# vwxyzjn/cleanrl

Measured on NVIDIA H100. Metric: env steps/sec (SPS) PPO Breakout num_envs=1024, higher is better.
Workload: dtype bf16

## Files before the change

### cleanrl_b200/csrc/common.cuh

```cuda
#pragma once
#include <cuda_runtime.h>
#include <cstdarg>
#include <cstdint>
#include <cstdio>
#include "../../include/b200rl.h"

namespace b200rl {

char* err_buf();
int fail(int code, const char* fmt, ...);

void note_launches(int n);
inline int check_launch(const char* what, int kernels = 1) {
    note_launches(kernels);
    cudaError_t e = cudaGetLastError();
    if (e != cudaSuccess) return fail(B200RL_ERR_CUDA, "%s: %s", what, cudaGetErrorString(e));
    return B200RL_OK;
}

#define B200RL_REQUIRE(cond, ...) \
    do { if (!(cond)) return ::b200rl::fail(B200RL_ERR_INVALID_ARGUMENT, __VA_ARGS__); } while (0)

inline bool aligned(const void* p, size_t a) { return (reinterpret_cast<uintptr_t>(p) % a) == 0; }
inline int64_t ceil_div(int64_t a, int64_t b) { return (a + b - 1) / b; }

bool prof_enabled();
void prof_begin(cudaStream_t s, const char* name, double flops, double bytes);
void prof_end(cudaStream_t s);
struct ProfScope {
    cudaStream_t s; bool on;
    ProfScope(cudaStream_t s_, const char* name, double flops, double bytes) : s(s_), on(prof_enabled()) {
        if (on) prof_begin(s, name, flops, bytes);
    }
    ~ProfScope() { if (on) prof_end(s); }
};

__device__ __forceinline__ float warp_sum(float v) {
#pragma unroll
    for (int o = 16; o > 0; o >>= 1) v += __shfl_xor_sync(0xffffffffu, v, o);
    return v;
}

__device__ __forceinline__ float block_sum(float v, float* red) {
    const int lane = threadIdx.x & 31, wid = threadIdx.x >> 5;
    v = warp_sum(v);
    __syncthreads();
    if (lane == 0) red[wid] = v;
    __syncthreads();
    const int nw = (blockDim.x + 31) >> 5;
    float r = (threadIdx.x < nw) ? red[threadIdx.x] : 0.f;
    if (wid == 0) r = warp_sum(r);
    if (threadIdx.x == 0) red[0] = r;
    __syncthreads();
    r = red[0];
    return r;
}

}
```

### cleanrl_b200/csrc/net_tc.cu

```cuda
#include <cuda.h>
#include <algorithm>
#include "tc_base.cuh"
#include "tc_conv_win.cuh"
#include "tc_conv1_u8.cuh"
#include "tc_gemm_tma.cuh"
#include "tc_wgrad_win.cuh"
#include "tc_reduce.cuh"
#include "tc_aux.cuh"
#include "tc_heads.cuh"
#include "tc_heads_wide.cuh"
#include "tc_lstm.cuh"

namespace b200rl {

struct NatureLayout {
    int A;
    int64_t c1w, c1b, c2w, c2b, c3w, c3b, fcw, fcb, hw, hb, total;
    int64_t w1f, w2f, w2dg, w3f, w3dg, wfcf, wfcdg, w1l, w1sc, packed_total;
    bool wide; int G; int64_t whf, whdg, hbp;
    int64_t wih, whh, bih, bhh, whhp;
    explicit NatureLayout(int A_) : A(A_), wih(-1), whh(-1), bih(-1), bhh(-1), whhp(-1) {
        int64_t o = 0;
        c1w = o; o += 32 * 4 * 8 * 8;  c1b = o; o += 32;
        c2w = o; o += 64 * 32 * 4 * 4; c2b = o; o += 64;
// ... 52 lines not shown
    }
};

struct NatureActs {
    int64_t x0, act1, act2, act3, hid, dhid, dact3a, dact3b, dact2a, dact2b, dact1, m1, m2, m3, m4, total;
    explicit NatureActs(int64_t n, bool with_x0 = true) {
        int64_t o = 0;
        x0 = o; if (with_x0) o += n * 28224;
        act1 = o; o += n * 12800;
        act2 = o; o += n * 5184;
        act3 = o; o += n * 3136;
        hid = o;  o += n * 512;
        dhid = o; o += n * 512;
        dact3a = o; o += n * 5184;
        dact3b = o; o += n * 7744;
        dact2a = o; o += n * 6400;
        dact2b = o; o += n * 7744;
        dact1 = o; o += n * 14112;
        auto pad8 = [](int64_t v) { return (v + 7) & ~int64_t(7); };
        m1 = o; o += pad8(n * 100 * 4 * 2);
        m2 = o; o += pad8(n * 81 * 2 * 2);
        m3 = o; o += pad8(n * 49 * 2 * 2);
        m4 = o; o += pad8(n * 16 * 2);
        total = o;
    }
};

static void gemm_rowmajor(KGemmParams& p, const bf16* x, int64_t n, int nchunks) {
    memset(&p, 0, sizeof(p));
    p.scale = 1.f;
    p.A = x; p.M = n; p.nchunks = nchunks;
}


static void win_defaults(WinParams& p) { memset(&p, 0, sizeof(p)); p.scale = 1.f; }
static int round8(int v) { return (v + 7) & ~7; }
static void win_conv1(WinParams& p, const bf16* x0, const int64_t* rows, int64_t n) {
    p.A = x0; p.rows = rows; p.n = (int)n; p.G = 441; p.Wp = 21; p.M = n * 441;
    p.tpi_shift = 2;
    p.n_images = rows ? (int64_t)1 << 24 : n;
    p.ntaps = 4; p.shift[0] = 0; p.shift[1] = 1; p.shift[2] = 21; p.shift[3] = 22; p.WR = round8(128 + 22);
}
static void win_conv2(WinParams& p, const bf16* act1, int64_t n) {
    p.A = act1; p.n = (int)n; p.G = 100; p.Wp = 10; p.M = n * 100;
    p.ntaps = 4; p.shift[0] = 0; p.shift[1] = 1; p.shift[2] = 10; p.shift[3] = 11; p.WR = round8(128 + 11);
}
static void win_conv3(WinParams& p, const bf16* act2, int64_t n) {
    p.A = act2; p.n = (int)n; p.G = 81; p.Wp = 9; p.M = n * 81;
    p.ntaps = 9; for (int ky = 0; ky < 3; ++ky) for (int kx = 0; kx < 3; ++kx) p.shift[ky * 3 + kx] = ky * 9 + kx;
    p.WR = round8(128 + 20);
}
static void wgw_defaults(WGradWinParams& w) { memset(&w, 0, sizeof(w)); }

static const int kC1Ctas = 264, kC2Ctas = 132, kC3Ctas = 132;
static WPlan conv1_wgrad_plan(int64_t n, bool u8) {
    return u8 ? wgrad_plan(n * 512, kC2Ctas, 512) : wgrad_plan(n * 512, kC1Ctas, 128);
}
static WPlan conv2_wgrad_plan(int64_t n) { return wgrad_plan(n * 100, kC2Ctas, 128); }
static WPlan conv3_wgrad_plan(int64_t n) { return wgrad_plan(n * 81, kC3Ctas, 128); }

static size_t wgrad_win_bytes(int splits, int nslots) { return (size_t)splits * nslots * 64 * 64 * sizeof(float); }
static size_t wgrad_win_bias_bytes(int splits) { return (size_t)splits * 64 * sizeof(float); }
static int launch_wgrad_win(const WGradWinParams& p, int ctas, cudaStream_t s, const char* what) {
    const size_t smem = (size_t)kWgradWinStages * ((size_t)p.WRX * 128 * p.cpr + 128 * 128) + 4096 + 1024;
    static SmemAttrCache attr;
    if (int rc0 = attr.ensure(tc_wgrad_win, smem, what)) return rc0;
    CUtensorMap tmX, tmY;
    memset(&tmX, 0, sizeof(tmX)); memset(&tmY, 0, sizeof(tmY));
    const int use_tma = p.tpi_shift ? 0 : 1;
    if (p.rows_per_cta % 128 != 0) return fail(B200RL_ERR_INVALID_ARGUMENT, "%s: rows per CTA must be a multiple of 128", what);
    if (ctas < 1 || (int64_t)(ctas - 1) * p.rows_per_cta >= p.M)
        return fail(B200RL_ERR_INVALID_ARGUMENT, "%s: every row split must own at least one row", what);
    int rc;
    if (use_tma) {
        if (p.rows || p.ldy != 64 || p.ncolsY != 64)
            return fail(B200RL_ERR_INVALID_ARGUMENT, "%s: linear-grid mode needs contiguous rows and 64-channel dY", what);
        if ((rc = make_tmap_2d(&tmX, p.X, p.M, (int64_t)p.cpr * 64, p.WRX, what))) return rc;
        if ((rc = make_tmap_2d(&tmY, p.Y, p.M, 64, 128, what))) return rc;
    } else {
        if ((128 << p.tpi_shift) < p.G) return fail(B200RL_ERR_INVALID_ARGUMENT, "%s: steps per image too small", what);
        if ((rc = make_tmap_3d(&tmX, p.X, p.n_images, p.G, (int64_t)p.cpr * 64, p.WRX, what))) return rc;
    }
    const dim3 grid((unsigned)ceil_div(p.nslots / 2, kWgradWinTilesPerCta), ctas);
    tc_wgrad_win<<<grid, kWgradWinThreads, smem, s>>>(tmX, tmY, p, use_tma);
    return check_launch(what);
}

}

using namespace b200rl;

namespace b200rl {
static bool head_ok(int A) { return A >= 1 && A < kMaxWideHeads; }
static size_t wide_dhead_bytes(int64_t n, const NatureLayout& L) { return ((size_t)n * L.G * 2 + 255) & ~(size_t)255; }
static size_t wide_small_bytes(int64_t n, const NatureLayout& L, int A1) {
    return wide_dhead_bytes(n, L) + colsum_f32_ws(n, A1);
}

static int trunk_fwd(const NatureLayout& L, const NatureActs& Q, const float* params, const bf16* P, bf16* act, int64_t n,
                     cudaStream_t s) {
    int rc;
    KGemmParams p;
    WinParams wp;
    win_defaults(wp); win_conv2(wp, act + Q.act1, n);
    wp.Bw = P + L.w2f; wp.N = 64; wp.vH = 9; wp.vW = 9; wp.out_mode = WOUT_DENSE; wp.out = act + Q.act2;
    wp.bias = params + L.c2b; wp.relu = 1; wp.mask_out = reinterpret_cast<uint32_t*>(act + Q.m2);
    { ProfScope ps(s, "conv2_fwd", 2.0 * n * 81 * 64 * 512, (double)n * ((12800 + 5184) * 2 + 648));
      if ((rc = launch_conv_win_t<128, 2, 2, 4>(wp, s, "naturecnn/conv2"))) return rc; }
    win_defaults(wp); win_conv3(wp, act + Q.act2, n);
    wp.Bw = P + L.w3f; wp.N = 64; wp.vH = 7; wp.vW = 7; wp.out_mode = WOUT_DENSE; wp.out = act + Q.act3;
    wp.bias = params + L.c3b; wp.relu = 1; wp.mask_out = reinterpret_cast<uint32_t*>(act + Q.m3);
    { ProfScope ps(s, "conv3_fwd", 2.0 * n * 49 * 64 * 576, (double)n * ((5184 + 3136) * 2 + 392));
      if ((rc = launch_conv_win_t<128, 1, 4, 9>(wp, s, "naturecnn/conv3"))) return rc; }
    gemm_rowmajor(p, act + Q.act3, n, 49);
    p.Bw = P + L.wfcf; p.N = 512; p.out = act + Q.hid; p.ldo = 512; p.bias = params + L.fcb; p.relu = 1;
    p.mask_out = reinterpret_cast<uint32_t*>(act + Q.m4);
    { ProfScope ps(s, "fc_fwd", 2.0 * n * 512 * 3136, (double)n * (3136 + 512) * 2 + 512.0 * 3136 * 2);
      if (n <= 8192) { if ((rc = launch_gemm_tma<64, 6>(p, s, "naturecnn/fc"))) return rc; }
      else if ((rc = launch_gemm_tma<128, 4>(p, s, "naturecnn/fc"))) return rc; }
    return B200RL_OK;
}

static int trunk_bwd(const NatureLayout& L, const NatureActs& Q, const bf16* P, bf16* act, float* grads, int64_t n,
                     float* wsbig, float* wssmall, void* tail_ready_event, bool dact1_fused, cudaStream_t s) {
    int rc;
    KGemmParams p;
    {
        int splits;
        { ProfScope ps(s, "fc_wgrad", 2.0 * n * 512 * 3136, (double)n * (3136 + 512) * 2 + 512.0 * 3136 * 4);
          if ((splits = launch_wgrad_tma(act + Q.dhid, 512, act + Q.act3, 3136, n, wsbig, s, "naturecnn/fc_wgrad")) < 0) return splits; }
        { ProfScope ps(s, "wgrad_fold_bias", 0, 0);
          note_launches(1); tc_fold_fc<<<(unsigned)ceil_div((int64_t)512 * 3136, 256), 256, 0, s>>>(wsbig, splits, 512, 13 * 256, 512, 3136, 64, 49, 1.f, grads + L.fcw);
          if ((rc = colsum(act + Q.dhid, n, 512, 512, wssmall, grads + L.fcb, s))) return rc; }
        if (tail_ready_event) {
            cudaError_t e = cudaEventRecord(reinterpret_cast<cudaEvent_t>(tail_ready_event), s);
            if (e != cudaSuccess) return fail(B200RL_ERR_CUDA, "naturecnn_backward: cudaEventRecord: %s", cudaGetErrorString(e));
        }
        gemm_rowmajor(p, act + Q.dhid, n, 8);
        p.Bw = P + L.wfcdg; p.N = 3136; p.out = act + Q.dact3a; p.out2 = act + Q.dact3b; p.dual_dact3 = 1;
        p.ldo = 3136; p.mask_bits = reinterpret_cast<const uint32_t*>(act + Q.m3);
        { ProfScope ps(s, "fc_dgrad", 2.0 * n * 512 * 3136, (double)n * ((3136 + 512) * 2 + 392) + 512.0 * 3136 * 2);
          if ((rc = launch_gemm_tma<128, 4>(p, s, "naturecnn/fc_dgrad"))) return rc; }
    }
    WGradWinParams gw;
    WinParams wp;
    FoldWin fw;
    {
        wgw_defaults(gw);
        gw.X = act + Q.act2; gw.M = n * 81; gw.n = (int)n; gw.G = 81; gw.cpr = 1; gw.nslots = 10; gw.WRX = round8(128 + 20);
        for (int t = 0; t < 9; ++t) gw.shift[t] = (t / 3) * 9 + (t % 3);
        const int st[10] = {0, 1, 2, 3, 4, 5, 6, 7, 7, 8};
        for (int k = 0; k < 10; ++k) { gw.slot_tap[k] = st[k]; gw.slot_cc[k] = 0; }
        gw.Y = act + Q.dact3a; gw.ldy = 64; gw.ncolsY = 64;
        const WPlan pl = conv3_wgrad_plan(n);
        gw.rows_per_cta = pl.rows_per_cta; gw.ws = wsbig; gw.wsb = wssmall;
        { ProfScope ps(s, "conv3_wgrad", 2.0 * n * 49 * 64 * 576, (double)n * (5184 + 5184) * 2);
          if ((rc = launch_wgrad_win(gw, pl.splits, s, "naturecnn/conv3_wgrad"))) return rc; }
        memset(&fw, 0, sizeof(fw));
        fw.layer = 3; fw.S = pl.splits; fw.nslots = 10; fw.Cout = 64; fw.scale = 1.f; fw.bscale = 1.f;
        for (int k = 0; k < 10; ++k) { fw.slot_tap[k] = st[k]; fw.slot_skip[k] = (k == 8); }
        { ProfScope ps(s, "wgrad_fold_bias", 0, 0);
          fw.wsb = wssmall; fw.db = grads + L.c3b;
          tc_fold_win<<<(unsigned)ceil_div(640 * 64 + 64, 32), 256, 0, s>>>(wsbig, fw, grads + L.c3w);
          if ((rc = check_launch("naturecnn/conv3_fold"))) return rc; }
        win_defaults(wp);
        wp.A = act + Q.dact3b; wp.n = (int)n; wp.G = 121; wp.Wp = 11; wp.M = n * 121; wp.ntaps = 9;
        for (int ky = 0; ky < 3; ++ky) for (int kx = 0; kx < 3; ++kx) wp.shift[ky * 3 + kx] = (2 - ky) * 11 + (2 - kx);
        wp.WR = round8(128 + 24);
        wp.Bw = P + L.w3dg; wp.N = 64; wp.vH = 9; wp.vW = 9; wp.out_mode = WOUT_DACT2;
        wp.out = act + Q.dact2a; wp.out2 = act + Q.dact2b; wp.mask_bits = reinterpret_cast<const uint32_t*>(act + Q.m2);
        { ProfScope ps(s, "conv3_dgrad", 2.0 * n * 81 * 64 * 576, (double)n * ((7744 + 6400 + 7744) * 2 + 648));
          if ((rc = launch_conv_win_t<128, 1, 4, 9>(wp, s, "naturecnn/conv3_dgrad"))) return rc; }
    }
    {
        wgw_defaults(gw);
        gw.X = act + Q.act1; gw.M = n * 100; gw.n = (int)n; gw.G = 100; gw.cpr = 2; gw.nslots = 8; gw.WRX = round8(128 + 11);
        gw.shift[0] = 0; gw.shift[1] = 1; gw.shift[2] = 10; gw.shift[3] = 11;
        for (int k = 0; k < 8; ++k) { gw.slot_tap[k] = k >> 1; gw.slot_cc[k] = k & 1; }
        gw.Y = act + Q.dact2a; gw.ldy = 64; gw.ncolsY = 64;
        const WPlan pl = conv2_wgrad_plan(n);
        gw.rows_per_cta = pl.rows_per_cta; gw.ws = wsbig; gw.wsb = wssmall;
        { ProfScope ps(s, "conv2_wgrad", 2.0 * n * 81 * 64 * 512, (double)n * (12800 + 6400) * 2);
          if ((rc = launch_wgrad_win(gw, pl.splits, s, "naturecnn/conv2_wgrad"))) return rc; }
        memset(&fw, 0, sizeof(fw));
        fw.layer = 2; fw.S = pl.splits; fw.nslots = 8; fw.Cout = 64; fw.scale = 1.f; fw.bscale = 1.f;
        for (int k = 0; k < 8; ++k) { fw.slot_tap[k] = k >> 1; fw.slot_cc[k] = k & 1; }
        { ProfScope ps(s, "wgrad_fold_bias", 0, 0);
          fw.wsb = wssmall; fw.db = grads + L.c2b;
          tc_fold_win<<<(unsigned)ceil_div(512 * 64 + 64, 32), 256, 0, s>>>(wsbig, fw, grads + L.c2w);
          if ((rc = check_launch("naturecnn/conv2_fold"))) return rc; }
        if (dact1_fused) return B200RL_OK;
        win_defaults(wp);
        wp.A = act + Q.dact2b; wp.n = (int)n; wp.G = 121; wp.Wp = 11; wp.M = n * 121; wp.ntaps = 4;
        for (int a = 0; a < 2; ++a) for (int b = 0; b < 2; ++b) wp.shift[a * 2 + b] = (1 - a) * 11 + (1 - b);
        wp.WR = round8(128 + 12);
        wp.Bw = P + L.w2dg; wp.N = 128; wp.vH = 10; wp.vW = 10; wp.out_mode = WOUT_DACT1;
        wp.out = act + Q.dact1; wp.mask_bits = reinterpret_cast<const uint32_t*>(act + Q.m1);
        { ProfScope ps(s, "conv2_dgrad", 2.0 * n * 400 * 32 * 256, (double)n * ((7744 + 14112) * 2 + 1600));
          if ((rc = launch_conv_win<128, 1, 4, 4>(wp, s, "naturecnn/conv2_dgrad"))) return rc; }
    }
    return B200RL_OK;
}
static size_t trunk_big_bytes(int64_t n) {
    return std::max({wgrad_tma_bytes(n, 512, 3136), wgrad_win_bytes(conv3_wgrad_plan(n).splits, 10),
                     wgrad_win_bytes(conv2_wgrad_plan(n).splits, 8)});
}
static size_t trunk_small_bytes(int64_t n) {
    return std::max({colsum_ws(n, 512), wgrad_win_bias_bytes(conv3_wgrad_plan(n).splits),
                     wgrad_win_bias_bytes(conv2_wgrad_plan(n).splits)});
}

static int wide_head_fwd(const NatureLayout& L, const bf16* P, const bf16* hid, int64_t n, int A1, float* out, cudaStream_t s) {
    KGemmParams p;
    gemm_rowmajor(p, hid, n, 8);
    p.Bw = P + L.whf; p.N = L.G; p.bias = reinterpret_cast<const float*>(P + L.hbp);
    p.out_f32 = out; p.ldo = A1; p.ncols_f32 = A1;
    return launch_gemm_tma<128, 4>(p, s, "wide_heads");
}

static int wide_head_bwd(const NatureLayout& L, const bf16* P, const float* dhead, int64_t n, int A1, const bf16* hid, bf16* dhid,
                         const uint32_t* hid_bits, float* dW, float* db, float* wsbig, float* wssmall, cudaStream_t s) {
    int rc;
    KGemmParams p;
    bf16* dh16 = reinterpret_cast<bf16*>(wssmall);
    float* dbpart = reinterpret_cast<float*>(reinterpret_cast<char*>(wssmall) + wide_dhead_bytes(n, L));
    int cb = (int)ceil_div(n * L.G, 256); if (cb > num_sms() * 8) cb = num_sms() * 8;
    tc_head_dhead_bf16<<<cb, 256, 0, s>>>(dhead, n, A1, L.G, dh16);
    if ((rc = check_launch("wide_heads_dhead"))) return rc;
    if ((rc = colsum_f32(dhead, n, A1, dbpart, db, s))) return rc;
    const int splits = launch_wgrad_tma(dh16, L.G, hid, 512, n, wsbig, s, "wide_heads_wgrad");
    if (splits < 0) return splits;
    tc_fold_fc<<<(unsigned)ceil_div((int64_t)A1 * 512, 256), 256, 0, s>>>(wsbig, splits, L.G, 512, A1, 512, 512, 1, 1.f, dW);
    if ((rc = check_launch("wide_heads_wgrad"))) return rc;
    gemm_rowmajor(p, dh16, n, L.G / 64);
    p.Bw = P + L.whdg; p.N = 512; p.out = dhid; p.ldo = 512;
    p.mask_bits = hid_bits;
    if (n <= 8192) { if ((rc = launch_gemm_tma<64, 6>(p, s, "wide_heads_dgrad"))) return rc; }
    else if ((rc = launch_gemm_tma<128, 4>(p, s, "wide_heads_dgrad"))) return rc;
    return B200RL_OK;
}
}

extern "C" int64_t b200rl_naturecnn_param_count(int A) { return A >= 1 ? NatureLayout(A).total : -1; }
extern "C" int64_t b200rl_naturecnn_grad_tail_offset(int A) { return A >= 1 ? NatureLayout(A).fcw : -1; }
extern "C" size_t b200rl_naturecnn_bf16_packed_bytes(int A) { return head_ok(A) ? (size_t)NatureLayout(A).packed_total * 2 : 0; }
extern "C" size_t b200rl_naturecnn_bf16_acts_bytes(int64_t n, int obs_format) {
    return n >= 0 ? (size_t)NatureActs(n, obs_format == B200RL_OBS_U8_NCHW).total * 2 + 256 : 0;
}

extern "C" int b200rl_frames_to_s2d_bf16(const uint8_t* obs, const int64_t* rows, int64_t n, void* out, void* stream) {
    B200RL_REQUIRE(n >= 0, "frames_to_s2d: negative n");
    if (n == 0) return B200RL_OK;
    B200RL_REQUIRE(obs && out, "frames_to_s2d: null pointer");
    B200RL_REQUIRE(aligned(obs, 4) && aligned(out, 16), "frames_to_s2d: misaligned buffer");
    cudaStream_t s = (cudaStream_t)stream;
    ProfScope ps(s, "frames_to_s2d", 0, (double)n * 28224 * 3);
    tc_frames_to_s2d<<<(unsigned)ceil_div(n * 1764, 256), 256, 0, s>>>(obs, rows, n, reinterpret_cast<bf16*>(out));
    return check_launch("frames_to_s2d");
}

extern "C" int b200rl_frames_to_s2d_u8(const uint8_t* obs, const int64_t* rows, int64_t n, uint8_t* out_rm, uint8_t* out_cm, void* stream) {
    B200RL_REQUIRE(n >= 0, "frames_to_s2d_u8: negative n");
    if (n == 0) return B200RL_OK;
    B200RL_REQUIRE(obs && out_rm && out_cm, "frames_to_s2d_u8: null pointer");
    B200RL_REQUIRE(aligned(obs, 16) && aligned(out_rm, 16) && aligned(out_cm, 16), "frames_to_s2d_u8: misaligned buffer");
    B200RL_REQUIRE(n <= (int64_t)1 << 28, "frames_to_s2d_u8: n too large");
    cudaStream_t s = (cudaStream_t)stream;
    ProfScope ps(s, "frames_to_s2d", 0, (double)n * (28224 + 28224 + 28672));
    tc_frames_to_s2d_u8<<<(unsigned)(n * 4), 256, 0, s>>>(obs, rows, n, out_rm, out_cm);
    return check_launch("frames_to_s2d_u8");
}

static size_t naturecnn_big_bytes(int64_t n, const NatureLayout& L) {
    return std::max({trunk_big_bytes(n), L.wide ? wgrad_tma_bytes(n, L.G, 512) : 0,
                     wgrad_win_bytes(conv1_wgrad_plan(n, false).splits, 4), wgrad_win_bytes(conv1_wgrad_plan(n, true).splits, 4)});
}

extern "C" size_t b200rl_naturecnn_bf16_workspace_bytes(int64_t n, int A) {
    if (n < 1 || !head_ok(A)) return 0;
    const NatureLayout L(A);
    const size_t small = std::max({trunk_small_bytes(n), L.wide ? wide_small_bytes(n, L, A + 1) : heads_partial_bytes(n, A + 1, 512),
                                   wgrad_win_bias_bytes(conv1_wgrad_plan(n, false).splits),
                                   wgrad_win_bias_bytes(conv1_wgrad_plan(n, true).splits)});
    return naturecnn_big_bytes(n, L) + small + 512;
}

extern "C" int b200rl_naturecnn_bf16_pack(const float* params, int A, void* packed, void* stream) {
    B200RL_REQUIRE(params && packed && head_ok(A), "naturecnn_pack: bad arguments (A must be in [1,%d])", kMaxWideHeads - 1);
    B200RL_REQUIRE(aligned(packed, 16), "naturecnn_pack: packed buffer must be 16-B aligned");
    const NatureLayout L(A);
    bf16* P = reinterpret_cast<bf16*>(packed);
    cudaStream_t s = (cudaStream_t)stream;
    ProfScope ps(s, "pack_weights", 0, (double)L.total * 4 + (double)L.packed_total * 2);
    tc_pack_conv1_s2d<<<32, 256, 0, s>>>(params + L.c1w, P + L.w1f);
    tc_pack_conv1_i8<<<32, 256, 0, s>>>(params + L.c1w, reinterpret_cast<int8_t*>(P + L.w1l), reinterpret_cast<float*>(P + L.w1sc));
    tc_pack_conv2_cells<<<128, 256, 0, s>>>(params + L.c2w, P + L.w2f);
    tc_pack_conv_s2_classes<<<(unsigned)ceil_div(32768, 256), 256, 0, s>>>(params + L.c2w, 64, 32, P + L.w2dg);
    tc_pack_conv<<<(unsigned)ceil_div(36864, 256), 256, 0, s>>>(params + L.c3w, 64, 64, 3, 3, 0, P + L.w3f, P + L.w3dg);
    tc_pack_fc<<<dim3(512 / 8, 49 / 7), 256, 0, s>>>(params + L.fcw, 512, 49, P + L.wfcf, P + L.wfcdg);
    if (L.wide) {
        tc_pack_head_wide<<<(unsigned)ceil_div((int64_t)L.G * 512, 256), 256, 0, s>>>(params + L.hw, params + L.hb, A + 1, L.G,
                                                                                    P + L.whf, P + L.whdg, reinterpret_cast<float*>(P + L.hbp));
        return check_launch("naturecnn_pack", 7);
    }
    return check_launch("naturecnn_pack", 6);
}

extern "C" int b200rl_naturecnn_bf16_forward(const void* obs, int obs_format, const int64_t* rows, int64_t n, int A,
                                             const float* params, const void* packed, void* acts,
                                             float* head_out, void* stream) {
    B200RL_REQUIRE(n >= 0, "naturecnn_forward: negative n");
    if (n == 0) return B200RL_OK;
    B200RL_REQUIRE(obs && params && packed && acts && head_out, "naturecnn_forward: null pointer");
    B200RL_REQUIRE(head_ok(A), "naturecnn_forward: A=%d outside [1,%d]", A, kMaxWideHeads - 1);
    B200RL_REQUIRE(obs_format == B200RL_OBS_U8_NCHW || obs_format == B200RL_OBS_S2D_BF16 || obs_format == B200RL_OBS_S2D_U8,
                   "naturecnn_forward: bad obs_format %d", obs_format);
    B200RL_REQUIRE(aligned(obs, 16) && aligned(acts, 16) && aligned(packed, 16), "naturecnn_forward: misaligned buffer");
    B200RL_REQUIRE(n <= (int64_t)1 << 22, "naturecnn_forward: n too large");
    const NatureLayout L(A);
    const NatureActs Q(n, obs_format == B200RL_OBS_U8_NCHW);
    const bf16* P = reinterpret_cast<const bf16*>(packed);
    bf16* act = reinterpret_cast<bf16*>(acts);
    cudaStream_t s = (cudaStream_t)stream;
    int rc;
    WinParams wp;
    const bf16* x0 = reinterpret_cast<const bf16*>(obs);
    const int64_t* x0rows = rows;
    if (obs_format == B200RL_OBS_U8_NCHW) {
        if ((rc = b200rl_frames_to_s2d_bf16(reinterpret_cast<const uint8_t*>(obs), rows, n, act + Q.x0, stream))) return rc;
        x0 = act + Q.x0; x0rows = nullptr;
    }
    if (obs_format == B200RL_OBS_S2D_U8) {
        Conv1U8Params cp;
        memset(&cp, 0, sizeof(cp));
        cp.rows = rows; cp.n = (int)n; cp.n_images = rows ? (int64_t)1 << 24 : n;
        cp.limbs = reinterpret_cast<const int8_t*>(P + L.w1l); cp.sc = reinterpret_cast<const float*>(P + L.w1sc);
        cp.bias = params + L.c1b; cp.out = act + Q.act1; cp.mask_out = reinterpret_cast<uint32_t*>(act + Q.m1);
        ProfScope ps(s, "conv1_fwd", 2.0 * n * 400 * 32 * 256, (double)n * (28224 + 12800 * 2 + 1600));
        if ((rc = launch_conv1_i8(cp, obs, s, "naturecnn/conv1_i8"))) return rc;
    } else {
    win_defaults(wp); win_conv1(wp, x0, x0rows, n);
    wp.Bw = P + L.w1f; wp.N = 32; wp.vH = 20; wp.vW = 20; wp.out_mode = WOUT_S2D2; wp.out = act + Q.act1;
    wp.bias = params + L.c1b; wp.scale = 1.0f / 255.0f; wp.relu = 1; wp.mask_out = reinterpret_cast<uint32_t*>(act + Q.m1);
    { ProfScope ps(s, "conv1_fwd", 2.0 * n * 400 * 32 * 256, (double)n * ((28224 + 12800) * 2 + 1600));
      if ((rc = launch_conv_win<32, 1, 9, 4>(wp, s, "naturecnn/conv1"))) return rc; }
    }
    if ((rc = trunk_fwd(L, Q, params, P, act, n, s))) return rc;
    if (L.wide) {
        ProfScope ps(s, "heads_fwd", 2.0 * n * 512 * (A + 1), (double)n * (1024 + 4 * (A + 1)) + (double)L.G * 1024);
        return wide_head_fwd(L, P, act + Q.hid, n, A + 1, head_out, s);
    }
    ProfScope ps(s, "heads_fwd", 2.0 * n * 512 * (A + 1), (double)n * (1024 + 4 * (A + 1)));
    return heads_fwd<512>(act + Q.hid, params + L.hw, params + L.hb, n, A + 1, head_out, s, "naturecnn/heads");
}

extern "C" int b200rl_naturecnn_bf16_backward(const void* obs, const void* obs_aux, int obs_format, const int64_t* rows, int64_t n, int A,
                                              const float* params, const void* packed, void* acts,
                                              const float* dhead, float* grads,
                                              void* workspace, size_t workspace_bytes, void* tail_ready_event, void* stream) {
    B200RL_REQUIRE(n >= 1, "naturecnn_backward: n must be >= 1");
    B200RL_REQUIRE(obs && params && packed && acts && dhead && grads && workspace, "naturecnn_backward: null pointer");
    B200RL_REQUIRE(head_ok(A), "naturecnn_backward: A=%d outside [1,%d]", A, kMaxWideHeads - 1);
    B200RL_REQUIRE(aligned(workspace, 16), "naturecnn_backward: workspace misaligned");
    const size_t need = b200rl_naturecnn_bf16_workspace_bytes(n, A);
    if (workspace_bytes < need) return fail(B200RL_ERR_WORKSPACE, "naturecnn_backward: workspace %zu < %zu", workspace_bytes, need);
    B200RL_REQUIRE(obs_format == B200RL_OBS_U8_NCHW || obs_format == B200RL_OBS_S2D_BF16 || obs_format == B200RL_OBS_S2D_U8,
                   "naturecnn_backward: bad obs_format %d", obs_format);
    B200RL_REQUIRE(obs_format != B200RL_OBS_S2D_U8 || (obs_aux && aligned(obs_aux, 16)), "naturecnn_backward: the uint8 rollout needs obs_aux");
    const NatureLayout L(A);
    const NatureActs Q(n, obs_format == B200RL_OBS_U8_NCHW);
    const bf16* P = reinterpret_cast<const bf16*>(packed);
    bf16* act = reinterpret_cast<bf16*>(acts);
    cudaStream_t s = (cudaStream_t)stream;
    const bf16* x0 = obs_format == B200RL_OBS_U8_NCHW ? act + Q.x0 : reinterpret_cast<const bf16*>(obs);
    const int64_t* x0rows = obs_format == B200RL_OBS_U8_NCHW ? nullptr : rows;
    const size_t big = (naturecnn_big_bytes(n, L) + 255) & ~(size_t)255;
    float* wsbig = reinterpret_cast<float*>(workspace);
    float* wssmall = reinterpret_cast<float*>(reinterpret_cast<char*>(workspace) + big);
    int rc;
    const int A1 = A + 1;
    if (L.wide) {
        ProfScope ps(s, "heads_bwd", 4.0 * n * 512 * A1, (double)n * (2048 + 64 + 8 * A1));
        if ((rc = wide_head_bwd(L, P, dhead, n, A1, act + Q.hid, act + Q.dhid, reinterpret_cast<const uint32_t*>(act + Q.m4),
                                grads + L.hw, grads + L.hb, wsbig, wssmall, s))) return rc;
    } else
    {
        ProfScope ps(s, "heads_bwd", 4.0 * n * 512 * A1, (double)n * (2048 + 64 + 8 * A1));
        if ((rc = heads_bwd_weight<512>(dhead, act + Q.hid, n, A1, wssmall, grads + L.hw, grads + L.hb, s, "naturecnn/heads_bwd"))) return rc;
        if ((rc = heads_bwd_data<512>(dhead, params + L.hw, reinterpret_cast<const uint8_t*>(act + Q.m4), n, A1, act + Q.dhid, s,
                                      "naturecnn/heads_bwd"))) return rc;
    }
    if ((rc = trunk_bwd(L, Q, P, act, grads, n, wsbig, wssmall, tail_ready_event, obs_format == B200RL_OBS_S2D_U8, s))) return rc;
    const bool u8 = obs_format == B200RL_OBS_S2D_U8;
    const WPlan pl = conv1_wgrad_plan(n, u8);
    if (u8) {
        Conv21BwdU8Params cw;
        memset(&cw, 0, sizeof(cw));
        cw.rows = rows; cw.n = (int)n; cw.rows_per_cta = pl.rows_per_cta; cw.ws = wsbig; cw.wsb = wssmall;
        cw.w2dg = P + L.w2dg; cw.m1 = reinterpret_cast<const uint32_t*>(act + Q.m1);
        { ProfScope ps(s, "conv21_bwd", 2.0 * 2.0 * n * 400 * 32 * 256, (double)n * (7744 * 2 + 1600 + 28672 + 14112 * 2));
          if ((rc = launch_conv21_bwd_u8(cw, obs_aux, rows ? (int64_t)1 << 24 : n, act + Q.dact2b, act + Q.dact1, pl.splits, s,
                                         "naturecnn/conv21_bwd_u8"))) return rc; }
    } else {
        WGradWinParams gw;
        wgw_defaults(gw);
        gw.X = x0; gw.rows = x0rows; gw.M = n * 512; gw.n = (int)n; gw.G = 441; gw.cpr = 1; gw.nslots = 4; gw.WRX = round8(128 + 22);
        gw.tpi_shift = 2; gw.n_images = x0rows ? (int64_t)1 << 24 : n;
        gw.shift[0] = 0; gw.shift[1] = 1; gw.shift[2] = 21; gw.shift[3] = 22;
        for (int k = 0; k < 4; ++k) { gw.slot_tap[k] = k; gw.slot_cc[k] = 0; }
        gw.Y = act + Q.dact1; gw.ldy = 32; gw.ncolsY = 32;
        gw.rows_per_cta = pl.rows_per_cta; gw.ws = wsbig; gw.wsb = wssmall;
        { ProfScope ps(s, "conv1_wgrad", 2.0 * n * 400 * 32 * 256, (double)n * (28224 + 14112) * 2);
          if ((rc = launch_wgrad_win(gw, pl.splits, s, "naturecnn/conv1_wgrad"))) return rc; }
    }
    FoldWin fw;
    memset(&fw, 0, sizeof(fw));
    fw.layer = 1; fw.S = pl.splits; fw.nslots = 4; fw.Cout = 32;
    fw.scale = u8 ? 1.0f / 255.0f / kDact1Scale : 1.0f / 255.0f;
    fw.bscale = u8 ? 1.0f / kDact1Scale : 1.f;
    for (int k = 0; k < 4; ++k) fw.slot_tap[k] = k;
    { ProfScope ps(s, "wgrad_fold_bias", 0, 0);
      fw.wsb = wssmall; fw.db = grads + L.c1b;
      tc_fold_win<<<(unsigned)ceil_div(256 * 32 + 32, 32), 256, 0, s>>>(wsbig, fw, grads + L.c1w);
      if ((rc = check_launch("naturecnn/conv1_fold"))) return rc; }
    return B200RL_OK;
}

namespace b200rl {
constexpr int64_t kLstmMaxRows = (int64_t)1 << 17;

struct LstmActs {
    NatureActs T;
    int64_t gx, hseq, hm, save, cm, dgates, total;
    explicit LstmActs(int64_t M) : T(M, false) {
        int64_t o = (T.total * 2 + 255) & ~int64_t(255);
        auto take = [&](int64_t bytes) { const int64_t r = o; o += (bytes + 255) & ~int64_t(255); return r; };
        gx = take(M * 512 * 4);
        hseq = take(M * 128 * 2);
        hm = take(M * 128 * 2);
        save = take(M * 640 * 4);
        cm = take(M * 128 * 4);
        dgates = take(M * 512 * 4);
        total = o;
    }
};

static bool lstm_heads_ok(int A) { return A >= 1 && A + 1 <= lstm::kMaxA1; }
static bool lstm_sizes_ok(int64_t S, int64_t n) { return S >= 1 && n >= 1 && S <= kLstmMaxRows && n <= kLstmMaxRows && S * n <= kLstmMaxRows; }

struct C1Plan { int64_t per_cta; int ctas; };
static C1Plan lstm_conv1_plan(int64_t M) {
    C1Plan c;
    const int64_t want = M < kC1Ctas ? M : kC1Ctas;
    c.per_cta = ceil_div(M, want);
    c.ctas = (int)ceil_div(M, c.per_cta);
    return c;
}
static size_t lstm_big_bytes(int64_t M, const NatureLayout& L) {
    const size_t a = std::max({wgrad_tma_bytes(M, L.G, 512), wgrad_tma_bytes(M, 512, 128), trunk_big_bytes(M),
                               (size_t)lstm_conv1_plan(M).ctas * 32 * 64 * 4});
    return (a + 255) & ~(size_t)255;
}
static size_t lstm_small_bytes(int64_t M, const NatureLayout& L) {
    return std::max({heads_partial_bytes(M, L.A + 1, 128), wide_small_bytes(M, L, 512), trunk_small_bytes(M),
                     (size_t)lstm_conv1_plan(M).ctas * 32 * 4});
}
}

extern "C" int64_t b200rl_lstm_agent_param_count(int A) { return A >= 1 ? NatureLayout(A, NatureLayout::Lstm{}).total : -1; }
extern "C" size_t b200rl_lstm_agent_bf16_packed_bytes(int A) {
    return lstm_heads_ok(A) ? (size_t)NatureLayout(A, NatureLayout::Lstm{}).packed_total * 2 : 0;
}
extern "C" size_t b200rl_lstm_agent_bf16_acts_bytes(int64_t S, int64_t n) {
    return lstm_sizes_ok(S, n) ? (size_t)LstmActs(S * n).total : 0;
}
extern "C" int b200rl_lstm_agent_bf16_acts_layout(int64_t S, int64_t n, int64_t* offsets) {
    B200RL_REQUIRE(offsets, "lstm_acts_layout: null pointer");
    B200RL_REQUIRE(lstm_sizes_ok(S, n), "lstm_acts_layout: S=%lld n=%lld out of range", (long long)S, (long long)n);
    const LstmActs Q(S * n);
    const int64_t v[B200RL_LSTM_ACTS_TENSORS] = {Q.T.act1 * 2, Q.T.m1 * 2, Q.T.act2 * 2, Q.T.act3 * 2, Q.T.hid * 2, Q.T.m4 * 2,
                                                 Q.gx, Q.hseq, Q.hm, Q.save, Q.cm, Q.dgates, Q.T.dhid * 2};
    for (int k = 0; k < B200RL_LSTM_ACTS_TENSORS; ++k) offsets[k] = v[k];
    return B200RL_OK;
}
extern "C" size_t b200rl_lstm_agent_bf16_workspace_bytes(int64_t S, int64_t n, int A) {
    if (!lstm_sizes_ok(S, n) || !lstm_heads_ok(A)) return 0;
    const NatureLayout L(A, NatureLayout::Lstm{});
    return lstm_big_bytes(S * n, L) + lstm_small_bytes(S * n, L) + 512;
}

extern "C" int b200rl_lstm_agent_bf16_pack(const float* params, int A, void* packed, void* stream) {
    B200RL_REQUIRE(params && packed, "lstm_pack: null pointer");
    B200RL_REQUIRE(lstm_heads_ok(A), "lstm_pack: A=%d outside [1,%d]", A, lstm::kMaxA1 - 1);
    B200RL_REQUIRE(aligned(params, 16) && aligned(packed, 16), "lstm_pack: misaligned buffer");
    const NatureLayout L(A, NatureLayout::Lstm{});
    bf16* P = reinterpret_cast<bf16*>(packed);
    cudaStream_t s = (cudaStream_t)stream;
    ProfScope ps(s, "pack_weights", 0, (double)L.total * 4 + (double)L.packed_total * 2);
    lstm::lstm_pack_conv1<<<8, 256, 0, s>>>(params + L.c1w, P + L.w1f);
    tc_pack_conv2_cells<<<128, 256, 0, s>>>(params + L.c2w, P + L.w2f);
    tc_pack_conv_s2_classes<<<(unsigned)ceil_div(32768, 256), 256, 0, s>>>(params + L.c2w, 64, 32, P + L.w2dg);
    tc_pack_conv<<<(unsigned)ceil_div(36864, 256), 256, 0, s>>>(params + L.c3w, 64, 64, 3, 3, 0, P + L.w3f, P + L.w3dg);
    tc_pack_fc<<<dim3(512 / 8, 49 / 7), 256, 0, s>>>(params + L.fcw, 512, 49, P + L.wfcf, P + L.wfcdg);
    tc_pack_head_wide<<<(unsigned)ceil_div((int64_t)L.G * 512, 256), 256, 0, s>>>(params + L.wih, params + L.bih, 512, L.G,
                                                                                P + L.whf, P + L.whdg, reinterpret_cast<float*>(P + L.hbp));
    tc_head_dhead_bf16<<<256, 256, 0, s>>>(params + L.whh, 512, 128, 128, P + L.whhp);
    return check_launch("lstm_pack", 7);
// ... 121 lines not shown
```

### cleanrl_b200/csrc/optim.cu

```cuda
#include "common.cuh"

namespace b200rl {

constexpr int kOptThreads = 256;
constexpr int kOptMaxBlocks = 132 * 8;

struct OptScratch {
    float norm;
    float coef;
    unsigned int ticket;
    unsigned int pad;
};

__global__ void __launch_bounds__(kOptThreads) grad_sumsq_kernel(
    const float* __restrict__ g, int64_t P, float inv_world_is_div, float world,
    float max_norm, OptScratch* sc, double* partials, float* norm_out) {
    __shared__ float red[32];
    __shared__ bool is_last;
    float s = 0.f;
    const int64_t stride = (int64_t)gridDim.x * blockDim.x;
    const int64_t tid = (int64_t)blockIdx.x * blockDim.x + threadIdx.x;
    const int64_t P4 = P >> 2;
    const float4* g4 = reinterpret_cast<const float4*>(g);
    for (int64_t i = tid; i < P4; i += stride) {
        float4 v = __ldg(g4 + i);
        if (inv_world_is_div != 0.f) { v.x /= world; v.y /= world; v.z /= world; v.w /= world; }
        s += v.x * v.x + v.y * v.y + v.z * v.z + v.w * v.w;
    }
    for (int64_t i = (P4 << 2) + tid; i < P; i += stride) {
        float v = g[i];
        if (inv_world_is_div != 0.f) v /= world;
        s += v * v;
    }
    const float bs = block_sum(s, red);
    if (threadIdx.x == 0) {
        partials[blockIdx.x] = (double)bs;
        __threadfence();
        is_last = (atomicAdd(&sc->ticket, 1u) == gridDim.x - 1);
    }
    __syncthreads();
    if (!is_last) return;
    __threadfence();
    __shared__ double dred[kOptThreads];
    double mine = 0.0;
    for (unsigned b = threadIdx.x; b < gridDim.x; b += blockDim.x) mine += __ldcg(partials + b);
    dred[threadIdx.x] = mine;
    __syncthreads();
    for (unsigned off = kOptThreads / 2; off > 0; off >>= 1) {
        if (threadIdx.x < off) dred[threadIdx.x] += dred[threadIdx.x + off];
        __syncthreads();
    }
    if (threadIdx.x == 0) {
        const double tot = dred[0];
        const float norm = (float)sqrt(tot);
        sc->norm = norm;
        float coef = 1.f;
        if (max_norm >= 0.f) coef = fminf(max_norm / (norm + 1e-6f), 1.0f);
        sc->coef = coef;
        if (norm_out) *norm_out = norm;
        sc->ticket = 0;
    }
}

struct AdamScalars {
    float w1;
    float beta2;
    float w2;
    float bc2_sqrt;
    float eps;
    float neg_step_size;
    float world;
    int divide_world;
    int do_clip;
};

__device__ __forceinline__ void adam_one(float& p, float g, float& m, float& v, const AdamScalars& a, float coef) {
    if (a.divide_world) g = g / a.world;
    if (a.do_clip) g = g * coef;
    m = fmaf(a.w1, g - m, m);
    v = v * a.beta2;
    v = __fadd_rn(v, __fmul_rn(__fmul_rn(a.w2, g), g));
    const float denom = __fadd_rn(__fdiv_rn(sqrtf(v), a.bc2_sqrt), a.eps);
    p = __fadd_rn(p, __fmul_rn(a.neg_step_size, __fdiv_rn(m, denom)));
}

__global__ void __launch_bounds__(kOptThreads) adam_kernel(
    float* __restrict__ p, const float* __restrict__ g, float* __restrict__ m, float* __restrict__ v,
    int64_t P, AdamScalars a, const OptScratch* sc, const float* __restrict__ dyn) {
    if (dyn) { a.bc2_sqrt = __ldg(dyn); a.neg_step_size = __ldg(dyn + 1); }
    const float coef = a.do_clip ? sc->coef : 1.f;
    const int64_t stride = (int64_t)gridDim.x * blockDim.x;
    const int64_t tid = (int64_t)blockIdx.x * blockDim.x + threadIdx.x;
    const int64_t P4 = P >> 2;
    float4* p4 = reinterpret_cast<float4*>(p);
    const float4* g4 = reinterpret_cast<const float4*>(g);
    float4* m4 = reinterpret_cast<float4*>(m);
    float4* v4 = reinterpret_cast<float4*>(v);
    for (int64_t i = tid; i < P4; i += stride) {
        float4 pp = p4[i], gg = __ldg(g4 + i), mm = m4[i], vv = v4[i];
        adam_one(pp.x, gg.x, mm.x, vv.x, a, coef);
        adam_one(pp.y, gg.y, mm.y, vv.y, a, coef);
        adam_one(pp.z, gg.z, mm.z, vv.z, a, coef);
        adam_one(pp.w, gg.w, mm.w, vv.w, a, coef);
        p4[i] = pp; m4[i] = mm; v4[i] = vv;
    }
    for (int64_t i = (P4 << 2) + tid; i < P; i += stride) {
        float pp = p[i], mm = m[i], vv = v[i];
        adam_one(pp, g[i], mm, vv, a, coef);
        p[i] = pp; m[i] = mm; v[i] = vv;
    }
}

static inline unsigned opt_blocks(int64_t P) {
    int64_t b = ceil_div(ceil_div(P, 4), kOptThreads);
    if (b < 1) b = 1;
    if (b > kOptMaxBlocks) b = kOptMaxBlocks;
    return (unsigned)b;
}

}

extern "C" size_t b200rl_clip_adam_workspace_bytes(int64_t P) {
    (void)P;
    return sizeof(b200rl::OptScratch) + sizeof(double) * b200rl::kOptMaxBlocks;
}

namespace b200rl {
static void adam_step_scalars(int64_t step, double lr, double beta1, double beta2, float* bc2_sqrt, float* neg_step_size) {
    const double bc1 = 1.0 - pow(beta1, (double)step);
    const double bc2 = 1.0 - pow(beta2, (double)step);
    const double step_size = lr / bc1;
    *bc2_sqrt = (float)sqrt(bc2);
    *neg_step_size = (float)(-step_size);
}

static int clip_adam_impl(float* params, const float* grads, float* exp_avg, float* exp_avg_sq, int64_t P, int64_t step, double lr,
                          const float* dyn, double beta1, double beta2, double eps, double max_norm, int world_size, float* norm_out,
                          void* workspace, size_t workspace_bytes, void* stream) {
    B200RL_REQUIRE(P >= 0, "clip_adam: negative P");
    if (P == 0) return B200RL_OK;
    B200RL_REQUIRE(params && grads && exp_avg && exp_avg_sq, "clip_adam: null pointer");
    B200RL_REQUIRE(aligned(params, 16) && aligned(grads, 16) && aligned(exp_avg, 16) && aligned(exp_avg_sq, 16),
                   "clip_adam: buffers must be 16-B aligned (float4 path)");
    B200RL_REQUIRE(dyn || step >= 1, "clip_adam: step is 1-based (got %lld)", (long long)step);
    B200RL_REQUIRE(!dyn || aligned(dyn, 4), "clip_adam: misaligned scalar table");
    B200RL_REQUIRE(world_size >= 1, "clip_adam: world_size must be >= 1");
    B200RL_REQUIRE(workspace && aligned(workspace, 16), "clip_adam: workspace null or misaligned");
    if (workspace_bytes < b200rl_clip_adam_workspace_bytes(P))
        return fail(B200RL_ERR_WORKSPACE, "clip_adam: workspace %zu < %zu bytes", workspace_bytes,
                    b200rl_clip_adam_workspace_bytes(P));
    cudaStream_t s = (cudaStream_t)stream;
    OptScratch* sc = reinterpret_cast<OptScratch*>(workspace);
    double* partials = reinterpret_cast<double*>(reinterpret_cast<char*>(workspace) + sizeof(OptScratch));
    const unsigned blocks = opt_blocks(P);
    ProfScope ps(s, "clip_adam", 0, 32.0 * P);
    const bool need_norm = (max_norm >= 0.0) || (norm_out != nullptr);
    if (need_norm) {
        cudaError_t e = cudaMemsetAsync(&sc->ticket, 0, sizeof(unsigned int), s);
        if (e != cudaSuccess) return fail(B200RL_ERR_CUDA, "clip_adam: memset: %s", cudaGetErrorString(e));
        grad_sumsq_kernel<<<blocks, kOptThreads, 0, s>>>(grads, P, world_size > 1 ? 1.f : 0.f, (float)world_size,
                                                        (float)max_norm, sc, partials, norm_out);
        int rc = check_launch("clip_adam/sumsq");
        if (rc) return rc;
    }
    AdamScalars a;
    a.w1 = (float)(1.0 - beta1);
    a.beta2 = (float)beta2;
    a.w2 = (float)(1.0 - beta2);
    a.bc2_sqrt = 1.f;
    a.neg_step_size = 0.f;
    if (!dyn) adam_step_scalars(step, lr, beta1, beta2, &a.bc2_sqrt, &a.neg_step_size);
    a.eps = (float)eps;
    a.world = (float)world_size;
    a.divide_world = world_size > 1;
    a.do_clip = max_norm >= 0.0;
    adam_kernel<<<blocks, kOptThreads, 0, s>>>(params, grads, exp_avg, exp_avg_sq, P, a, sc, dyn);
    return check_launch("clip_adam/adam");
}
}

extern "C" int b200rl_clip_adam_f32(float* params, const float* grads, float* exp_avg, float* exp_avg_sq,
                                    int64_t P, int64_t step, double lr, double beta1, double beta2, double eps,
                                    double max_norm, int world_size, float* norm_out,
                                    void* workspace, size_t workspace_bytes, void* stream) {
    return b200rl::clip_adam_impl(params, grads, exp_avg, exp_avg_sq, P, step, lr, nullptr, beta1, beta2, eps, max_norm, world_size,
                                  norm_out, workspace, workspace_bytes, stream);
}

extern "C" int b200rl_adam_step_scalars(int64_t step, double lr, double beta1, double beta2, float* out2) {
    B200RL_REQUIRE(out2 && step >= 1, "adam_step_scalars: bad arguments");
    b200rl::adam_step_scalars(step, lr, beta1, beta2, out2, out2 + 1);
    return B200RL_OK;
}

extern "C" int b200rl_clip_adam_dyn_f32(float* params, const float* grads, float* exp_avg, float* exp_avg_sq,
                                        int64_t P, const float* step_scalars, double beta1, double beta2, double eps,
                                        double max_norm, int world_size, float* norm_out,
                                        void* workspace, size_t workspace_bytes, void* stream) {
    B200RL_REQUIRE(step_scalars, "clip_adam_dyn: null scalar table");
    return b200rl::clip_adam_impl(params, grads, exp_avg, exp_avg_sq, P, 0, 0.0, step_scalars, beta1, beta2, eps, max_norm, world_size,
                                  norm_out, workspace, workspace_bytes, stream);
}
```

### cleanrl_b200/csrc/policy.cu

```cuda
#include "common.cuh"
#include <cfloat>

namespace b200rl {

constexpr int kMaxA = 64;

struct RowStats {
    float lse;
    float m2;
    float s2;
};

__device__ __forceinline__ RowStats row_stats(const float* __restrict__ x, int A) {
    float m = -INFINITY;
    for (int k = 0; k < A; ++k) m = fmaxf(m, x[k]);
    const float mm = (fabsf(m) == INFINITY) ? 0.f : m;
    float s = 0.f;
    for (int k = 0; k < A; ++k) s += expf(x[k] - mm);
    RowStats r;
    r.lse = logf(s) + mm;
    float m2 = -INFINITY;
    for (int k = 0; k < A; ++k) m2 = fmaxf(m2, x[k] - r.lse);
    float s2 = 0.f;
    for (int k = 0; k < A; ++k) s2 += expf((x[k] - r.lse) - m2);
    r.m2 = m2;
    r.s2 = s2;
    return r;
}

__global__ void __launch_bounds__(128) categorical_sample_kernel(
    const float* __restrict__ logits, int64_t ld, const float* __restrict__ noise,
    const float* __restrict__ value_in, int64_t ldv, int64_t n, int A,
    int64_t* __restrict__ action, float* __restrict__ logprob, float* __restrict__ entropy,
    float* __restrict__ value_out) {
    const int64_t i = (int64_t)blockIdx.x * blockDim.x + threadIdx.x;
    if (i >= n) return;
    const float* x = logits + i * ld;
    const float* q = noise + i * (int64_t)A;
    const RowStats rs = row_stats(x, A);
    float best = -INFINITY, ent = 0.f;
    int arg = 0;
    for (int k = 0; k < A; ++k) {
        const float nl = x[k] - rs.lse;
        const float p = expf(nl - rs.m2) / rs.s2;
        const float sc = p / q[k];
        if (sc > best) { best = sc; arg = k; }
        ent += fmaxf(nl, -FLT_MAX) * p;
    }
    action[i] = arg;
    logprob[i] = x[arg] - rs.lse;
    if (entropy) entropy[i] = -ent;
    if (value_out && value_in) value_out[i] = value_in[i * ldv];
}

__global__ void __launch_bounds__(128) categorical_eval_kernel(
    const float* __restrict__ logits, int64_t ld, const int64_t* __restrict__ action, int64_t n, int A,
    float* __restrict__ logprob, float* __restrict__ entropy) {
    const int64_t i = (int64_t)blockIdx.x * blockDim.x + threadIdx.x;
    if (i >= n) return;
    const float* x = logits + i * ld;
    const RowStats rs = row_stats(x, A);
    float ent = 0.f;
    for (int k = 0; k < A; ++k) {
        const float nl = x[k] - rs.lse;
        ent += fmaxf(nl, -FLT_MAX) * (expf(nl - rs.m2) / rs.s2);
    }
    int a = (int)action[i];
    a = a < 0 ? 0 : (a >= A ? A - 1 : a);
    logprob[i] = x[a] - rs.lse;
    if (entropy) entropy[i] = -ent;
}

__device__ __forceinline__ float adv_pass(const float* __restrict__ b_adv, const int64_t* __restrict__ inds, int64_t M,
                                          float mean, bool squared) {
    float s = 0.f;
    const int64_t step = blockDim.x;
    int64_t i = threadIdx.x;
    for (; i + 7 * step < M; i += 8 * step) {
        int64_t j[8];
        float v[8];
#pragma unroll
        for (int u = 0; u < 8; ++u) j[u] = inds ? __ldg(inds + i + u * step) : i + u * step;
#pragma unroll
        for (int u = 0; u < 8; ++u) v[u] = __ldg(b_adv + j[u]);
#pragma unroll
        for (int u = 0; u < 8; ++u) {
            const float d = v[u] - mean;
            s += squared ? d * d : v[u];
        }
    }
    for (; i < M; i += step) {
        const float v = b_adv[inds ? inds[i] : i];
        const float d = v - mean;
        s += squared ? d * d : v;
    }
    return s;
}
__global__ void __launch_bounds__(1024) adv_stats_kernel(
    const float* __restrict__ b_adv, const int64_t* __restrict__ inds, int64_t M, float* __restrict__ out2) {
    __shared__ float red[32];
    const float mean = block_sum(adv_pass(b_adv, inds, M, 0.f, false), red) / (float)M;
    const float ss = block_sum(adv_pass(b_adv, inds, M, mean, true), red);
    if (threadIdx.x == 0) {
        out2[0] = mean;
        out2[1] = sqrtf(ss / (float)(M - 1));
    }
}

constexpr int kLossThreads = 256;
constexpr int kNumStats = 7;

struct LossParams {
    const float* logits; int64_t ld;
    const float* value; int64_t ldv;
    const int64_t* inds;
    const int64_t* b_actions;
    const float* b_logprobs; const float* b_adv; const float* b_ret; const float* b_val;
    int64_t M; int A;
    float clip, ent_coef, vf_coef;
    int norm_adv, clip_vloss;
    float* dlogits; int64_t ldd;
    float* dvalue; int64_t lddv;
    float* stats;
    const float* adv_stats;
    float* partials;
    unsigned int* ticket;
};

__global__ void __launch_bounds__(kLossThreads) ppo_loss_kernel(LossParams P) {
    __shared__ float red[32];
    __shared__ bool is_last;
    const int64_t i = (int64_t)blockIdx.x * blockDim.x + threadIdx.x;
    float acc[kNumStats];
#pragma unroll
    for (int k = 0; k < kNumStats; ++k) acc[k] = 0.f;
    if (i < P.M) {
        const int64_t j = P.inds ? P.inds[i] : i;
        const float* x = P.logits + i * P.ld;
        const int A = P.A;
        const int a = (int)P.b_actions[j];
        const RowStats rs = row_stats(x, A);
        float ent = 0.f;
        for (int k = 0; k < A; ++k) {
            const float nl = x[k] - rs.lse;
            const float p = expf(nl - rs.m2) / rs.s2;
            ent += fmaxf(nl, -FLT_MAX) * p;
        }
        ent = -ent;
        const float newlogprob = x[a] - rs.lse;
        const float logratio = newlogprob - P.b_logprobs[j];
        const float ratio = expf(logratio);
        float adv = P.b_adv[j];
        if (P.norm_adv) adv = (adv - P.adv_stats[0]) / (P.adv_stats[1] + 1e-8f);
        const float lo = 1.f - P.clip, hi = 1.f + P.clip;
        const float rc = fminf(fmaxf(ratio, lo), hi);
        const float pg1 = -adv * ratio, pg2 = -adv * rc;
        const float pg = fmaxf(pg1, pg2);
        const float nv = P.value[i * P.ldv];
        const float R = P.b_ret[j], V = P.b_val[j];
        float vterm, gv;
        const float du = nv - R;
        const float vu = du * du;
        if (P.clip_vloss) {
            const float d = nv - V;
            const float vcl = V + fminf(fmaxf(d, -P.clip), P.clip);
            const float dc = vcl - R;
            const float vc = dc * dc;
            vterm = fmaxf(vu, vc);
            const float gu = 2.f * du;
            const float gc = (d >= -P.clip && d <= P.clip) ? 2.f * dc : 0.f;
            gv = (vu > vc) ? gu : ((vc > vu) ? gc : 0.5f * (gu + gc));
        } else {
            vterm = vu;
            gv = 2.f * du;
        }
        acc[0] = pg;
        acc[1] = vterm;
        acc[2] = ent;
        acc[3] = -logratio;
        acc[4] = (ratio - 1.f) - logratio;
        acc[5] = (fabsf(ratio - 1.0f) > P.clip) ? 1.f : 0.f;
        const float invM = 1.0f / (float)P.M;
        const float inrange = (ratio >= lo && ratio <= hi) ? 1.f : 0.f;
        float g_ratio = 0.f;
        if (pg1 > pg2) g_ratio = -adv;
        else if (pg1 == pg2) g_ratio = 0.5f * (-adv) * (1.f + inrange);
        const float g_lp = g_ratio * ratio * invM;
        const float g_ent = -P.ent_coef * invM;
        float* dl = P.dlogits + i * P.ldd;
        for (int k = 0; k < A; ++k) {
            const float nl = x[k] - rs.lse;
            const float p = expf(nl - rs.m2) / rs.s2;
            const float onehot = (k == a) ? 1.f : 0.f;
            dl[k] = g_lp * (onehot - p) + g_ent * (-p * (nl + ent));
        }
        P.dvalue[i * P.lddv] = P.vf_coef * 0.5f * invM * gv;
    }
#pragma unroll
    for (int k = 0; k < 6; ++k) {
        const float s = block_sum(acc[k], red);
        if (threadIdx.x == 0) P.partials[(int64_t)blockIdx.x * kNumStats + k] = s;
    }
    if (threadIdx.x == 0) {
        __threadfence();
        const unsigned t = atomicAdd(P.ticket, 1u);
        is_last = (t == gridDim.x - 1);
    }
    __syncthreads();
    if (!is_last) return;
    __threadfence();
    float tot[6];
#pragma unroll
// ... 133 lines not shown
        acc[1] = vterm;
        acc[2] = ent;
        acc[3] = -logratio;
        acc[4] = (ratio - 1.f) - logratio;
        acc[5] = (fabsf(ratio - 1.0f) > P.clip) ? 1.f : 0.f;
        const float invM = 1.0f / (float)P.M;
        const float inrange = (ratio >= lo && ratio <= hi) ? 1.f : 0.f;
        float g_ratio = 0.f;
        if (pg1 > pg2) g_ratio = -adv;
        else if (pg1 == pg2) g_ratio = 0.5f * (-adv) * (1.f + inrange);
        g_lp = g_ratio * ratio * invM;
        float* dm = P.dmean + i * P.ldd;
        for (int d = 0; d < D; ++d) {
            const float std = expf(P.logstd[d]);
            dm[d] = g_lp * (a[d] - m[d]) / (std * std);
        }
        P.dvalue[i * P.lddv] = P.vf_coef * 0.5f * invM * gv;
    }
    float* pb = P.partials + (int64_t)blockIdx.x * (kNumStats + kMaxD);
#pragma unroll
    for (int k = 0; k < 6; ++k) {
        const float s = block_sum(acc[k], red);
        if (threadIdx.x == 0) pb[k] = s;
    }
    for (int d = 0; d < D; ++d) {
        float t = 0.f;
        if (i < P.M) {
            const float std = expf(P.logstd[d]);
            const float diff = a[d] - m[d];
            t = g_lp * (diff * diff / (std * std) - 1.f);
        }
        const float s = block_sum(t, red);
        if (threadIdx.x == 0) pb[kNumStats + d] = s;
    }
    if (threadIdx.x == 0) {
        __threadfence();
        is_last = (atomicAdd(P.ticket, 1u) == gridDim.x - 1);
    }
    __syncthreads();
    if (!is_last) return;
    __threadfence();
    float tot[6];
#pragma unroll
    for (int k = 0; k < 6; ++k) {
        float s = 0.f;
        for (unsigned b = threadIdx.x; b < gridDim.x; b += blockDim.x) s += __ldcg(P.partials + (int64_t)b * (kNumStats + kMaxD) + k);
        tot[k] = block_sum(s, red);
    }
    for (int d = 0; d < D; ++d) {
        float s = 0.f;
        for (unsigned b = threadIdx.x; b < gridDim.x; b += blockDim.x) s += __ldcg(P.partials + (int64_t)b * (kNumStats + kMaxD) + kNumStats + d);
        const float t = block_sum(s, red);
        if (threadIdx.x == 0) P.dlogstd[d] = t - P.ent_coef;
    }
    if (threadIdx.x == 0) {
        const float invM = 1.0f / (float)P.M;
        const float pg_loss = tot[0] * invM;
        const float v_loss = 0.5f * (tot[1] * invM);
        const float ent_loss = tot[2] * invM;
        P.stats[0] = pg_loss; P.stats[1] = v_loss; P.stats[2] = ent_loss;
        P.stats[3] = tot[3] * invM; P.stats[4] = tot[4] * invM; P.stats[5] = tot[5] * invM;
        P.stats[6] = pg_loss - P.ent_coef * ent_loss + v_loss * P.vf_coef;
        P.stats[7] = P.norm_adv ? P.adv_stats[0] : 0.f;
        P.stats[8] = P.norm_adv ? P.adv_stats[1] : 1.f;
        *P.ticket = 0;
    }
}

}

extern "C" int b200rl_categorical_sample_f32(const float* logits, int64_t ld_logits, const float* noise,
                                             const float* value_in, int64_t ld_value,
                                             int64_t n, int A,
                                             int64_t* action, float* logprob, float* entropy, float* value_out,
                                             void* stream) {
    using namespace b200rl;
    B200RL_REQUIRE(n >= 0, "categorical_sample: negative n");
    if (n == 0) return B200RL_OK;
    B200RL_REQUIRE(A >= 1 && A <= kMaxA, "categorical_sample: A=%d outside [1,%d]", A, kMaxA);
    B200RL_REQUIRE(logits && noise && action && logprob, "categorical_sample: null pointer");
    B200RL_REQUIRE(ld_logits >= A, "categorical_sample: ld_logits < A");
    const unsigned blocks = (unsigned)ceil_div(n, 128);
    ProfScope ps((cudaStream_t)stream, "categorical_sample", 0, (double)n * (8.0 * A + 24));
    categorical_sample_kernel<<<blocks, 128, 0, (cudaStream_t)stream>>>(
        logits, ld_logits, noise, value_in, ld_value, n, A, action, logprob, entropy, value_out);
    return check_launch("categorical_sample");
}

extern "C" int b200rl_categorical_eval_f32(const float* logits, int64_t ld_logits, const int64_t* action,
                                           int64_t n, int A, float* logprob, float* entropy, void* stream) {
    using namespace b200rl;
    B200RL_REQUIRE(n >= 0, "categorical_eval: negative n");
    if (n == 0) return B200RL_OK;
    B200RL_REQUIRE(A >= 1 && A <= kMaxA, "categorical_eval: A=%d outside [1,%d]", A, kMaxA);
    B200RL_REQUIRE(logits && action && logprob, "categorical_eval: null pointer");
    B200RL_REQUIRE(ld_logits >= A, "categorical_eval: ld_logits < A");
    categorical_eval_kernel<<<(unsigned)ceil_div(n, 128), 128, 0, (cudaStream_t)stream>>>(
        logits, ld_logits, action, n, A, logprob, entropy);
    return check_launch("categorical_eval");
}

extern "C" size_t b200rl_ppo_loss_workspace_bytes(int64_t M) {
    using namespace b200rl;
    if (M < 0) return 0;
    const int64_t blocks = ceil_div(M > 0 ? M : 1, kLossThreads);
    return 32 + (size_t)blocks * kNumStats * sizeof(float);
}

extern "C" int b200rl_ppo_loss_f32(const float* new_logits, int64_t ld_logits,
                                   const float* new_value, int64_t ld_value,
                                   const int64_t* mb_inds,
                                   const int64_t* b_actions, const float* b_logprobs,
                                   const float* b_advantages, const float* b_returns, const float* b_values,
                                   int64_t M, int A,
                                   double clip_coef, double ent_coef, double vf_coef,
                                   int norm_adv, int clip_vloss,
                                   float* dlogits, int64_t ld_dlogits, float* dvalue, int64_t ld_dvalue,
                                   float* stats, void* workspace, size_t workspace_bytes, void* stream) {
    using namespace b200rl;
    B200RL_REQUIRE(M >= 1, "ppo_loss: M must be >= 1 (got %lld)", (long long)M);
    B200RL_REQUIRE(!norm_adv || M >= 2, "ppo_loss: norm_adv needs M >= 2 (unbiased std)");
    B200RL_REQUIRE(A >= 1 && A <= kMaxA, "ppo_loss: A=%d outside [1,%d]", A, kMaxA);
    B200RL_REQUIRE(new_logits && new_value && b_actions && b_logprobs && b_advantages && b_returns && b_values,
                   "ppo_loss: null input pointer");
    B200RL_REQUIRE(dlogits && dvalue && stats, "ppo_loss: null output pointer");
    B200RL_REQUIRE(ld_logits >= A && ld_dlogits >= A && ld_value >= 1 && ld_dvalue >= 1, "ppo_loss: bad strides");
    B200RL_REQUIRE(workspace && aligned(workspace, 16), "ppo_loss: workspace null or not 16-B aligned");
    if (workspace_bytes < b200rl_ppo_loss_workspace_bytes(M))
        return fail(B200RL_ERR_WORKSPACE, "ppo_loss: workspace %zu < %zu bytes", workspace_bytes,
                    b200rl_ppo_loss_workspace_bytes(M));
    cudaStream_t s = (cudaStream_t)stream;
    float* adv_stats = reinterpret_cast<float*>(workspace);
    unsigned int* ticket = reinterpret_cast<unsigned int*>(reinterpret_cast<char*>(workspace) + 16);
    float* partials = reinterpret_cast<float*>(reinterpret_cast<char*>(workspace) + 32);
    ProfScope ps(s, "ppo_loss", 0, (double)M * (44.0 + 8.0 * A));
    cudaError_t e = cudaMemsetAsync(ticket, 0, sizeof(unsigned int), s);
    if (e != cudaSuccess) return fail(B200RL_ERR_CUDA, "ppo_loss: memset: %s", cudaGetErrorString(e));
    if (norm_adv) { note_launches(1); adv_stats_kernel<<<1, 1024, 0, s>>>(b_advantages, mb_inds, M, adv_stats); }
    LossParams P;
    P.logits = new_logits; P.ld = ld_logits; P.value = new_value; P.ldv = ld_value;
    P.inds = mb_inds; P.b_actions = b_actions; P.b_logprobs = b_logprobs; P.b_adv = b_advantages;
    P.b_ret = b_returns; P.b_val = b_values; P.M = M; P.A = A;
    P.clip = (float)clip_coef; P.ent_coef = (float)ent_coef; P.vf_coef = (float)vf_coef;
    P.norm_adv = norm_adv; P.clip_vloss = clip_vloss;
    P.dlogits = dlogits; P.ldd = ld_dlogits; P.dvalue = dvalue; P.lddv = ld_dvalue;
    P.stats = stats; P.adv_stats = adv_stats; P.partials = partials; P.ticket = ticket;
    const unsigned blocks = (unsigned)ceil_div(M, kLossThreads);
    ppo_loss_kernel<<<blocks, kLossThreads, 0, s>>>(P);
    return check_launch("ppo_loss");
}

extern "C" int b200rl_gaussian_sample_f32(const float* mean, int64_t ld_mean, const float* logstd, const float* noise,
                                          const float* value_in, int64_t ld_value, int64_t n, int D,
                                          float* action, float* logprob, float* entropy, float* value_out, void* stream) {
    using namespace b200rl;
    B200RL_REQUIRE(n >= 0, "gaussian_sample: negative n");
    if (n == 0) return B200RL_OK;
    B200RL_REQUIRE(D >= 1 && D <= kMaxD, "gaussian_sample: D=%d outside [1,%d]", D, kMaxD);
    B200RL_REQUIRE(mean && logstd && noise && action && logprob, "gaussian_sample: null pointer");
    B200RL_REQUIRE(ld_mean >= D, "gaussian_sample: ld_mean < D");
    ProfScope ps((cudaStream_t)stream, "gaussian_sample", 0, (double)n * (12.0 * D + 16));
    gaussian_sample_kernel<<<(unsigned)ceil_div(n, 128), 128, 0, (cudaStream_t)stream>>>(
        mean, ld_mean, logstd, noise, value_in, ld_value, n, D, action, logprob, entropy, value_out);
    return check_launch("gaussian_sample");
}

extern "C" int b200rl_gaussian_eval_f32(const float* mean, int64_t ld_mean, const float* logstd, const float* action,
                                        int64_t n, int D, float* logprob, float* entropy, void* stream) {
    using namespace b200rl;
    B200RL_REQUIRE(n >= 0, "gaussian_eval: negative n");
    if (n == 0) return B200RL_OK;
    B200RL_REQUIRE(D >= 1 && D <= kMaxD, "gaussian_eval: D=%d outside [1,%d]", D, kMaxD);
    B200RL_REQUIRE(mean && logstd && action && logprob, "gaussian_eval: null pointer");
    B200RL_REQUIRE(ld_mean >= D, "gaussian_eval: ld_mean < D");
    gaussian_eval_kernel<<<(unsigned)ceil_div(n, 128), 128, 0, (cudaStream_t)stream>>>(mean, ld_mean, logstd, action, n, D, logprob, entropy);
    return check_launch("gaussian_eval");
}

extern "C" size_t b200rl_ppo_loss_gaussian_workspace_bytes(int64_t M) {
    using namespace b200rl;
    if (M < 0) return 0;
    return 32 + (size_t)ceil_div(M > 0 ? M : 1, kLossThreads) * (kNumStats + kMaxD) * sizeof(float);
}

extern "C" int b200rl_ppo_loss_gaussian_f32(const float* new_mean, int64_t ld_mean, const float* logstd,
                                            const float* new_value, int64_t ld_value, const int64_t* mb_inds,
                                            const float* b_actions, const float* b_logprobs,
                                            const float* b_advantages, const float* b_returns, const float* b_values,
                                            int64_t M, int D, double clip_coef, double ent_coef, double vf_coef,
                                            int norm_adv, int clip_vloss,
                                            float* dmean, int64_t ld_dmean, float* dlogstd, float* dvalue, int64_t ld_dvalue,
                                            float* stats, void* workspace, size_t workspace_bytes, void* stream) {
    using namespace b200rl;
    B200RL_REQUIRE(M >= 1, "ppo_loss_gaussian: M must be >= 1");
    B200RL_REQUIRE(!norm_adv || M >= 2, "ppo_loss_gaussian: norm_adv needs M >= 2");
    B200RL_REQUIRE(D >= 1 && D <= kMaxD, "ppo_loss_gaussian: D=%d outside [1,%d]", D, kMaxD);
    B200RL_REQUIRE(new_mean && logstd && new_value && b_actions && b_logprobs && b_advantages && b_returns && b_values,
                   "ppo_loss_gaussian: null input pointer");
    B200RL_REQUIRE(dmean && dlogstd && dvalue && stats, "ppo_loss_gaussian: null output pointer");
    B200RL_REQUIRE(ld_mean >= D && ld_dmean >= D && ld_value >= 1 && ld_dvalue >= 1, "ppo_loss_gaussian: bad strides");
    B200RL_REQUIRE(workspace && aligned(workspace, 16), "ppo_loss_gaussian: workspace null or misaligned");
    if (workspace_bytes < b200rl_ppo_loss_gaussian_workspace_bytes(M))
        return fail(B200RL_ERR_WORKSPACE, "ppo_loss_gaussian: workspace %zu < %zu bytes", workspace_bytes,
                    b200rl_ppo_loss_gaussian_workspace_bytes(M));
    cudaStream_t s = (cudaStream_t)stream;
    float* adv_stats = reinterpret_cast<float*>(workspace);
    unsigned int* ticket = reinterpret_cast<unsigned int*>(reinterpret_cast<char*>(workspace) + 16);
    float* partials = reinterpret_cast<float*>(reinterpret_cast<char*>(workspace) + 32);
    ProfScope ps(s, "ppo_loss_gaussian", 0, (double)M * (48.0 + 12.0 * D));
    cudaError_t e = cudaMemsetAsync(ticket, 0, sizeof(unsigned int), s);
    if (e != cudaSuccess) return fail(B200RL_ERR_CUDA, "ppo_loss_gaussian: memset: %s", cudaGetErrorString(e));
    if (norm_adv) { note_launches(1); adv_stats_kernel<<<1, 1024, 0, s>>>(b_advantages, mb_inds, M, adv_stats); }
    GLossParams P;
    P.mean = new_mean; P.ld = ld_mean; P.logstd = logstd; P.value = new_value; P.ldv = ld_value; P.inds = mb_inds;
    P.b_actions = b_actions; P.b_logprobs = b_logprobs; P.b_adv = b_advantages; P.b_ret = b_returns; P.b_val = b_values;
    P.M = M; P.D = D; P.clip = (float)clip_coef; P.ent_coef = (float)ent_coef; P.vf_coef = (float)vf_coef;
    P.norm_adv = norm_adv; P.clip_vloss = clip_vloss;
    P.dmean = dmean; P.ldd = ld_dmean; P.dlogstd = dlogstd; P.dvalue = dvalue; P.lddv = ld_dvalue;
    P.stats = stats; P.adv_stats = adv_stats; P.partials = partials; P.ticket = ticket;
    ppo_loss_gaussian_kernel<<<(unsigned)ceil_div(M, kLossThreads), kLossThreads, 0, s>>>(P);
    return check_launch("ppo_loss_gaussian");
}
```

### cleanrl_b200/csrc/tc_aux.cuh

```cuda
#pragma once
#include "tc_base.cuh"

namespace b200rl {
using namespace tc;

__global__ void __launch_bounds__(256) tc_frames_to_s2d(const uint8_t* __restrict__ obs, const int64_t* __restrict__ rows,
                                                        int64_t n, bf16* __restrict__ out) {
    const int64_t idx = (int64_t)blockIdx.x * blockDim.x + threadIdx.x;
    if (idx >= n * 21 * 21 * 4) return;
    const int c = (int)(idx & 3);
    int64_t t = idx >> 2;
    const int X = (int)(t % 21); t /= 21;
    const int Y = (int)(t % 21);
    const int64_t i = t / 21;
    const int64_t img = rows ? rows[i] : i;
    const uint8_t* src = obs + img * 28224 + c * 7056 + (Y * 4) * 84 + X * 4;
    uint32_t o[8];
#pragma unroll
    for (int sy = 0; sy < 4; ++sy) {
        const uint32_t w = __ldg(reinterpret_cast<const uint32_t*>(src + sy * 84));
        o[2 * sy] = pack_bf16x2((float)(w & 0xFF), (float)((w >> 8) & 0xFF));
        o[2 * sy + 1] = pack_bf16x2((float)((w >> 16) & 0xFF), (float)(w >> 24));
    }
    int4* dst = reinterpret_cast<int4*>(out + (idx >> 2) * 64 + c * 16);
    dst[0] = make_int4((int)o[0], (int)o[1], (int)o[2], (int)o[3]);
    dst[1] = make_int4((int)o[4], (int)o[5], (int)o[6], (int)o[7]);
}

__global__ void tc_pack_conv(const float* __restrict__ w, int Cout, int Cin, int KH, int KW, int nchw_k,
                             bf16* __restrict__ fwd, bf16* __restrict__ dgrad) {
    const int64_t idx = (int64_t)blockIdx.x * blockDim.x + threadIdx.x;
    const int64_t total = (int64_t)Cout * Cin * KH * KW;
    if (idx >= total) return;
    int kx = (int)(idx % KW); int64_t t = idx / KW;
    int ky = (int)(t % KH); t /= KH;
    int c = (int)(t % Cin); int co = (int)(t / Cin);
    const bf16 v = __float2bfloat16(w[idx]);
    const int K = Cin * KH * KW;
    if (nchw_k) fwd[(int64_t)co * K + (c * KH + ky) * KW + kx] = v;
    else fwd[(int64_t)co * K + (ky * KW + kx) * Cin + c] = v;
    if (dgrad) dgrad[(int64_t)c * (KH * KW * Cout) + (ky * KW + kx) * Cout + co] = v;
}
__global__ void tc_pack_conv1_s2d(const float* __restrict__ w, bf16* __restrict__ fwd) {
    const int idx = blockIdx.x * blockDim.x + threadIdx.x;
    if (idx >= 32 * 256) return;
    const int kx = idx & 7, ky = (idx >> 3) & 7, c = (idx >> 6) & 3, co = idx >> 8;
    const int a = ky >> 2, sy = ky & 3, b = kx >> 2, sx = kx & 3;
    fwd[co * 256 + (a * 2 + b) * 64 + c * 16 + sy * 4 + sx] = __float2bfloat16(w[idx]);
}
__global__ void tc_pack_conv2_cells(const float* __restrict__ w, bf16* __restrict__ fwd) {
    const int idx = blockIdx.x * blockDim.x + threadIdx.x;
    if (idx >= 64 * 512) return;
    const int kx = idx & 3, ky = (idx >> 2) & 3, c = (idx >> 4) & 31, co = idx >> 9;
    const int a = ky >> 1, py = ky & 1, b = kx >> 1, px = kx & 1;
    fwd[co * 512 + (a * 2 + b) * 128 + (py * 2 + px) * 32 + c] = __float2bfloat16(w[idx]);
}
__global__ void tc_pack_conv_s2_classes(const float* __restrict__ w, int Cout, int Cin, bf16* __restrict__ dg) {
    const int64_t idx = (int64_t)blockIdx.x * blockDim.x + threadIdx.x;
    const int64_t total = (int64_t)4 * Cin * 4 * Cout;
    if (idx >= total) return;
    int co = (int)(idx % Cout); int64_t t = idx / Cout;
    int ab = (int)(t % 4); t /= 4;
    int c = (int)(t % Cin); int cls = (int)(t / Cin);
    const int py = cls >> 1, px = cls & 1, a = ab >> 1, b = ab & 1;
    dg[idx] = __float2bfloat16(w[(((int64_t)co * Cin + c) * 4 + (py + 2 * a)) * 4 + (px + 2 * b)]);
}
__global__ void __launch_bounds__(256) tc_pack_fc(const float* __restrict__ w, int O, int PP, bf16* __restrict__ fwd,
                                                  bf16* __restrict__ dgrad) {
    constexpr int C = 64, PS = 7, R = 8;
    __shared__ float sw[R * C * PS];
    const int K = C * PP;
    const int o0 = blockIdx.x * R, p0 = blockIdx.y * PS;
    for (int i = threadIdx.x; i < R * C * PS; i += blockDim.x) {
        const int pl = i % PS, rc = i / PS;
        sw[i] = w[(int64_t)(o0 + (rc >> 6)) * K + (rc & 63) * PP + p0 + pl];
    }
    __syncthreads();
    for (int i = threadIdx.x; i < R * PS * (C / 8); i += blockDim.x) {
        const int g = i & 7, pl = (i >> 3) % PS, r = i / (8 * PS);
        const float* src = sw + (r * C + g * 8) * PS + pl;
        int4 v;
        v.x = (int)pack_bf16x2(src[0 * PS], src[1 * PS]); v.y = (int)pack_bf16x2(src[2 * PS], src[3 * PS]);
        v.z = (int)pack_bf16x2(src[4 * PS], src[5 * PS]); v.w = (int)pack_bf16x2(src[6 * PS], src[7 * PS]);
        *reinterpret_cast<int4*>(fwd + (int64_t)(o0 + r) * K + (p0 + pl) * C + g * 8) = v;
    }
    for (int i = threadIdx.x; i < PS * C; i += blockDim.x) {
        const int c = i & 63, pl = i >> 6;
        const float* src = sw + c * PS + pl;
        int4 v;
        v.x = (int)pack_bf16x2(src[0 * C * PS], src[1 * C * PS]); v.y = (int)pack_bf16x2(src[2 * C * PS], src[3 * C * PS]);
        v.z = (int)pack_bf16x2(src[4 * C * PS], src[5 * C * PS]); v.w = (int)pack_bf16x2(src[6 * C * PS], src[7 * C * PS]);
        *reinterpret_cast<int4*>(dgrad + ((int64_t)(p0 + pl) * C + c) * O + o0) = v;
    }
}

}
```

### cleanrl_b200/csrc/tc_conv1_u8.cuh

```cuda
#pragma once
#include "tc_base.cuh"
#include <cuda_fp16.h>
#include "tc_conv_win.cuh"

namespace b200rl {
using namespace tc;

__device__ __forceinline__ uint64_t desc_kmajor_sw64(uint32_t smem_addr) {
    return (uint64_t)((smem_addr & 0x3FFFFu) >> 4) | (1ull << 16) | (32ull << 32) | kDescSwizzle64;
}
__device__ __forceinline__ uint64_t desc_mnmajor_sw64(uint32_t smem_addr, uint32_t lbo) {
    return (uint64_t)((smem_addr & 0x3FFFFu) >> 4) | ((uint64_t)((lbo >> 4) & 0x3FFF) << 16) | (32ull << 32) | kDescSwizzle64;
}
__device__ __forceinline__ uint32_t img64_off(int r, int c) { return (uint32_t)(r * 64 + ((c ^ ((r >> 1) & 3)) << 4)); }
__global__ void __launch_bounds__(256) tc_frames_to_s2d_u8(const uint8_t* __restrict__ obs, const int64_t* __restrict__ rows, int64_t n,
                                                           uint8_t* __restrict__ out_rm, uint8_t* __restrict__ out_cm) {
    __shared__ __align__(16) uint8_t plane[7056];
    const int64_t i = blockIdx.x >> 2;
    const int c = blockIdx.x & 3;
    const int64_t img = rows ? rows[i] : i;
    const int4* src = reinterpret_cast<const int4*>(obs + img * 28224 + c * 7056);
    for (int t = threadIdx.x; t < 441; t += 256) reinterpret_cast<int4*>(plane)[t] = __ldg(src + t);
    __syncthreads();
    for (int pos = threadIdx.x; pos < 441; pos += 256) {
        const int Y = pos / 21, X = pos - Y * 21;
        const uint8_t* p = plane + (Y * 4) * 84 + X * 4;
        int4 v;
        v.x = *reinterpret_cast<const int*>(p); v.y = *reinterpret_cast<const int*>(p + 84);
        v.z = *reinterpret_cast<const int*>(p + 168); v.w = *reinterpret_cast<const int*>(p + 252);
        *reinterpret_cast<int4*>(out_rm + (i * 441 + pos) * 64 + c * 16) = v;
    }
    for (int t = threadIdx.x; t < 16 * 112; t += 256) {
        const int ch = t / 112, q = t - ch * 112;
        const int sy = ch >> 2, sx = ch & 3;
        uint32_t w = 0;
#pragma unroll
        for (int e = 0; e < 4; ++e) {
            const int pos = q * 4 + e;
            if (pos < 441) {
                const int Y = pos / 21, X = pos - Y * 21;
                w |= (uint32_t)plane[(Y * 4 + sy) * 84 + X * 4 + sx] << (8 * e);
            }
        }
        *reinterpret_cast<uint32_t*>(out_cm + (i * 64 + c * 16 + ch) * 448 + q * 4) = w;
    }
}

__global__ void __launch_bounds__(256) tc_pack_conv1_i8(const float* __restrict__ w, int8_t* __restrict__ limbs, float* __restrict__ sc) {
    __shared__ float red[32];
    const int co = blockIdx.x, idx = threadIdx.x;
    const float v = w[co * 256 + idx];
    float m = fabsf(v);
#pragma unroll
    for (int o = 16; o > 0; o >>= 1) m = fmaxf(m, __shfl_xor_sync(0xffffffffu, m, o));
    if ((idx & 31) == 0) red[idx >> 5] = m;
    __syncthreads();
    float mx = red[0];
#pragma unroll
    for (int k = 1; k < 8; ++k) mx = fmaxf(mx, red[k]);
    const float s = mx > 0.f ? mx * (128.0f / 127.0f) : 1.0f;
    const float u = v / s * 128.0f;
    float l1 = rintf(u);
    l1 = fminf(fmaxf(l1, -127.f), 127.f);
    float l2 = rintf((u - l1) * 128.0f);
    l2 = fminf(fmaxf(l2, -127.f), 127.f);
    const int kx = idx & 7, ky = (idx >> 3) & 7, c = idx >> 6;
    const int a = ky >> 2, sy = ky & 3, b = kx >> 2, sx = kx & 3;
    const int k = (a * 2 + b) * 64 + c * 16 + sy * 4 + sx;
    limbs[co * 256 + k] = (int8_t)l1;
    limbs[(32 + co) * 256 + k] = (int8_t)l2;
    if (idx == 0) {
        sc[co] = s / 128.0f / 255.0f;
        sc[32 + co] = s / 16384.0f / 255.0f;
    }
}

struct Conv1U8Params {
    const int64_t* rows;
    int n;
    int64_t n_images;
    const int8_t* limbs;
    const float* sc;
    const float* bias;
    bf16* out;
    uint32_t* mask_out;
};

constexpr int kConv1I8Threads = 384;
template <int STAGES>
__global__ void __launch_bounds__(kConv1I8Threads, 1) tc_conv1_i8(const __grid_constant__ CUtensorMap tmA, const Conv1U8Params p, int total_tiles) {
    constexpr int BN = 64, WR = 144, NTAPS = 4;
    constexpr int STAGE_BYTES = WR * 128;
    constexpr int B_CHUNK = BN * 64;
    extern __shared__ uint8_t smem_raw[];
    __shared__ uint64_t full_bar[STAGES], empty_bar[STAGES];
    __shared__ __align__(16) float s_sc[32], s_bias[32];
    uint8_t* smem = reinterpret_cast<uint8_t*>((reinterpret_cast<uintptr_t>(smem_raw) + 1023) & ~uintptr_t(1023));
    const int tid = threadIdx.x, warp = tid >> 5;
    uint8_t* sW = smem;
    uint8_t* sRing = smem + NTAPS * B_CHUNK;

    if (tid == 0) {
        for (int s = 0; s < STAGES; ++s) { mbar_init(&full_bar[s], 1); mbar_init(&empty_bar[s], 8); }
        fence_barrier_init();
        tma_prefetch_desc(&tmA);
    }
    for (int idx = tid; idx < NTAPS * BN * 4; idx += blockDim.x) {
        const int c16 = idx & 3;
        const int t = (idx >> 2) & 3;
        const int r = idx >> 4;
        *reinterpret_cast<int4*>(sW + t * B_CHUNK + img64_off(r, c16)) = ldg16(p.limbs + r * 256 + t * 64 + c16 * 16);
    }
    if (tid < 32) { s_sc[tid] = p.sc[32 + tid]; s_bias[tid] = p.bias[tid]; }
    fence_proxy_async_smem();
    __syncthreads();
    const int tile_begin = (int)(((int64_t)total_tiles * blockIdx.x) / gridDim.x);
    const int tile_end = (int)(((int64_t)total_tiles * (blockIdx.x + 1)) / gridDim.x);

    if (warp == 0) {
        if (tid == 0) {
            uint32_t q = 0;
            int z_next = 0;
            if (tile_begin < tile_end) {
                const int img = tile_begin >> 1;
                z_next = p.rows ? (int)__ldg(p.rows + img) : img;
            }
            for (int tile = tile_begin; tile < tile_end; ++tile, ++q) {
                const uint32_t s = q % STAGES;
                const int z = z_next;
                if (tile + 1 < tile_end) {
                    const int img = (tile + 1) >> 1;
                    z_next = p.rows ? (int)__ldg(p.rows + img) : img;
                }
                if (q >= (uint32_t)STAGES) mbar_wait(&empty_bar[s], ((q / STAGES) - 1) & 1);
                mbar_arrive_expect_tx(&full_bar[s], (uint32_t)STAGE_BYTES);
                tma_load_3d(smem_u32(sRing + (size_t)s * STAGE_BYTES), &tmA, 0, (tile & 1) * 128, z, &full_bar[s]);
            }
        }
    } else if (warp >= 4) {
        const int wg = (warp - 4) >> 2, wt = tid & 127, lane = tid & 31, qd = lane & 3;
        const uint32_t w_base = smem_u32(sW);
        constexpr int off[4] = {0, 1, 21, 22};
        int acc[2][32];
#pragma unroll
        for (int e = 0; e < 2; ++e)
#pragma unroll
            for (int c = 0; c < 32; ++c) acc[e][c] = 0;
        for (int tile = tile_begin; tile < tile_end; ++tile) {
            const uint32_t q = (uint32_t)(tile - tile_begin), s = q % STAGES;
            mbar_wait(&full_bar[s], (q / STAGES) & 1);
            wgmma_fence();
            const uint32_t win = smem_u32(sRing + (size_t)s * STAGE_BYTES) + (uint32_t)(wg * 64 * 128);
#pragma unroll
            for (int e = 0; e < 2; ++e) {
#pragma unroll
                for (int t = 0; t < NTAPS; ++t) {
                    const int po = e + off[t];
                    const uint64_t a = desc_kmajor(win + (uint32_t)((po >> 1) * 128 + (po & 1) * 64));
                    const uint64_t b = desc_kmajor_sw64(w_base + (uint32_t)(t * B_CHUNK));
#pragma unroll
                    for (int kk = 0; kk < 2; ++kk) wgmma_u8s8_n64(acc[e], a + 2 * kk, b + 2 * kk, (t | kk) != 0 ? 1u : 0u);
                }
            }
            wgmma_commit();
            wgmma_wait<0>();
            wgmma_fence_operands(acc[0]);
            wgmma_fence_operands(acc[1]);
            if (lane == 0) mbar_arrive(&empty_bar[s]);
            const int i = tile >> 1;
#pragma unroll
            for (int e = 0; e < 2; ++e) {
#pragma unroll
                for (int hr = 0; hr < 2; ++hr) {
                    const int lrow = wg * 64 + ((wt >> 5) << 4) + (lane >> 2) + 8 * hr;
                    const int rem = 2 * (((tile & 1) << 7) + lrow) + e;
                    const int Y = (rem * 3121) >> 16, X = rem - Y * 21;
                    const bool valid = rem < 441 && Y < 20 && X < 20;
                    const int64_t cell = ((int64_t)i * 10 + (Y >> 1)) * 10 + (X >> 1);
                    const int cls = (Y & 1) * 2 + (X & 1);
                    uint32_t bits = 0u, pk[4];
#pragma unroll
                    for (int j = 0; j < 4; ++j) {
                        const int co = 8 * j + 2 * qd;
                        const float f0 = fmaf((float)(acc[e][4 * j + 2 * hr] * 128 + acc[e][4 * (j + 4) + 2 * hr]), s_sc[co], s_bias[co]);
                        const float f1 = fmaf((float)(acc[e][4 * j + 2 * hr + 1] * 128 + acc[e][4 * (j + 4) + 2 * hr + 1]), s_sc[co + 1],
                                              s_bias[co + 1]);
                        bits |= (f0 > 0.f ? 1u : 0u) << co;
                        bits |= (f1 > 0.f ? 1u : 0u) << (co + 1);
                        pk[j] = pack_bf16x2_relu(f0, f1);
                    }
                    bits |= __shfl_xor_sync(0xffffffffu, bits, 1);
                    bits |= __shfl_xor_sync(0xffffffffu, bits, 2);
                    if (valid) {
                        if (qd == 0) p.mask_out[cell * 4 + cls] = bits;
                        uint32_t* dst = reinterpret_cast<uint32_t*>(reinterpret_cast<uint8_t*>(p.out) + (cell * 4 + cls) * 64);
#pragma unroll
                        for (int j = 0; j < 4; ++j) dst[4 * j + qd] = pk[j];
                    }
// ... 7 lines not shown
    const int64_t* rows;
    int n;
    int64_t rows_per_cta;
    const bf16* w2dg;
    const uint32_t* m1;
    float* ws;
    float* wsb;
};
constexpr int kC1WXStages = 6, kC21WinStages = 2;
constexpr int kC1WBlock = 64 * 128, kC1WYBytes = 128 * 64, kC1WYPadRows = 24, kC1WYPad = kC1WYPadRows * 64;
constexpr int kC1WShift = 21;
constexpr int kC21WinRows = 140, kC21WinBytes = 18 * 1024;
constexpr int kC21W2Bytes = 4 * 128 * 128;
constexpr int kC21ImgBytes = kC1WYPad + 4 * kC1WYBytes;
constexpr float kDact1Scale = 4096.0f;

__device__ __forceinline__ uint32_t prmt(uint32_t a, uint32_t b, uint32_t sel) {
    uint32_t d;
    asm("prmt.b32 %0, %1, %2, %3;" : "=r"(d) : "r"(a), "r"(b), "r"(sel));
    return d;
}
constexpr float kU8Bias = 1024.0f;


__device__ __forceinline__ uint32_t pair_f16_biased(const uint32_t (&w)[5], int j, bool up, uint32_t sel) {
    const uint32_t lo = up ? w[j + 1] : w[j];
    const uint32_t hi = up ? w[j + 2] : w[j + 1];
    return prmt(prmt(lo, hi, sel), 0x64646464u, 0x5140u);
}
__device__ __forceinline__ uint4 lds128(uint32_t addr) {
    uint4 v;
    asm volatile("ld.shared.v4.u32 {%0, %1, %2, %3}, [%4];" : "=r"(v.x), "=r"(v.y), "=r"(v.z), "=r"(v.w) : "r"(addr) : "memory");
    return v;
}
__device__ __forceinline__ uint32_t pack_f16x2_sat(float lo, float hi) {
    uint32_t d;
    asm("cvt.rn.satfinite.f16x2.f32 %0, %1, %2;" : "=r"(d) : "f"(hi), "f"(lo));
    return d;
}

__device__ __forceinline__ void sts32(uint32_t addr, uint32_t v) { asm volatile("st.shared.u32 [%0], %1;" ::"r"(addr), "r"(v) : "memory"); }
__device__ __forceinline__ void tma_store_3d(const void* tmap, uint32_t smem_src, int x, int y, int z) {
    asm volatile("cp.async.bulk.tensor.3d.global.shared::cta.bulk_group [%0, {%1, %2, %3}], [%4];"
                 ::"l"(reinterpret_cast<uint64_t>(tmap)), "r"(x), "r"(y), "r"(z), "r"(smem_src) : "memory");
}
__device__ __forceinline__ void bulk_commit() { asm volatile("cp.async.bulk.commit_group;" ::: "memory"); }
template <int N> __device__ __forceinline__ void bulk_wait_read() { asm volatile("cp.async.bulk.wait_group.read %0;" ::"n"(N) : "memory"); }
template <int N> __device__ __forceinline__ void bulk_wait() { asm volatile("cp.async.bulk.wait_group %0;" ::"n"(N) : "memory"); }

template <int R> __device__ __forceinline__ void setmaxnreg_dec() { asm volatile("setmaxnreg.dec.sync.aligned.u32 %0;" ::"n"(R)); }
template <int R> __device__ __forceinline__ void setmaxnreg_inc() { asm volatile("setmaxnreg.inc.sync.aligned.u32 %0;" ::"n"(R)); }
constexpr int kC1WRegsProducer = 40, kC21RegsDgrad = 128, kC1WRegsMma = 168;
static_assert(128 * kC1WRegsProducer + 128 * kC21RegsDgrad + 256 * kC1WRegsMma <= 65536, "register budgets exceed the SM");

constexpr int kC1WThreads = 512;
__global__ void __launch_bounds__(kC1WThreads, 1) tc_conv21_bwd_u8(const __grid_constant__ CUtensorMap tmX, const __grid_constant__ CUtensorMap tmWin,
                                                                 const __grid_constant__ CUtensorMap tmY, const Conv21BwdU8Params p) {
    constexpr int XS = kC1WXStages, WS = kC21WinStages;
    extern __shared__ uint8_t smem_raw[];
    __shared__ uint64_t xfull[XS], xempty[XS], wfull[WS], wempty[WS], yfull[2], yempty[2];
    __shared__ float sRed[32 * 32], sBias[32];
    uint8_t* smem = reinterpret_cast<uint8_t*>((reinterpret_cast<uintptr_t>(smem_raw) + 1023) & ~uintptr_t(1023));
    uint8_t* sW2 = smem;
    uint8_t* sWin = sW2 + kC21W2Bytes;
    uint8_t* sX = sWin + (size_t)WS * kC21WinBytes;
    uint8_t* sImg = sX + (size_t)XS * kC1WBlock;
    const int tid = threadIdx.x, warp = tid >> 5, lane = tid & 31;
    if (tid == 0) {
        for (int s = 0; s < XS; ++s) { mbar_init(&xfull[s], 1); mbar_init(&xempty[s], 12); }
        for (int s = 0; s < WS; ++s) { mbar_init(&wfull[s], 1); mbar_init(&wempty[s], 4); }
        for (int s = 0; s < 2; ++s) { mbar_init(&yfull[s], 1); mbar_init(&yempty[s], 8); }
        fence_barrier_init();
        tma_prefetch_desc(&tmX);
        tma_prefetch_desc(&tmWin);
        tma_prefetch_desc(&tmY);
    }
    for (int idx = tid; idx < 4 * 128 * 8; idx += blockDim.x) {
        const int c16 = idx & 7, r = (idx >> 3) & 127, t = idx >> 10;
        *reinterpret_cast<int4*>(sW2 + t * (128 * 128) + img_off(r, c16)) = ldg16(p.w2dg + r * 256 + t * 64 + c16 * 8);
    }
    for (int idx = tid; idx < 2 * kC21ImgBytes / 16; idx += blockDim.x) reinterpret_cast<int4*>(sImg)[idx] = make_int4(0, 0, 0, 0);
    fence_proxy_async_smem();
    __syncthreads();
    const int64_t M = (int64_t)p.n * 512;
    const int64_t m_begin = (int64_t)blockIdx.x * p.rows_per_cta;
    int64_t m_end = m_begin + p.rows_per_cta;
    if (m_end > M) m_end = M;
    const int nsteps = m_end > m_begin ? (int)((m_end - m_begin) >> 7) : 0;
    const int nimg = nsteps >> 2;
    const int64_t g0 = m_begin >> 7;
    const int img0 = (int)(m_begin >> 9);

    if (warp < 4) {
        setmaxnreg_dec<kC1WRegsProducer>();
        if (warp == 0 && lane == 0 && nsteps > 0) {
            auto image_of = [&](int64_t g) -> int {
                int64_t img = g >> 2;
                if (img >= p.n) img = p.n - 1;
                return p.rows ? (int)__ldg(p.rows + img) : (int)img;
            };
            int z = image_of(g0), z_next = image_of(g0 + 4);
            for (int k = 0; k <= nsteps; ++k) {
                const int64_t g = g0 + k;
                if (k > 0 && (g & 3) == 0) { z = z_next; z_next = image_of(g + 4); }
                const int xs = k % XS;
                if (k >= XS) mbar_wait(&xempty[xs], ((k / XS) - 1) & 1);
                mbar_arrive_expect_tx(&xfull[xs], (uint32_t)kC1WBlock);
                tma_load_3d(smem_u32(sX + (size_t)xs * kC1WBlock), &tmX, (int)(g & 3) * 128, 0, z, &xfull[xs]);
            }
        } else if (warp == 1 && lane == 0) {
            for (int j = 0; j < nimg; ++j) {
                const int s = j % WS;
                if (j >= WS) mbar_wait(&wempty[s], ((j / WS) - 1) & 1);
                mbar_arrive_expect_tx(&wfull[s], (uint32_t)(kC21WinRows * 128));
                tma_load_2d(smem_u32(sWin + (size_t)s * kC21WinBytes), &tmWin, 0, (img0 + j) * 121, &wfull[s]);
            }
        }
    } else if (warp < 8) {
        const int wt = tid - 128, lane4 = lane >> 2, qd = lane & 3;
        const uint32_t w_base = smem_u32(sW2);
        const int rq = wt >> 2, c16 = wt & 3;
        float bsum[8];
#pragma unroll
        for (int e = 0; e < 8; ++e) bsum[e] = 0.f;
        for (int j = 0; j < nimg; ++j) {
            const int i = img0 + j, buf = j & 1, s = j % WS;
            const uint32_t img = smem_u32(sImg + (size_t)buf * kC21ImgBytes) + kC1WYPad;
            mbar_wait(&wfull[s], (j / WS) & 1);
            if (j >= 2) mbar_wait(&yempty[buf], ((j >> 1) - 1) & 1);
            if (wt == 0) bulk_wait_read<1>();
            named_bar(1, 128);
#pragma unroll 1
            for (int h2 = 0; h2 < 2; ++h2) {
                float d[64];
                wgmma_fence();
                const uint32_t win = smem_u32(sWin + (size_t)s * kC21WinBytes) + (uint32_t)(h2 * 64 * 128);
                constexpr int shift[4] = {12, 11, 1, 0};
#pragma unroll
                for (int t = 0; t < 4; ++t) {
                    const uint64_t a = desc_kmajor(win + (uint32_t)shift[t] * 128u);
                    const uint64_t b = desc_kmajor(w_base + (uint32_t)(t * 128 * 128));
#pragma unroll
                    for (int kk = 0; kk < 4; ++kk) WgmmaBf16<128, 0, 0>::mma(d, a + 2 * kk, b + 2 * kk, (t | kk) != 0 ? 1u : 0u);
                }
                wgmma_commit();
                int pos[2];
                uint4 mb[2];
#pragma unroll
                for (int hr = 0; hr < 2; ++hr) {
                    const int r = h2 * 64 + ((wt >> 5) << 4) + lane4 + 8 * hr;
                    const int Y = (r * 5958) >> 16, X = r - Y * 11;
                    const bool valid = Y < 10 && X < 10;
                    pos[hr] = valid ? 2 * Y * 21 + 2 * X : -1;
                    mb[hr] = make_uint4(0u, 0u, 0u, 0u);
                    if (valid) {
                        const int4 t = ldg16(p.m1 + ((int64_t)i * 100 + Y * 10 + X) * 4);
                        mb[hr] = make_uint4((uint32_t)t.x, (uint32_t)t.y, (uint32_t)t.z, (uint32_t)t.w);
                    }
                }
                wgmma_wait<0>();
                wgmma_fence_operands(d);
                if (h2 == 1 && lane == 0) mbar_arrive(&wempty[s]);
#pragma unroll
                for (int hr = 0; hr < 2; ++hr) {
                    if (pos[hr] < 0) continue;
                    const uint32_t mw[4] = {mb[hr].x, mb[hr].y, mb[hr].z, mb[hr].w};
// ... 39 lines not shown
            float t = 0.f;
#pragma unroll
            for (int l = 0; l < 32; ++l) t += sRed[l * 32 + wt];
            p.wsb[(int64_t)blockIdx.x * 64 + wt] = t;
            sBias[wt] = t * kU8Bias;
        }
        named_bar(2, 384);
    } else {
        setmaxnreg_inc<kC1WRegsMma>();
        const int h = (warp - 8) >> 2, wt = tid & 127, qd = lane & 3;
        const int c0 = ((wt >> 5) << 4) + (lane >> 2);
        const bool up = qd >= 2;
        const uint32_t pb = (uint32_t)((2 * qd + h) & 3), psel = pb | ((pb + 1) << 4);
        float d[32];
#pragma unroll
        for (int e = 0; e < 32; ++e) d[e] = 0.f;
        for (int it = 0; it < nsteps; ++it) {
            const int xm = it % XS, xh = (it + 1) % XS, buf = (it >> 2) & 1;
            mbar_wait(&xfull[xm], (it / XS) & 1);
            if (h == 1) mbar_wait(&xfull[xh], ((it + 1) / XS) & 1);
            uint32_t a[8][4];
#pragma unroll
            for (int r = 0; r < 2; ++r) {
                const int c = c0 + 8 * r;
                const uint32_t bm = smem_u32(sX + (size_t)xm * kC1WBlock + c * 128);
                const uint32_t bh = smem_u32(sX + (size_t)xh * kC1WBlock + c * 128);
                const uint32_t sw = (uint32_t)(c & 7);
                uint4 cur = lds128(bm + ((0u ^ sw) << 4));
#pragma unroll
                for (int kk = 0; kk < 8; ++kk) {
                    uint4 nxt = make_uint4(0, 0, 0, 0);
                    if (h == 1) nxt = lds128((kk < 7 ? bm : bh) + ((((uint32_t)(kk + 1) & 7u) ^ sw) << 4));
                    const uint32_t w[5] = {cur.x, cur.y, cur.z, cur.w, nxt.x};
                    a[kk][r] = pair_f16_biased(w, 0, up, psel);
                    a[kk][2 + r] = pair_f16_biased(w, 2, up, psel);
                    if (kk < 7) cur = h == 1 ? nxt : lds128(bm + ((((uint32_t)(kk + 1)) ^ sw) << 4));
                }
            }
            __syncwarp();
            if (lane == 0) {
                mbar_arrive(&xempty[xm]);
                if (h == 1) { mbar_arrive(&xempty[xh]); if (it == 0) mbar_arrive(&xempty[xm]); }
            }
            if ((it & 3) == 0) mbar_wait(&yfull[buf], (it >> 3) & 1);
            wgmma_fence();
            const uint32_t ystep = smem_u32(sImg + (size_t)buf * kC21ImgBytes) + (uint32_t)(kC1WYPad + (it & 3) * kC1WYBytes);
            const uint64_t yd = desc_mnmajor_sw64(ystep - kC1WShift * 64, kC1WShift * 64);
#pragma unroll
            for (int kk = 0; kk < 8; ++kk) wgmma_f16_rs_n64_tb(d, a[kk], yd + 64 * kk, (it | kk) != 0 ? 1u : 0u);
            wgmma_commit();
            wgmma_wait<0>();
            if ((it & 3) == 3 && lane == 0) mbar_arrive(&yempty[buf]);
        }
        wgmma_fence_operands(d);
        named_bar(2, 384);
        float* wsc = p.ws + (int64_t)blockIdx.x * 256 * 64;
#pragma unroll
        for (int b = 0; b < 2; ++b) {
#pragma unroll
            for (int r = 0; r < 2; ++r) {
                float* dst = wsc + (int64_t)((2 * b + h) * 64 + c0 + 8 * r) * 64;
#pragma unroll
                for (int j = 0; j < 4; ++j) {
                    const int co = 8 * j + 2 * qd, e = (b == 0 ? 16 : 0) + 4 * j + 2 * r;
                    *reinterpret_cast<float2*>(dst + co) = make_float2(d[e] - sBias[co], d[e + 1] - sBias[co + 1]);
                }
            }
        }
    }
}

static int launch_conv21_bwd_u8(const Conv21BwdU8Params& p, const void* frames_cm, int64_t n_images, const bf16* dact2b, void* dact1_f16,
                                int ctas, cudaStream_t s, const char* what) {
    const size_t smem = (size_t)kC21W2Bytes + (size_t)kC21WinStages * kC21WinBytes + (size_t)kC1WXStages * kC1WBlock + 2 * (size_t)kC21ImgBytes + 1024;
    int rc;
    if (p.rows_per_cta % 512 != 0) return fail(B200RL_ERR_INVALID_ARGUMENT, "%s: a CTA must own whole images (512 grid rows)", what);
    CUtensorMap tmX, tmWin, tmY;
    memset(&tmX, 0, sizeof(tmX)); memset(&tmWin, 0, sizeof(tmWin)); memset(&tmY, 0, sizeof(tmY));
    if ((rc = make_tmap_3d_u8(&tmX, frames_cm, n_images, 64, 448, 448, 64, 128, what))) return rc;
    if ((rc = make_tmap_2d(&tmWin, dact2b, (int64_t)p.n * 121, 64, kC21WinRows, what))) return rc;
    if ((rc = make_tmap_3d_u8(&tmY, dact1_f16, p.n, 441, 64, 64, 128, 64, what))) return rc;
    static SmemAttrCache attr;
    if ((rc = attr.ensure(tc_conv21_bwd_u8, smem, what))) return rc;
    tc_conv21_bwd_u8<<<ctas, kC1WThreads, smem, s>>>(tmX, tmWin, tmY, p);
    return check_launch(what);
}

constexpr int kConv1I8Stages = 8;
static int launch_conv1_i8(const Conv1U8Params& p, const void* frames_rm, cudaStream_t s, const char* what) {
    constexpr int STAGES = kConv1I8Stages;
    const size_t smem = (size_t)4 * 64 * 64 + (size_t)STAGES * 144 * 128 + 1024;
    const int total = p.n * 2;
    int grid = num_sms();
    if (grid > total) grid = total;
    CUtensorMap tmA;
    memset(&tmA, 0, sizeof(tmA));
    int rc = make_tmap_pairs_u8(&tmA, frames_rm, p.n_images, what);
    if (rc) return rc;
    static SmemAttrCache attr;
    if ((rc = attr.ensure(tc_conv1_i8<STAGES>, smem, what))) return rc;
    tc_conv1_i8<STAGES><<<grid, kConv1I8Threads, smem, s>>>(tmA, p, total);
    return check_launch(what);
}

}
```

### cleanrl_b200/csrc/tc_conv_win.cuh

```cuda
#pragma once
#include "tc_base.cuh"

namespace b200rl {
using namespace tc;

enum { WOUT_DENSE = 0, WOUT_S2D2 = 1, WOUT_DACT2 = 2, WOUT_DACT1 = 3 };
struct WinParams {
    const bf16* A;
    const int64_t* rows;
    int64_t M;
    int n, G, Wp;
    int tpi_shift;
    int64_t n_images;
    int ntaps;
    int shift[16];
    int WR;
    const bf16* Bw;
    int N;
    int vH, vW;
    int out_mode;
    bf16* out;
    bf16* out2;
    const uint32_t* mask_bits;
    uint32_t* mask_out;
// ... 220 lines not shown
    }
}

template <int BN, int CPR, int STAGES, int NTAPS>
static int launch_conv_win(const WinParams& p, cudaStream_t s, const char* what) {
    if (p.ntaps != NTAPS) return fail(B200RL_ERR_INVALID_ARGUMENT, "%s: %d taps, kernel instance has %d", what, p.ntaps, NTAPS);
    if (p.out_mode != WOUT_S2D2 && p.out_mode != WOUT_DACT1)
        return fail(B200RL_ERR_INVALID_ARGUMENT, "%s: dense and conv3 data-gradient outputs run on tc_conv_win_t", what);
    if (p.out_mode == WOUT_DACT1 && (BN != 128 || p.N != 128))
        return fail(B200RL_ERR_INVALID_ARGUMENT, "%s: the conv2 data gradient stores 4 groups of 32 channels per cell", what);
    const size_t smem = (size_t)p.ntaps * CPR * BN * 128 + (size_t)STAGES * p.WR * 128 * CPR + conv_win_acc_bytes<BN>() + 1024;
    static SmemAttrCache attr;
    if (int rc = attr.ensure(tc_conv_win<BN, CPR, STAGES, NTAPS>, smem, what)) return rc;
    if ((int64_t)p.G * p.Wp >= 65536 || p.G < 1 || p.N % 32 != 0)
        return fail(B200RL_ERR_INVALID_ARGUMENT, "%s: grid %d x width %d outside the epilogue's multiply-shift range, or N %% 32 != 0", what, p.G, p.Wp);
    if (p.rows && !p.tpi_shift) return fail(B200RL_ERR_INVALID_ARGUMENT, "%s: the image gather needs image-aligned tiling", what);
    if (p.tpi_shift && (128 << p.tpi_shift) < p.G) return fail(B200RL_ERR_INVALID_ARGUMENT, "%s: tiles per image too small", what);
    const int total = p.tpi_shift ? (int)((int64_t)p.n << p.tpi_shift) : (int)ceil_div(p.M, 128);
    int grid = num_sms();
    if (grid > total) grid = total;
    CUtensorMap tmA;
    memset(&tmA, 0, sizeof(tmA));
    int rc;
    if (p.tpi_shift) rc = make_tmap_3d(&tmA, p.A, p.n_images, p.G, (int64_t)CPR * 64, p.WR, what);
    else rc = make_tmap_2d(&tmA, p.A, p.M, (int64_t)CPR * 64, p.WR, what);
    if (rc) return rc;
    tc_conv_win<BN, CPR, STAGES, NTAPS><<<grid, kConvWinThreads, smem, s>>>(tmA, p, total);
    return check_launch(what);
}

constexpr int kConvWinTThreads = 384;
constexpr int kConvWinTLds = 64 + 4;
template <int BP>
__host__ __device__ constexpr size_t conv_win_t_stage_bytes() { return (size_t)2 * BP * kConvWinTLds * sizeof(float); }

template <int R>
__device__ __forceinline__ void stage_acc_transposed(float* st, int wg_tid, const float (&d)[R]) {
    const int co = ((wg_tid >> 5) << 4) + ((wg_tid & 31) >> 2), pos = (wg_tid & 3) * 2;
#pragma unroll
    for (int j = 0; j < R / 4; ++j) {
        float* p0 = st + (8 * j + pos) * kConvWinTLds + co;
        p0[0] = d[4 * j];
        p0[kConvWinTLds] = d[4 * j + 1];
        p0[8] = d[4 * j + 2];
        p0[kConvWinTLds + 8] = d[4 * j + 3];
    }
}

template <int BP, int CPR, int STAGES, int NTAPS>
__global__ void __launch_bounds__(kConvWinTThreads, 1) tc_conv_win_t(const __grid_constant__ CUtensorMap tmA, const WinParams p,
                                                                     int total_tiles) {
    static_assert(BP % 128 == 0, "one thread per position row of a 128-row slice");
    static_assert(STAGES % 2 == 0, "each consumer warpgroup owns every other stage");
    constexpr int RPT = BP / 128;
    constexpr int A_CHUNK = 64 * 128;
    constexpr int LDS = kConvWinTLds;
    extern __shared__ uint8_t smem_raw[];
    __shared__ uint64_t full_bar[STAGES], empty_bar[STAGES];
    uint8_t* smem = reinterpret_cast<uint8_t*>((reinterpret_cast<uintptr_t>(smem_raw) + 1023) & ~uintptr_t(1023));
    const int tid = threadIdx.x, warp = tid >> 5;
    const int nchunks = NTAPS * CPR;
    const int K = nchunks * 64;
    const int IMG = p.WR * 128;
    const int STAGE_BYTES = IMG * CPR;
    uint8_t* sW = smem;
    uint8_t* sRing = smem + (size_t)nchunks * A_CHUNK;
    float* sAcc = reinterpret_cast<float*>(sRing + (size_t)STAGES * STAGE_BYTES);

    if (tid == 0) {
        for (int s = 0; s < STAGES; ++s) { mbar_init(&full_bar[s], 1); mbar_init(&empty_bar[s], 4); }
        fence_barrier_init();
        tma_prefetch_desc(&tmA);
    }
    for (int idx = tid; idx < nchunks * 64 * 8; idx += blockDim.x) {
        const int c16 = idx & 7;
        const int t = idx >> 3;
        const int r = t & 63, j = t >> 6;
        int4 v = make_int4(0, 0, 0, 0);
        if (r < p.N) v = ldg16(p.Bw + (int64_t)r * K + j * 64 + c16 * 8);
        *reinterpret_cast<int4*>(sW + (size_t)j * A_CHUNK + img_off(r, c16)) = v;
    }
    fence_proxy_async_smem();
    __syncthreads();
    const int tile_begin = (int)(((int64_t)total_tiles * blockIdx.x) / gridDim.x);
    const int tile_end = (int)(((int64_t)total_tiles * (blockIdx.x + 1)) / gridDim.x);

    if (warp == 0) {
        if (tid == 0) {
            uint32_t q = 0;
            for (int tile = tile_begin; tile < tile_end; ++tile, ++q) {
                const uint32_t s = q % STAGES;
                if (q >= (uint32_t)STAGES) mbar_wait(&empty_bar[s], ((q / STAGES) - 1) & 1);
                const uint32_t dst = smem_u32(sRing + (size_t)s * STAGE_BYTES);
                mbar_arrive_expect_tx(&full_bar[s], (uint32_t)STAGE_BYTES);
#pragma unroll
                for (int c = 0; c < CPR; ++c) tma_load_2d(dst + c * IMG, &tmA, c * 64, tile * BP, &full_bar[s]);
            }
        }
    } else if (warp >= 4) {
        const int wg = (warp - 4) >> 2, wt = tid & 127;
        float* st = sAcc + wg * BP * LDS;
        const uint32_t w_base = smem_u32(sW);
        const uint32_t mW = (65536u + (uint32_t)p.Wp - 1u) / (uint32_t)p.Wp;
        constexpr int NW = 2;
        float d[BP / 2];
#pragma unroll
        for (int e = 0; e < BP / 2; ++e) d[e] = 0.f;
        for (int tile = tile_begin + wg; tile < tile_end; tile += 2) {
            const uint32_t q = (uint32_t)(tile - tile_begin), s = q % STAGES;
            mbar_wait(&full_bar[s], (q / STAGES) & 1);
            wgmma_fence();
            const uint32_t win = smem_u32(sRing + (size_t)s * STAGE_BYTES);
#pragma unroll
            for (int t = 0; t < NTAPS; ++t) {
#pragma unroll
                for (int c = 0; c < CPR; ++c) {
                    const uint64_t b = desc_kmajor(win + (uint32_t)(c * IMG) + (uint32_t)p.shift[t] * 128u);
                    const uint64_t a = desc_kmajor(w_base + (uint32_t)((t * CPR + c) * A_CHUNK));
#pragma unroll
                    for (int kk = 0; kk < 4; ++kk)
                        WgmmaBf16<BP, 0, 0>::mma(d, a + 2 * kk, b + 2 * kk, (t | c | kk) != 0 ? 1u : 0u);
                }
            }
            wgmma_commit();
            bool valid[RPT];
            int64_t o1[RPT], o2[RPT], ob[RPT];
            uint32_t mb[RPT][NW];
#pragma unroll
            for (int rr = 0; rr < RPT; ++rr) {
                const int64_t r = (int64_t)tile * BP + rr * 128 + wt;
                const int i = (int)(r / p.G);
                const int rem = (int)(r - (int64_t)i * p.G);
                const int Y = (int)(((uint32_t)rem * mW) >> 16), X = rem - Y * p.Wp;
                valid[rr] = r < p.M && (Y < p.vH) && (X < p.vW);
                o2[rr] = 0;
                if (p.out_mode == WOUT_DENSE) {
                    const int64_t orow = ((int64_t)i * p.vH + Y) * p.vW + X;
                    o1[rr] = orow * p.N; ob[rr] = orow * (p.N >> 5);
                } else {
                    o1[rr] = ((int64_t)i * 100 + Y * 10 + X) * 64;
                    o2[rr] = ((int64_t)i * 121 + (Y + 1) * 11 + (X + 1)) * 64;
                    ob[rr] = ((int64_t)i * 81 + Y * 9 + X) * 2;
                }
                mb[rr][0] = mb[rr][1] = 0xFFFFFFFFu;
                if (p.mask_bits != nullptr && valid[rr]) {
                    const uint2 t = __ldg(reinterpret_cast<const uint2*>(p.mask_bits + ob[rr]));
                    mb[rr][0] = t.x; mb[rr][1] = t.y;
                }
            }
            wgmma_wait<0>();
            wgmma_fence_operands(d);
            if ((tid & 31) == 0) mbar_arrive(&empty_bar[s]);
            named_bar(1 + wg, 128);
            stage_acc_transposed(st, wt, d);
            named_bar(1 + wg, 128);
#pragma unroll
            for (int rr = 0; rr < RPT; ++rr) {
                float* srow = st + (rr * 128 + wt) * LDS;
#pragma unroll
                for (int g = 0; g < NW; ++g) {
                    if (!valid[rr] || g * 32 >= p.N) continue;
                    uint32_t v[32];
#pragma unroll
                    for (int e = 0; e < 8; ++e) {
                        const float4 f = *reinterpret_cast<const float4*>(srow + g * 32 + 4 * e);
                        v[4 * e] = __float_as_uint(f.x); v[4 * e + 1] = __float_as_uint(f.y);
// ... 4 lines not shown
#pragma unroll
                        for (int e = 0; e < 8; ++e) {
                            const float4 bv = __ldg(bp + e);
                            v[4 * e] = __float_as_uint(fmaf(__uint_as_float(v[4 * e]), p.scale, bv.x));
                            v[4 * e + 1] = __float_as_uint(fmaf(__uint_as_float(v[4 * e + 1]), p.scale, bv.y));
                            v[4 * e + 2] = __float_as_uint(fmaf(__uint_as_float(v[4 * e + 2]), p.scale, bv.z));
                            v[4 * e + 3] = __float_as_uint(fmaf(__uint_as_float(v[4 * e + 3]), p.scale, bv.w));
                        }
                    } else {
#pragma unroll
                        for (int e = 0; e < 32; ++e) v[e] = __float_as_uint(__uint_as_float(v[e]) * p.scale);
                    }
                    if (p.relu) {
                        uint32_t bits = 0u;
#pragma unroll
                        for (int e = 0; e < 32; ++e) bits |= (__uint_as_float(v[e]) > 0.f ? 1u : 0u) << e;
                        if (p.mask_out) p.mask_out[ob[rr] + g] = bits;
                    }
                    if (p.mask_bits) {
#pragma unroll
                        for (int e = 0; e < 32; ++e) if (!((mb[rr][g] >> e) & 1u)) v[e] = 0u;
                    }
                    int4 w[4];
                    if (p.relu) {
#pragma unroll
                        for (int e = 0; e < 4; ++e) {
                            w[e].x = (int)pack_bf16x2_relu(__uint_as_float(v[8 * e]), __uint_as_float(v[8 * e + 1]));
                            w[e].y = (int)pack_bf16x2_relu(__uint_as_float(v[8 * e + 2]), __uint_as_float(v[8 * e + 3]));
                            w[e].z = (int)pack_bf16x2_relu(__uint_as_float(v[8 * e + 4]), __uint_as_float(v[8 * e + 5]));
                            w[e].w = (int)pack_bf16x2_relu(__uint_as_float(v[8 * e + 6]), __uint_as_float(v[8 * e + 7]));
                        }
                    } else {
#pragma unroll
                        for (int e = 0; e < 4; ++e) {
                            w[e].x = (int)pack_bf16x2(__uint_as_float(v[8 * e]), __uint_as_float(v[8 * e + 1]));
                            w[e].y = (int)pack_bf16x2(__uint_as_float(v[8 * e + 2]), __uint_as_float(v[8 * e + 3]));
                            w[e].z = (int)pack_bf16x2(__uint_as_float(v[8 * e + 4]), __uint_as_float(v[8 * e + 5]));
                            w[e].w = (int)pack_bf16x2(__uint_as_float(v[8 * e + 6]), __uint_as_float(v[8 * e + 7]));
                        }
                    }
                    int4* brow = reinterpret_cast<int4*>(srow) + 4 * g;
#pragma unroll
                    for (int e = 0; e < 4; ++e) brow[e] = w[e];
                }
                *reinterpret_cast<longlong2*>(srow + 64) = make_longlong2(valid[rr] ? o1[rr] : -1, o2[rr]);
            }
            named_bar(1 + wg, 128);
#pragma unroll
            for (int m = 0; m < BP / 16; ++m) {
                const int k = m * 128 + wt, part = k & 7;
                const float* srow = st + (k >> 3) * LDS;
                const longlong2 off = *reinterpret_cast<const longlong2*>(srow + 64);
                if (off.x < 0) continue;
                const int4 val = reinterpret_cast<const int4*>(srow)[part];
                *reinterpret_cast<int4*>(p.out + off.x + part * 8) = val;
                if (p.out_mode == WOUT_DACT2) *reinterpret_cast<int4*>(p.out2 + off.y + part * 8) = val;
            }
        }
    }
}

template <int BP, int CPR, int STAGES, int NTAPS>
static int launch_conv_win_t(WinParams p, cudaStream_t s, const char* what) {
    if (p.ntaps != NTAPS) return fail(B200RL_ERR_INVALID_ARGUMENT, "%s: %d taps, kernel instance has %d", what, p.ntaps, NTAPS);
    if (p.N != 64) return fail(B200RL_ERR_INVALID_ARGUMENT, "%s: N = %d, the kernel computes 64 output channels", what, p.N);
    if ((int64_t)p.G * p.Wp >= 65536 || p.G < 1)
        return fail(B200RL_ERR_INVALID_ARGUMENT, "%s: grid %d x width %d outside the epilogue's multiply-shift range", what, p.G, p.Wp);
    if (p.rows || p.tpi_shift) return fail(B200RL_ERR_INVALID_ARGUMENT, "%s: the channel-major kernel walks a contiguous linear grid", what);
    if (p.out_mode != WOUT_DENSE && p.out_mode != WOUT_DACT2)
        return fail(B200RL_ERR_INVALID_ARGUMENT, "%s: only bf16 dense and conv3 data-gradient outputs in this kernel", what);
    int maxs = 0;
    for (int t = 0; t < NTAPS; ++t) maxs = p.shift[t] > maxs ? p.shift[t] : maxs;
    p.WR = (BP + maxs + 7) & ~7;
    if (p.WR > 256) return fail(B200RL_ERR_INVALID_ARGUMENT, "%s: window of %d rows exceeds a TMA box", what, p.WR);
    const size_t smem = (size_t)NTAPS * CPR * 64 * 128 + (size_t)STAGES * p.WR * 128 * CPR + conv_win_t_stage_bytes<BP>() + 1024;
    static SmemAttrCache attr;
    if (int rc = attr.ensure(tc_conv_win_t<BP, CPR, STAGES, NTAPS>, smem, what)) return rc;
    const int total = (int)ceil_div(p.M, BP);
    int grid = num_sms();
    if (grid > total) grid = total;
    CUtensorMap tmA;
    memset(&tmA, 0, sizeof(tmA));
    if (int rc = make_tmap_2d(&tmA, p.A, p.M, (int64_t)CPR * 64, p.WR, what)) return rc;
    tc_conv_win_t<BP, CPR, STAGES, NTAPS><<<grid, kConvWinTThreads, smem, s>>>(tmA, p, total);
    return check_launch(what);
}

}
```

### cleanrl_b200/csrc/tc_gemm_tma.cuh

```cuda
#pragma once
#include "tc_base.cuh"

namespace b200rl {
using namespace tc;

struct KGemmParams {
    const void* A;
    int64_t M;
    int nchunks;
    const bf16* Bw;
    int N;
    bf16* out;
    int ldo;
    const float* bias;
    float scale;
    int relu;
    const uint32_t* mask_bits;
    uint32_t* mask_out;
    int dual_dact3;
    bf16* out2;
    float* out_f32;
    int ncols_f32;
};

constexpr int kGemmThreads = 384;
template <int BN>
__host__ __device__ constexpr size_t gemm_acc_bytes() { return (size_t)128 * (BN + 4) * sizeof(float); }
template <int BN, int STAGES>
__global__ void __launch_bounds__(kGemmThreads, 1) tc_gemm_tma(const __grid_constant__ CUtensorMap tmA,
                                                               const __grid_constant__ CUtensorMap tmB,
                                                               const KGemmParams p, int total_tiles, int ntiles_n) {
    constexpr int A_BYTES = 128 * 128;
    constexpr int B_BYTES = BN * 128;
    constexpr int STAGE_BYTES = A_BYTES + B_BYTES;
    constexpr int LDA = BN + 4;
    extern __shared__ uint8_t smem_raw[];
    __shared__ uint64_t full_bar[STAGES], empty_bar[STAGES];
    uint8_t* smem = reinterpret_cast<uint8_t*>((reinterpret_cast<uintptr_t>(smem_raw) + 1023) & ~uintptr_t(1023));
    float* sAcc = reinterpret_cast<float*>(smem + (size_t)STAGES * STAGE_BYTES);
    const int tid = threadIdx.x, warp = tid >> 5;
    const int nch = p.nchunks;
    if (tid == 0) {
        for (int s = 0; s < STAGES; ++s) { mbar_init(&full_bar[s], 1); mbar_init(&empty_bar[s], 256); }
        fence_barrier_init();
        tma_prefetch_desc(&tmA);
        tma_prefetch_desc(&tmB);
    }
    __syncthreads();

    if (warp == 0) {
        if ((tid & 31) == 0) {
            uint32_t q = 0;
            for (int tile = blockIdx.x; tile < total_tiles; tile += gridDim.x) {
                const int mt = tile / ntiles_n, n0 = (tile - mt * ntiles_n) * BN;
                for (int j = 0; j < nch; ++j, ++q) {
                    const uint32_t s = q % STAGES;
                    if (q >= (uint32_t)STAGES) mbar_wait(&empty_bar[s], ((q / STAGES) - 1) & 1);
                    const uint32_t dst = smem_u32(smem + (size_t)s * STAGE_BYTES);
                    mbar_arrive_expect_tx(&full_bar[s], STAGE_BYTES);
                    tma_load_2d(dst, &tmA, j * 64, mt * 128, &full_bar[s]);
                    tma_load_2d(dst + A_BYTES, &tmB, j * 64, n0, &full_bar[s]);
                }
            }
        }
    } else if (warp >= 4) {
        const int wg = (warp - 4) >> 2, wt = tid & 127;
        float* st = sAcc + wg * 64 * LDA;
        const int lr = wt & 63, half = wt >> 6;
        const int nwords = p.N >> 5;
        constexpr int NW = BN / 32;
        float d[BN / 2];
#pragma unroll
        for (int e = 0; e < BN / 2; ++e) d[e] = 0.f;
        uint32_t q = 0;
        for (int tile = blockIdx.x; tile < total_tiles; tile += gridDim.x) {
            const int mt = tile / ntiles_n, n0 = (tile - mt * ntiles_n) * BN;
            for (int j = 0; j < nch; ++j, ++q) {
                const uint32_t s = q % STAGES;
                mbar_wait(&full_bar[s], (q / STAGES) & 1);
                wgmma_fence();
                const uint32_t stage_addr = smem_u32(smem + (size_t)s * STAGE_BYTES);
                const uint64_t a = desc_kmajor(stage_addr + wg * 64 * 128), b = desc_kmajor(stage_addr + A_BYTES);
#pragma unroll
                for (int kk = 0; kk < 4; ++kk) WgmmaBf16<BN, 0, 0>::mma(d, a + 2 * kk, b + 2 * kk, (j | kk) != 0 ? 1u : 0u);
                wgmma_commit();
                wgmma_wait<0>();
                mbar_arrive(&empty_bar[s]);
            }
            wgmma_fence_operands(d);
            const int r = mt * 128 + wg * 64 + lr;
            const bool rvalid = r < (int)p.M;
            const int64_t wb = (int64_t)r * nwords + (n0 >> 5);
            named_bar(1 + wg, 128);
            stage_acc(st, LDA, wt, d);
            named_bar(1 + wg, 128);
#pragma unroll
            for (int g = 0; g < NW; ++g) {
                const int col = n0 + g * 32;
                if (!rvalid || (g & 1) != half || col >= p.N) continue;
                uint32_t v[32];
#pragma unroll
                for (int e = 0; e < 8; ++e) {
                    const float4 f = *reinterpret_cast<const float4*>(st + lr * LDA + g * 32 + 4 * e);
                    v[4 * e] = __float_as_uint(f.x); v[4 * e + 1] = __float_as_uint(f.y);
                    v[4 * e + 2] = __float_as_uint(f.z); v[4 * e + 3] = __float_as_uint(f.w);
                }
                const uint32_t mbw = p.mask_bits != nullptr ? __ldg(p.mask_bits + wb + g) : 0xFFFFFFFFu;
                if (p.bias) {
                    const float4* bp = reinterpret_cast<const float4*>(p.bias + col);
#pragma unroll
                    for (int e = 0; e < 8; ++e) {
                        const float4 bv = __ldg(bp + e);
                        v[4 * e] = __float_as_uint(fmaf(__uint_as_float(v[4 * e]), p.scale, bv.x));
                        v[4 * e + 1] = __float_as_uint(fmaf(__uint_as_float(v[4 * e + 1]), p.scale, bv.y));
                        v[4 * e + 2] = __float_as_uint(fmaf(__uint_as_float(v[4 * e + 2]), p.scale, bv.z));
                        v[4 * e + 3] = __float_as_uint(fmaf(__uint_as_float(v[4 * e + 3]), p.scale, bv.w));
                    }
                } else {
#pragma unroll
                    for (int e = 0; e < 32; ++e) v[e] = __float_as_uint(__uint_as_float(v[e]) * p.scale);
                }
                if (p.relu) {
                    uint32_t bits = 0u;
#pragma unroll
                    for (int e = 0; e < 32; ++e) {
                        const bool pos = __uint_as_float(v[e]) > 0.f;
                        bits |= (pos ? 1u : 0u) << e;
                        v[e] = pos ? v[e] : 0u;
                    }
                    if (p.mask_out) p.mask_out[wb + g] = bits;
                }
                if (p.mask_bits) {
#pragma unroll
                    for (int e = 0; e < 32; ++e) if (!((mbw >> e) & 1u)) v[e] = 0u;
                }
                if (p.out_f32) {
                    float* dst = p.out_f32 + (int64_t)r * p.ldo + col;
#pragma unroll
                    for (int e = 0; e < 32; ++e) if (col + e < p.ncols_f32) dst[e] = __uint_as_float(v[e]);
                    continue;
                }
                int4 w[4];
#pragma unroll
                for (int e = 0; e < 4; ++e) {
                    w[e].x = (int)pack_bf16x2(__uint_as_float(v[8 * e]), __uint_as_float(v[8 * e + 1]));
                    w[e].y = (int)pack_bf16x2(__uint_as_float(v[8 * e + 2]), __uint_as_float(v[8 * e + 3]));
                    w[e].z = (int)pack_bf16x2(__uint_as_float(v[8 * e + 4]), __uint_as_float(v[8 * e + 5]));
                    w[e].w = (int)pack_bf16x2(__uint_as_float(v[8 * e + 6]), __uint_as_float(v[8 * e + 7]));
                }
                if (p.dual_dact3) {
                    const int px = col >> 6;
                    const int oy = px / 7, ox = px - oy * 7;
                    bf16* dst = p.out + ((int64_t)r * 81 + oy * 9 + ox) * 64 + (g & 1) * 32;
                    bf16* dst2 = p.out2 + ((int64_t)r * 121 + (oy + 2) * 11 + ox + 2) * 64 + (g & 1) * 32;
                    st_global_32b(dst, w[0], w[1]); st_global_32b(dst + 16, w[2], w[3]);
                    st_global_32b(dst2, w[0], w[1]); st_global_32b(dst2 + 16, w[2], w[3]);
                } else {
                    bf16* dst = p.out + (int64_t)r * p.ldo + col;
                    st_global_32b(dst, w[0], w[1]); st_global_32b(dst + 16, w[2], w[3]);
                }
            }
        }
    }
}

constexpr int kWgradTmaThreads = 384;
constexpr int kFcWgradXChunks = 2, kFcWgradYChunks = 4;
static __global__ void __launch_bounds__(kWgradTmaThreads, 1) tc_wgrad_tma(const __grid_constant__ CUtensorMap tmX,
                                                                    const __grid_constant__ CUtensorMap tmY,
                                                                    int64_t M, int64_t rows_per_cta, float* ws) {
    constexpr int R = 64, STAGES = 4, nxc = kFcWgradXChunks, nyc = kFcWgradYChunks, NY = 64 * nyc;
    extern __shared__ uint8_t smem_raw[];
    __shared__ uint64_t full_bar[STAGES], empty_bar[STAGES];
    uint8_t* smem = reinterpret_cast<uint8_t*>((reinterpret_cast<uintptr_t>(smem_raw) + 1023) & ~uintptr_t(1023));
    const int tid = threadIdx.x, warp = tid >> 5;
    const int xc0 = blockIdx.y * nxc, yc0 = blockIdx.z * nyc;
    constexpr int chunk_img = R * 128;
    constexpr int stage_bytes = (nxc + nyc) * chunk_img;
    if (tid == 0) {
        for (int s = 0; s < STAGES; ++s) { mbar_init(&full_bar[s], 1); mbar_init(&empty_bar[s], 8); }
        fence_barrier_init();
        tma_prefetch_desc(&tmX);
        tma_prefetch_desc(&tmY);
    }
    __syncthreads();
    const int64_t m_begin = (int64_t)blockIdx.x * rows_per_cta;
    int64_t m_end = m_begin + rows_per_cta;
    if (m_end > M) m_end = M;
    const int nsteps = m_end > m_begin ? (int)((m_end - m_begin + R - 1) / R) : 0;

    if (warp == 0 && (tid & 31) == 0) {
        for (int it = 0; it < nsteps; ++it) {
            const int s = it % STAGES;
            if (it >= STAGES) mbar_wait(&empty_bar[s], ((it / STAGES) - 1) & 1);
            const uint32_t dst = smem_u32(smem + (size_t)s * stage_bytes);
            const int m0 = (int)(m_begin + (int64_t)it * R);
            mbar_arrive_expect_tx(&full_bar[s], (uint32_t)stage_bytes);
            for (int c = 0; c < nxc; ++c) tma_load_2d(dst + c * chunk_img, &tmX, (xc0 + c) * 64, m0, &full_bar[s]);
            for (int c = 0; c < nyc; ++c) tma_load_2d(dst + (nxc + c) * chunk_img, &tmY, (yc0 + c) * 64, m0, &full_bar[s]);
        }
    } else if (warp >= 4) {
        const int wg = (warp - 4) >> 2, wt = tid & 127;
        float d[NY / 2];
#pragma unroll
        for (int e = 0; e < NY / 2; ++e) d[e] = 0.f;
        for (int it = 0; it < nsteps; ++it) {
            const int s = it % STAGES;
            mbar_wait(&full_bar[s], (it / STAGES) & 1);
            wgmma_fence();
            const uint32_t xa = smem_u32(smem + (size_t)s * stage_bytes), ya = xa + nxc * chunk_img;
#pragma unroll
            for (int kk = 0; kk < R / 16; ++kk) {
                const uint64_t adesc = desc_mnmajor(xa + wg * chunk_img + kk * 2048, chunk_img);
                const uint64_t bdesc = desc_mnmajor(ya + kk * 2048, chunk_img);
                WgmmaBf16<NY, 1, 1>::mma(d, adesc, bdesc, (it | kk) != 0 ? 1u : 0u);
            }
            wgmma_commit();
            wgmma_wait<0>();
            if ((tid & 31) == 0) mbar_arrive(&empty_bar[s]);
        }
        wgmma_fence_operands(d);
        const int64_t NYtot = (int64_t)gridDim.z * nyc * 64;
        const int64_t KXtot = (int64_t)gridDim.y * nxc * 64;
        float* wsb = ws + (int64_t)blockIdx.x * KXtot * NYtot;
        const int row = ((wt >> 5) << 4) + ((wt & 31) >> 2), col = (wt & 3) * 2;
        float* d0 = wsb + ((int64_t)xc0 * 64 + wg * 64 + row) * NYtot + (int64_t)yc0 * 64 + col;
        float* d8 = d0 + 8 * NYtot;
#pragma unroll
        for (int j = 0; j < NY / 8; ++j) {
            *reinterpret_cast<float2*>(d0 + 8 * j) = make_float2(d[4 * j], d[4 * j + 1]);
            *reinterpret_cast<float2*>(d8 + 8 * j) = make_float2(d[4 * j + 2], d[4 * j + 3]);
        }
    }
}

template <int BN, int STAGES>
static int launch_gemm_tma(const KGemmParams& p, cudaStream_t s, const char* what) {
    const size_t smem = (size_t)STAGES * (128 * 128 + BN * 128) + gemm_acc_bytes<BN>() + 1024;
    static SmemAttrCache attr;
    int rc;
    if (p.N % 64 != 0 || BN % 64 != 0) return fail(B200RL_ERR_INVALID_ARGUMENT, "%s: N must be a multiple of 64", what);
    if ((rc = attr.ensure(tc_gemm_tma<BN, STAGES>, smem, what))) return rc;
    CUtensorMap tmA, tmB;
    const int64_t K = (int64_t)p.nchunks * 64;
    if ((rc = make_tmap_2d(&tmA, p.A, p.M, K, 128, what))) return rc;
    if ((rc = make_tmap_2d(&tmB, p.Bw, p.N, K, BN, what))) return rc;
    const int ntn = (int)ceil_div(p.N, BN);
    const int total = (int)ceil_div(p.M, 128) * ntn;
    int grid = num_sms();
    if (grid > total) grid = total;
    tc_gemm_tma<BN, STAGES><<<grid, kGemmThreads, smem, s>>>(tmA, tmB, p, total, ntn);
    return check_launch(what);
}

static int64_t round_up(int64_t a, int64_t b) { return ceil_div(a, b) * b; }
struct WPlan { int64_t rows_per_cta; int splits; };
static WPlan wgrad_plan(int64_t M, int target_ctas, int quantum = 32) {
    WPlan w;
    w.rows_per_cta = round_up(ceil_div(M, target_ctas), quantum);
    if (w.rows_per_cta < quantum) w.rows_per_cta = quantum;
    w.splits = (int)ceil_div(M, w.rows_per_cta);
    if (w.splits < 1) w.splits = 1;
    return w;
}
constexpr int kFcSplits = 8;

static size_t wgrad_tma_bytes(int64_t M, int xcols, int ycols) {
    return (size_t)wgrad_plan(M, kFcSplits, 64).splits * xcols * round_up(ycols, 64 * kFcWgradYChunks) * sizeof(float);
}
static int launch_wgrad_tma(const void* X, int xcols, const void* Y, int ycols, int64_t M, float* ws, cudaStream_t s,
                            const char* what) {
    if (xcols % (64 * kFcWgradXChunks) != 0) return fail(B200RL_ERR_INVALID_ARGUMENT, "%s: X columns must be a multiple of 128", what);
    const WPlan pl = wgrad_plan(M, kFcSplits, 64);
    CUtensorMap tmX, tmY;
    int rc;
    if ((rc = make_tmap_2d(&tmX, X, M, xcols, 64, what))) return rc;
    if ((rc = make_tmap_2d(&tmY, Y, M, ycols, 64, what))) return rc;
    const size_t smem = (size_t)4 * (kFcWgradXChunks + kFcWgradYChunks) * 64 * 128 + 1024;
    static SmemAttrCache attr;
    if ((rc = attr.ensure(tc_wgrad_tma, smem, what))) return rc;
    const dim3 grid(pl.splits, xcols / (64 * kFcWgradXChunks), (unsigned)ceil_div(ycols, 64 * kFcWgradYChunks));
    tc_wgrad_tma<<<grid, kWgradTmaThreads, smem, s>>>(tmX, tmY, M, pl.rows_per_cta, ws);
    if ((rc = check_launch(what))) return rc;
    return pl.splits;
}

}
```

### cleanrl_b200/csrc/tc_heads.cuh

```cuda
#pragma once
#include "tc_base.cuh"
#include "tc_reduce.cuh"

namespace b200rl {
using namespace tc;

constexpr int kMaxHeads = 24;
constexpr int kHeadsPartialBlocks = 264;
static inline int64_t heads_rows_per_block(int64_t n) {
    int64_t rpb = (n + kHeadsPartialBlocks - 1) / kHeadsPartialBlocks;
    if (rpb < 16) rpb = 16;
    if (rpb > 256) rpb = 256;
    return rpb;
}

template <int HT = 512>
__global__ void __launch_bounds__(256) tc_heads_fwd(const bf16* __restrict__ hid, const float* __restrict__ Wh,
                                                    const float* __restrict__ bh, int64_t n, int A1, int H,
                                                    float* __restrict__ out) {
    constexpr int NQ = (HT + 255) / 256;
    extern __shared__ float sW[];
    for (int i = threadIdx.x; i < A1 * HT; i += blockDim.x) sW[i] = Wh[i];
    __syncthreads();
    const int lane = threadIdx.x & 31, wpb = blockDim.x >> 5;
    for (int64_t row = (int64_t)blockIdx.x * wpb + (threadIdx.x >> 5); row < n; row += (int64_t)gridDim.x * wpb) {
        float hv[8 * NQ];
        const bf16* hp = hid + row * HT;
#pragma unroll
        for (int q = 0; q < NQ; ++q) {
            const bool own = HT % 256 == 0 || lane * 8 < HT;
            const int4 v = own ? ldg16(hp + q * 256 + lane * 8) : make_int4(0, 0, 0, 0);
            const uint32_t w[4] = {(uint32_t)v.x, (uint32_t)v.y, (uint32_t)v.z, (uint32_t)v.w};
#pragma unroll
            for (int e = 0; e < 4; ++e) {
                hv[q * 8 + 2 * e] = __uint_as_float(w[e] << 16);
                hv[q * 8 + 2 * e + 1] = __uint_as_float(w[e] & 0xFFFF0000u);
            }
        }
        float mine = 0.f;
        for (int a = 0; a < A1; ++a) {
            float s = 0.f;
#pragma unroll
            for (int q = 0; q < NQ; ++q) {
                if (HT % 256 != 0 && lane * 8 >= HT) continue;
                const float4 w0 = *reinterpret_cast<const float4*>(sW + a * HT + q * 256 + lane * 8);
                const float4 w1 = *reinterpret_cast<const float4*>(sW + a * HT + q * 256 + lane * 8 + 4);
                s = fmaf(hv[q * 8 + 0], w0.x, s); s = fmaf(hv[q * 8 + 1], w0.y, s);
                s = fmaf(hv[q * 8 + 2], w0.z, s); s = fmaf(hv[q * 8 + 3], w0.w, s);
                s = fmaf(hv[q * 8 + 4], w1.x, s); s = fmaf(hv[q * 8 + 5], w1.y, s);
                s = fmaf(hv[q * 8 + 6], w1.z, s); s = fmaf(hv[q * 8 + 7], w1.w, s);
            }
            s = warp_sum(s);
            if (lane == a) mine = s + bh[a];
        }
        if (lane < A1) out[row * A1 + lane] = mine;
    }
}
template <int HT = 512>
__global__ void __launch_bounds__(256) tc_heads_bwd_data(const float* __restrict__ dhead, const float* __restrict__ Wh,
                                                         const uint8_t* __restrict__ hid_bits, int64_t n, int A1, int H,
                                                         bf16* __restrict__ dhid) {
    constexpr int G = HT / 8;
    extern __shared__ float sWt[];
    for (int i = threadIdx.x; i < A1 * HT; i += blockDim.x) {
        const int a = i / HT, h = i % HT;
        sWt[a * HT + (h & 7) * G + (h >> 3)] = Wh[i];
    }
    __syncthreads();
    const int64_t total = n * G;
    for (int64_t idx = (int64_t)blockIdx.x * blockDim.x + threadIdx.x; idx < total; idx += (int64_t)gridDim.x * blockDim.x) {
        const int64_t row = idx / G;
        const int g = (int)(idx % G);
        const uint32_t m = hid_bits[idx];
        float o[8];
#pragma unroll
        for (int e = 0; e < 8; ++e) o[e] = 0.f;
        for (int a = 0; a < A1; ++a) {
            const float d = __ldg(dhead + row * A1 + a);
#pragma unroll
            for (int e = 0; e < 8; ++e) o[e] = fmaf(d, sWt[a * HT + e * G + g], o[e]);
        }
#pragma unroll
        for (int e = 0; e < 8; ++e) if (!((m >> e) & 1u)) o[e] = 0.f;
        int4 w;
        w.x = (int)pack_bf16x2(o[0], o[1]); w.y = (int)pack_bf16x2(o[2], o[3]);
        w.z = (int)pack_bf16x2(o[4], o[5]); w.w = (int)pack_bf16x2(o[6], o[7]);
        *reinterpret_cast<int4*>(dhid + row * HT + g * 8) = w;
    }
}
template <int MAXA, int HT = 512>
__global__ void __launch_bounds__(512) tc_heads_bwd_weight(const float* __restrict__ dhead, const bf16* __restrict__ hid,
                                                           int64_t n, int A1, int H, int64_t rows_per_block,
                                                           float* __restrict__ part) {
    extern __shared__ float sD[];
    const int hp = threadIdx.x % (HT / 2), rl = threadIdx.x / (HT / 2);
    const int64_t r0 = (int64_t)blockIdx.x * rows_per_block;
    int64_t r1 = r0 + rows_per_block;
    if (r1 > n) r1 = n;
    const int nrows = (int)(r1 > r0 ? r1 - r0 : 0);
    for (int i = threadIdx.x; i < nrows * A1; i += blockDim.x) sD[i] = dhead[r0 * A1 + i];
    __syncthreads();
    float acc0[MAXA], acc1[MAXA], bacc[MAXA];
#pragma unroll
    for (int a = 0; a < MAXA; ++a) { acc0[a] = 0.f; acc1[a] = 0.f; bacc[a] = 0.f; }
    const uint32_t* h2 = reinterpret_cast<const uint32_t*>(hid);
    int r = rl;
    for (; r + 14 < nrows; r += 16) {
        uint32_t hv[8];
#pragma unroll
        for (int u = 0; u < 8; ++u) hv[u] = __ldg(h2 + (r0 + r + 2 * u) * (HT / 2) + hp);
#pragma unroll
        for (int u = 0; u < 8; ++u) {
            const float x0 = __uint_as_float(hv[u] << 16), x1 = __uint_as_float(hv[u] & 0xFFFF0000u);
            const float* dr = sD + (r + 2 * u) * A1;
#pragma unroll
            for (int a = 0; a < MAXA; ++a) {
                if (a < A1) {
                    const float d = dr[a];
                    acc0[a] = fmaf(d, x0, acc0[a]); acc1[a] = fmaf(d, x1, acc1[a]); bacc[a] += d;
                }
            }
        }
    }
    for (; r < nrows; r += 2) {
        const uint32_t hv = __ldg(h2 + (r0 + r) * (HT / 2) + hp);
        const float x0 = __uint_as_float(hv << 16), x1 = __uint_as_float(hv & 0xFFFF0000u);
        const float* dr = sD + r * A1;
#pragma unroll
        for (int a = 0; a < MAXA; ++a) {
            if (a < A1) {
                const float d = dr[a];
                acc0[a] = fmaf(d, x0, acc0[a]); acc1[a] = fmaf(d, x1, acc1[a]); bacc[a] += d;
            }
        }
    }
    float* pb = part + ((int64_t)blockIdx.x * 2 + rl) * A1 * (H + 2);
#pragma unroll
    for (int a = 0; a < MAXA; ++a) {
        if (a < A1) {
            *reinterpret_cast<float2*>(pb + (int64_t)a * (H + 2) + 2 * hp) = make_float2(acc0[a], acc1[a]);
            if (hp == 0) pb[(int64_t)a * (H + 2) + H] = bacc[a];
        }
    }
}
static __global__ void __launch_bounds__(256) tc_heads_fold(const float* __restrict__ part, int nslabs, int A1, int H,
                                                     float* __restrict__ dW, float* __restrict__ db) {
    __shared__ float red[256];
    const int idx = blockIdx.x * 32 + (threadIdx.x & 31);
    const int a = idx / (H + 2), h = idx - a * (H + 2);
    const bool valid = a < A1 && h <= H;
    const float s = zlane_sum(part, (int64_t)A1 * (H + 2), nslabs, idx, valid, red);
    if (!valid || threadIdx.x >= 32) return;
    if (h == H) db[a] = s; else dW[(int64_t)a * H + h] = s;
}

template <int H>
static int heads_fwd(const bf16* hid, const float* Wh, const float* bh, int64_t n, int A1, float* out, cudaStream_t s,
                     const char* what) {
    static_assert(H == 128 || H == 256 || H == 512, "head input width");
    const int grid = (int)(ceil_div(n, 8) < (int64_t)num_sms() * 8 ? ceil_div(n, 8) : (int64_t)num_sms() * 8);
    tc_heads_fwd<H><<<grid, 256, (size_t)A1 * H * sizeof(float), s>>>(hid, Wh, bh, n, A1, H, out);
    return check_launch(what);
}
static size_t heads_partial_bytes(int64_t n, int A1, int H) {
    return (size_t)2 * ceil_div(n, heads_rows_per_block(n)) * A1 * (H + 2) * sizeof(float);
}
template <int H>
static int heads_bwd_weight(const float* dhead, const bf16* hid, int64_t n, int A1, float* part, float* dW, float* db,
                            cudaStream_t s, const char* what) {
    static_assert(H == 128 || H == 256 || H == 512, "head input width");
    const int64_t rpb = heads_rows_per_block(n);
    const int nb = (int)ceil_div(n, rpb);
    const size_t sd = (size_t)rpb * A1 * sizeof(float);
    if (A1 <= 8) tc_heads_bwd_weight<8, H><<<nb, H, sd, s>>>(dhead, hid, n, A1, H, rpb, part);
    else tc_heads_bwd_weight<kMaxHeads, H><<<nb, H, sd, s>>>(dhead, hid, n, A1, H, rpb, part);
    tc_heads_fold<<<(unsigned)ceil_div(A1 * (H + 2), 32), 256, 0, s>>>(part, 2 * nb, A1, H, dW, db);
    return check_launch(what, 2);
}
template <int H>
static int heads_bwd_data(const float* dhead, const float* Wh, const uint8_t* hid_bits, int64_t n, int A1, bf16* dhid,
                          cudaStream_t s, const char* what) {
    static_assert(H == 128 || H == 256 || H == 512, "head input width");
    const int grid = (int)(ceil_div(n * H, 2048) < (int64_t)num_sms() * 8 ? ceil_div(n * H, 2048) : (int64_t)num_sms() * 8);
    tc_heads_bwd_data<H><<<grid, 256, (size_t)A1 * H * sizeof(float), s>>>(dhead, Wh, hid_bits, n, A1, H, dhid);
    return check_launch(what);
}

}
```

### cleanrl_b200/csrc/tc_reduce.cuh

```cuda
#pragma once
#include "tc_base.cuh"
#include "tc_wgrad_win.cuh"

namespace b200rl {
using namespace tc;

__device__ __forceinline__ float zlane_sum(const float* __restrict__ part, int64_t slab, int nslabs, int64_t idx, bool valid,
                                           float* red ) {
    const int zl = threadIdx.x >> 5, ol = threadIdx.x & 31;
    float s = 0.f;
    if (valid) {
        int z = zl;
        for (; z + 24 < nslabs; z += 32) {
            const float v0 = part[(int64_t)z * slab + idx], v1 = part[(int64_t)(z + 8) * slab + idx];
            const float v2 = part[(int64_t)(z + 16) * slab + idx], v3 = part[(int64_t)(z + 24) * slab + idx];
            s += v0; s += v1; s += v2; s += v3;
        }
        for (; z < nslabs; z += 8) s += part[(int64_t)z * slab + idx];
    }
    red[threadIdx.x] = s;
    __syncthreads();
    float t = 0.f;
    if (zl == 0) {
#pragma unroll
        for (int l = 0; l < 8; ++l) t += red[l * 32 + ol];
    }
    return t;
}

struct FoldWin { int layer, S, nslots, Cout; int slot_tap[16], slot_cc[16], slot_skip[16]; float scale;
                 float bscale;
                 const float* wsb; float* db; };
static __global__ void __launch_bounds__(256) tc_fold_win(const float* __restrict__ ws, const FoldWin f, float* __restrict__ dst) {
    __shared__ float red[256];
    const int idx = blockIdx.x * 32 + (threadIdx.x & 31);
    const int KX = f.nslots * 64;
    if (idx >= KX * f.Cout) {
        const int co = idx - KX * f.Cout;
        const bool valid = co < f.Cout && f.db != nullptr;
        const float s = zlane_sum(f.wsb, 64, f.S, co, valid, red);
        if (valid && threadIdx.x < 32) f.db[co] = s * f.bscale;
        return;
    }
    const int xi = idx / f.Cout, co = idx - xi * f.Cout;
    const int slot = xi >> 6, row = xi & 63;
    const bool valid = !f.slot_skip[slot];
    float s = zlane_sum(ws, (int64_t)KX * 64, f.S, (int64_t)xi * 64 + co, valid, red);
    if (!valid || threadIdx.x >= 32) return;
    s *= f.scale;
    const int tap = f.slot_tap[slot];
    int64_t o;
    if (f.layer == 1) {
        const int c = row >> 4, sy = (row >> 2) & 3, sx = row & 3;
        o = (((int64_t)co * 4 + c) * 8 + ((tap >> 1) * 4 + sy)) * 8 + (tap & 1) * 4 + sx;
    } else if (f.layer == 2) {
        const int q = f.slot_cc[slot] * 64 + row;
        const int g = q >> 5, c = q & 31;
        o = (((int64_t)co * 32 + c) * 4 + (2 * (tap >> 1) + (g >> 1))) * 4 + 2 * (tap & 1) + (g & 1);
    } else {
        o = ((int64_t)co * 64 + row) * 9 + tap;
    }
    dst[o] = s;
}

static __global__ void tc_fold_fc(const float* __restrict__ ws, int S, int KX, int NY, int validX, int validY,
                           int C, int KK, float scale, float* __restrict__ dst) {
    const int64_t idx = (int64_t)blockIdx.x * blockDim.x + threadIdx.x;
    const int64_t total = (int64_t)validX * validY;
    if (idx >= total) return;
    const int xi = (int)(idx / validY), yi = (int)(idx - (int64_t)xi * validY);
    float s = 0.f;
    const int64_t slab = (int64_t)KX * NY;
    for (int z = 0; z < S; ++z) s += ws[z * slab + (int64_t)xi * NY + yi];
    const int pp = yi / C, c = yi - pp * C;
    dst[(int64_t)xi * validY + (int64_t)c * KK + pp] = s * scale;
}

static __global__ void __launch_bounds__(256) tc_colsum_partial(const bf16* __restrict__ Y, int64_t M, int ld, int ncols,
                                                         int64_t rows_per_block, float* __restrict__ part) {
    __shared__ float red[256 * 8];
    const int cg = ncols >> 3;
    const int lanes = 256 / cg;
    const int tx = threadIdx.x % cg, ty = threadIdx.x / cg;
    const int64_t r0 = (int64_t)blockIdx.x * rows_per_block;
    int64_t r1 = r0 + rows_per_block;
    if (r1 > M) r1 = M;
    float acc[8];
#pragma unroll
    for (int e = 0; e < 8; ++e) acc[e] = 0.f;
    if (ty < lanes) {
        for (int64_t r = r0 + ty; r < r1; r += lanes) {
            const int4 v = ldg16(Y + r * ld + tx * 8);
            const uint32_t w[4] = {(uint32_t)v.x, (uint32_t)v.y, (uint32_t)v.z, (uint32_t)v.w};
#pragma unroll
            for (int e = 0; e < 4; ++e) {
                acc[2 * e] += __uint_as_float(w[e] << 16);
                acc[2 * e + 1] += __uint_as_float(w[e] & 0xFFFF0000u);
            }
        }
    }
#pragma unroll
    for (int e = 0; e < 8; ++e) red[threadIdx.x * 8 + e] = acc[e];
    __syncthreads();
    for (int c = threadIdx.x; c < ncols; c += blockDim.x) {
        const int g = c >> 3, e = c & 7;
        float s = 0.f;
        for (int l = 0; l < lanes; ++l) s += red[(l * cg + g) * 8 + e];
        part[(int64_t)blockIdx.x * ncols + c] = s;
    }
}
static __global__ void __launch_bounds__(256) tc_colsum_final(const float* __restrict__ part, int nblocks, int ncols,
                                                       float* __restrict__ db) {
    __shared__ float red[256];
    const int c = blockIdx.x * 32 + (threadIdx.x & 31);
    const float s = zlane_sum(part, ncols, nblocks, c, c < ncols, red);
    if (c < ncols && threadIdx.x < 32) db[c] = s;
}

static int64_t colsum_rows(int64_t M) {
    const int64_t rpb = ceil_div(M, 132 * 3);
    return rpb < 64 ? 64 : rpb;
}
static int colsum(const bf16* Y, int64_t M, int ld, int ncols, float* part, float* db, cudaStream_t s) {
    const int64_t rpb = colsum_rows(M);
    const int nb = (int)ceil_div(M, rpb);
    tc_colsum_partial<<<nb, 256, 0, s>>>(Y, M, ld, ncols, rpb, part);
    tc_colsum_final<<<(unsigned)ceil_div(ncols, 32), 256, 0, s>>>(part, nb, ncols, db);
    return check_launch("colsum", 2);
}
static size_t colsum_ws(int64_t M, int ncols) { return (size_t)ceil_div(M, colsum_rows(M)) * ncols * sizeof(float); }

}
```

### cleanrl_b200/csrc/tc_wgrad_win.cuh

```cuda
#pragma once
#include "tc_base.cuh"

namespace b200rl {
using namespace tc;

constexpr int kWgradWinStages = 3;
struct WGradWinParams {
    const bf16* X; const int64_t* rows; int64_t M; int n, G;
    int tpi_shift;
    int64_t n_images;
    int cpr;
    int nslots;
    int slot_tap[16], slot_cc[16];
    int shift[16];
    int WRX;
    const bf16* Y; int ldy, ncolsY;
    int64_t rows_per_cta;
    float* ws;
    float* wsb;
};

constexpr int kWgradWinThreads = 512;
constexpr int kWgradWinTilesPerCta = 2;

template <int NT>
__device__ __forceinline__ void wgrad_win_mma(const WGradWinParams& p, uint8_t* smem, int stage_bytes, int XBYTES, int IMGX,
                                              uint64_t* full_bar, uint64_t* empty_bar, int nsteps, int t0, int w, int tid) {
    constexpr int R = 128, STAGES = kWgradWinStages, NY = 64;
    const int wt = tid & 127;
    uint32_t arel[NT];
#pragma unroll
    for (int tt = 0; tt < NT; ++tt) {
        const int slot = 2 * (t0 + tt) + w;
        arel[tt] = (uint32_t)(p.slot_cc[slot] * IMGX + p.shift[p.slot_tap[slot]] * 128);
    }
    float d[NT][NY / 2];
#pragma unroll
    for (int tt = 0; tt < NT; ++tt)
#pragma unroll
        for (int e = 0; e < NY / 2; ++e) d[tt][e] = 0.f;
    auto step = [&](int it) {
        const int s = it % STAGES;
        mbar_wait(&full_bar[s], (it / STAGES) & 1);
        wgmma_fence();
        const uint32_t xa = smem_u32(smem + (size_t)s * stage_bytes), ya = xa + XBYTES;
        const uint64_t yd = desc_mnmajor(ya, 0);
#pragma unroll
        for (int tt = 0; tt < NT; ++tt) {
            const uint64_t xd = desc_mnmajor(xa + arel[tt], 0);
#pragma unroll
            for (int kk = 0; kk < R / 16; ++kk)
                WgmmaBf16<NY, 1, 1>::mma(d[tt], xd + kk * 128, yd + kk * 128, (it | kk) != 0 ? 1u : 0u);
        }
        wgmma_commit();
    };
    for (int it = 0; it + 1 < nsteps; ++it) {
        step(it);
        wgmma_wait<1>();
        if (it > 0 && (tid & 31) == 0) mbar_arrive(&empty_bar[(it - 1) % STAGES]);
    }
    step(nsteps - 1);
    wgmma_wait<0>();
    const int row = ((wt >> 5) << 4) + ((wt & 31) >> 2), col = (wt & 3) * 2;
    float* wsb = p.ws + (int64_t)blockIdx.y * (p.nslots * 64) * NY;
#pragma unroll
    for (int tt = 0; tt < NT; ++tt) {
        wgmma_fence_operands(d[tt]);
        float* d0 = wsb + (int64_t)((2 * (t0 + tt) + w) * 64 + row) * NY + col;
#pragma unroll
        for (int j = 0; j < NY / 8; ++j) {
            *reinterpret_cast<float2*>(d0 + 8 * j) = make_float2(d[tt][4 * j], d[tt][4 * j + 1]);
            *reinterpret_cast<float2*>(d0 + 8 * NY + 8 * j) = make_float2(d[tt][4 * j + 2], d[tt][4 * j + 3]);
        }
    }
}

static __global__ void __launch_bounds__(kWgradWinThreads, 1) tc_wgrad_win(const __grid_constant__ CUtensorMap tmX, const __grid_constant__ CUtensorMap tmY,
                                                       const WGradWinParams p, int use_tma) {
    constexpr int R = 128, STAGES = kWgradWinStages, LOOKAHEAD = 1, NY = 64, TT = kWgradWinTilesPerCta;
    static_assert(TT == 2, "the wgmma warpgroups dispatch on 1 or 2 tiles per CTA");
    extern __shared__ uint8_t smem_raw[];
    __shared__ uint64_t full_bar[STAGES], empty_bar[STAGES];
    uint8_t* smem = reinterpret_cast<uint8_t*>((reinterpret_cast<uintptr_t>(smem_raw) + 1023) & ~uintptr_t(1023));
    const int tid = threadIdx.x, warp = tid >> 5;
    const int IMGX = p.WRX * 128;
    const int XBYTES = IMGX * p.cpr;
    const int stage_bytes = XBYTES + R * 128;
    const int xt = p.nslots / 2;
    const int t0 = blockIdx.x * TT;
    float* sRed = reinterpret_cast<float*>(smem + (size_t)STAGES * stage_bytes);
    if (tid == 0) {
        for (int s = 0; s < STAGES; ++s) { mbar_init(&full_bar[s], use_tma ? 1 : 5); mbar_init(&empty_bar[s], (use_tma ? 4 : 0) + 8); }
        fence_barrier_init();
        tma_prefetch_desc(&tmX);
        if (use_tma) tma_prefetch_desc(&tmY);
    }
    __syncthreads();
    const int64_t m_begin = (int64_t)blockIdx.y * p.rows_per_cta;
    int64_t m_end = m_begin + p.rows_per_cta;
    if (m_end > p.M) m_end = p.M;
    const int nsteps = m_end > m_begin ? (int)((m_end - m_begin + R - 1) / R) : 0;
    const int tmask = (1 << p.tpi_shift) - 1;
    const int64_t g0 = m_begin / R;

    if (warp == 4) {
        if ((tid & 31) == 0) {
            int z_next = 0;
            if (!use_tma && nsteps > 0) {
                const int64_t img = g0 >> p.tpi_shift;
                z_next = p.rows ? (int)__ldg(p.rows + (img < p.n ? img : 0)) : (int)img;
            }
            for (int it = 0; it < nsteps; ++it) {
                const int s = it % STAGES;
                const int z = z_next;
                if (!use_tma && it + 1 < nsteps) {
                    const int64_t img1 = (g0 + it + 1) >> p.tpi_shift;
                    z_next = p.rows ? (int)__ldg(p.rows + (img1 < p.n ? img1 : 0)) : (int)img1;
                }
                if (it >= STAGES) mbar_wait(&empty_bar[s], ((it / STAGES) - 1) & 1);
                const uint32_t dst = smem_u32(smem + (size_t)s * stage_bytes);
                if (use_tma) {
                    const int m0 = (int)(m_begin + (int64_t)it * R);
                    mbar_arrive_expect_tx(&full_bar[s], (uint32_t)stage_bytes);
                    for (int c = 0; c < p.cpr; ++c) tma_load_2d(dst + c * IMGX, &tmX, c * 64, m0, &full_bar[s]);
                    tma_load_2d(dst + XBYTES, &tmY, 0, m0, &full_bar[s]);
                } else {
                    const int t_in = (int)((g0 + it) & tmask);
                    mbar_arrive_expect_tx(&full_bar[s], (uint32_t)XBYTES);
                    for (int c = 0; c < p.cpr; ++c) tma_load_3d(dst + c * IMGX, &tmX, c * 64, t_in * 128, z, &full_bar[s]);
                }
            }
        }
    } else if (warp < 4) {
        const int rq = tid >> 3, c16 = tid & 7;
        float bsum[8];
#pragma unroll
        for (int e = 0; e < 8; ++e) bsum[e] = 0.f;
        auto add_step = [&](const uint8_t* sYp) {
#pragma unroll
            for (int ps = 0; ps < R / 16; ++ps) {
                const int rr = ps * 16 + rq;
                const int4 v = *reinterpret_cast<const int4*>(sYp + img_off(rr, c16));
                const uint32_t w[4] = {(uint32_t)v.x, (uint32_t)v.y, (uint32_t)v.z, (uint32_t)v.w};
#pragma unroll
                for (int e = 0; e < 4; ++e) {
                    bsum[2 * e] += __uint_as_float(w[e] << 16);
                    bsum[2 * e + 1] += __uint_as_float(w[e] & 0xFFFF0000u);
                }
            }
        };
        if (use_tma) {
            for (int it = 0; it < nsteps; ++it) {
                const int s = it % STAGES;
                mbar_wait(&full_bar[s], (it / STAGES) & 1);
                add_step(smem + (size_t)s * stage_bytes + XBYTES);
                __syncwarp();
                if ((tid & 31) == 0) mbar_arrive(&empty_bar[s]);
            }
        } else {
            for (int it = 0; it < nsteps; ++it) {
                const int s = it % STAGES;
                const int64_t g = g0 + it;
                const int64_t img = g >> p.tpi_shift;
                const int t_in = (int)(g & tmask);
                if (it >= STAGES) mbar_wait(&empty_bar[s], ((it / STAGES) - 1) & 1);
                const uint32_t sY = smem_u32(smem + (size_t)s * stage_bytes + XBYTES);
#pragma unroll
                for (int ps = 0; ps < R / 16; ++ps) {
                    const int rr = ps * 16 + rq;
                    const int rl = t_in * 128 + rr;
                    const int col = c16 * 8;
                    const bool ok = rl < p.G && img < p.n && col < p.ncolsY;
                    cp_async16(sY + img_off(rr, c16), p.Y + (ok ? (img * p.G + rl) * (int64_t)p.ldy + col : 0), ok ? 16u : 0u);
                }
                cp_async_commit();
                if (it >= LOOKAHEAD) {
                    cp_async_wait<LOOKAHEAD>();
                    const int sd = (it - LOOKAHEAD) % STAGES;
                    add_step(smem + (size_t)sd * stage_bytes + XBYTES);
                    fence_proxy_async_smem();
// ... 30 lines not shown
```

### cleanrl_b200/ppo_engine.py

```python
from __future__ import annotations

import os
import time

import numpy as np
import torch

from . import ops

STAT_NAMES = ops.STAT_NAMES


def _torch_dtype(np_dtype):
    return torch.uint8 if np.dtype(np_dtype) == np.uint8 else torch.float32


def _pin(t):
    return t.pin_memory() if torch.cuda.is_available() else t


def _sync():
    if torch.cuda.is_available():
        torch.cuda.current_stream().synchronize()

# ... 50 lines not shown
        self.next_done = torch.zeros(N, dtype=f32, device=device)
        self.next_value = torch.zeros(N, dtype=f32, device=device)
        self.rewards_h = _pin(torch.zeros((T, N), dtype=f32))
        self.dones_h = _pin(torch.zeros((T, N), dtype=f32))
        self.next_done_h = _pin(torch.zeros(N, dtype=f32))
        self.actions_h = _pin(torch.zeros_like(self.actions[0], device="cpu"))
        self.obs_stage_h = _pin(torch.zeros((N,) + tuple(obs_shape), dtype=self.obs_dtype))
        E = int(args.update_epochs)
        self.b_inds_h = _pin(torch.zeros((E, self.B), dtype=torch.int64))
        self.b_inds = torch.zeros((E, self.B), dtype=torch.int64, device=device)
        n_upd = int(args.update_epochs) * self.num_minibatches
        self.stats = torch.zeros(max(n_upd, 1), 16, dtype=f32, device=device)
        self.stats_h = _pin(torch.zeros(max(n_upd, 1), 16, dtype=f32))
        self.grad_norm = torch.zeros(1, dtype=f32, device=device)
        self.update_graphs = os.environ.get("CLEANRL_B200_UPDATE_GRAPHS", "1") != "0"
        self.host_seconds = {"shuffle": 0.0, "update_enqueue": 0.0, "update_wait": 0.0}
        self._shuffle = (ops.numpy_global_shuffle if device.type == "cuda" and os.environ.get("CLEANRL_B200_NATIVE_SHUFFLE", "1") != "0"
                         else np.random.shuffle)
        self._upd_graphs, self._upd_kernels, self._upd_iters = {}, {}, 0
        self.hyper = torch.zeros(max(n_upd, 1), 2, dtype=f32, device=device)
        self.hyper_h = _pin(torch.zeros(max(n_upd, 1), 2, dtype=f32))
        self.flat = agent.flat
        if self.overlap_exchange:
            agent.grad_tail()
        if cuda_graphs is None:
            cuda_graphs = os.environ.get("CLEANRL_B200_CUDA_GRAPHS", "1") != "0"
        self.cuda_graphs = bool(cuda_graphs) and device.type == "cuda"
        chunks = int(os.environ.get("CLEANRL_B200_H2D_CHUNKS", "4"))
        self.h2d_chunks = chunks if (self.cuda_graphs and getattr(self, "s2d", False) and chunks > 1
                                     and N % chunks == 0 and N // chunks >= 128) else 1
        C = self.h2d_chunks
        if C == 4 and N % 16 == 0:
            sizes = [5 * N // 16, 5 * N // 16, 4 * N // 16, 2 * N // 16]
        else:
            sizes = [N // C] * C
        self.chunk_bounds = [(sum(sizes[:c]), sum(sizes[:c + 1])) for c in range(C)]
        self.noise_buf = None
        if self.h2d_chunks > 1:
            self.copy_stream = torch.cuda.Stream(device=device)
            self.chunk_events = [torch.cuda.Event() for _ in range(self.h2d_chunks)]
            self.noise_buf = torch.zeros(agent.noise_shape(N), dtype=f32, device=device)
        self._parts = None
        want_delta = os.environ.get("CLEANRL_B200_DELTA_UPLOAD")
        if want_delta is None:
            want_delta = "1" if int(os.environ.get("LOCAL_WORLD_SIZE", "1") or 1) <= 1 else "0"
        self.delta_upload = bool(getattr(self, "u8_rollout", False)) and want_delta != "0"
        self._delta_allowed = self.delta_upload
        self._delta = None
        self.delta_redos = 0
        self.delta_full_frames = 0
        self._graphs = {}
        self._graph_pool = None
        self._graph_kernels = {}
        self._graph_warm = set()
        self.graph_launches = 0
        self.h2d_bytes = 0
        self.d2h_bytes = 0
        self.kernel_launches = 0

    def _to_storage(self, src_u8, step, sl=slice(None)):
        dst = self.next_obs if step is None else self.obs[step]
        if self.u8_rollout:
            dst_t = self.next_obs_t if step is None else self.obs_t[step]
            ops.frames_to_s2d_u8(src_u8, dst[sl], dst_t[sl])
        else:
            ops.frames_to_s2d(src_u8, out=dst[sl])

    def _upload_obs(self, step, obs_np, convert=True):
        dst = self.next_obs if step is None else self.obs[step]
        src = torch.from_numpy(np.ascontiguousarray(obs_np))
        if src.dtype != self.obs_dtype:
            src = src.to(self.obs_dtype)
        if not src.is_pinned():
            self.obs_stage_h.copy_(src)
            src = self.obs_stage_h
        if self.s2d:
            self.obs_u8.copy_(src, non_blocking=True)
            if convert:
                self._to_storage(self.obs_u8, step)
        else:
            dst.copy_(src, non_blocking=True)
        self.h2d_bytes += src.numel() * src.element_size()

    def _step_device_work(self, step, noise=None):
        if self.s2d:
            self._to_storage(self.obs_u8, step)
        self.agent.sample_into(self.obs[step], self.actions[step], self.logprobs[step], self.values[step], noise=noise)

    def _chunk_device_work(self, step, c):
        sl = slice(*self.chunk_bounds[c])
        self._to_storage(self.obs_u8[sl], step, sl)
        self.agent.sample_into(self.obs[step][sl], self.actions[step][sl], self.logprobs[step][sl],
                               self.values[step][sl], noise=self.noise_buf[sl])

    def _run_step(self, step, chunk=None):
        if chunk is not None:
            work, key = (lambda: self._chunk_device_work(step, chunk)), (step, chunk)
            return self._run_graphed(work, key, warm_key=("c", chunk))
        if self._graphable() and not getattr(self.agent.noise_fn, "graph_safe", False):
            if self.noise_buf is None:
                self.noise_buf = torch.zeros(self.agent.noise_shape(self.N), dtype=torch.float32, device=self.device)
            self.agent.draw_noise_into(self.noise_buf)
            return self._run_graphed(lambda: self._step_device_work(step, noise=self.noise_buf), step, warm_key=("f", 0))
        return self._run_graphed(lambda: self._step_device_work(step), step, warm_key=("f", 0))

    def _graphable(self):
        return self.cuda_graphs and self.agent.graph_capturable

    def _run_graphed(self, work, key, warm_key):
        if not self._graphable():
            return work()
        if self.agent.uses_tc_plan():
            self.agent._tc_plan()
        g = self._graphs.get(key)
        if g is None:
            if warm_key not in self._graph_warm:
                rng = torch.cuda.get_rng_state(self.device)
                work()
                torch.cuda.current_stream().synchronize()
                torch.cuda.set_rng_state(rng, self.device)
                self._graph_warm.add(warm_key)
            from . import _lib
            l0 = _lib.load().b200rl_launch_count()
            g = torch.cuda.CUDAGraph()
            if self._graph_pool is None:
                self._graph_pool = torch.cuda.graph_pool_handle()
            with torch.cuda.graph(g, pool=self._graph_pool):
                work()
            self._graphs[key] = g
            self.agent.pin_workspaces()
            self._graph_kernels[key] = _lib.load().b200rl_launch_count() - l0
        g.replay()
        self.graph_launches += self._graph_kernels[key]

    @torch.no_grad()
    def policy_step(self, step, next_obs_np, next_done_np):
        if self.h2d_chunks > 1 and self._graphable():
            self._pipelined_step(step, next_obs_np)
            self.dones_h[step].copy_(torch.as_tensor(np.asarray(next_done_np, dtype=np.float32)))
        else:
            self.dones_h[step].copy_(torch.as_tensor(np.asarray(next_done_np, dtype=np.float32)))
            self._upload_obs(step, next_obs_np, convert=False)
            self._run_step(step)
        self.actions_h.copy_(self.actions[step], non_blocking=True)
        self.d2h_bytes += self.actions_h.numel() * self.actions_h.element_size()
        _sync()
        return self.actions_h.numpy()

    def _pipelined_step(self, step, obs_np):
        src = torch.from_numpy(np.ascontiguousarray(obs_np))
        if not src.is_pinned():
            self.obs_stage_h.copy_(src)
            src = self.obs_stage_h
        C = self.h2d_chunks
        main = torch.cuda.current_stream()
        with torch.cuda.stream(self.copy_stream):
            for c, (lo, hi) in enumerate(self.chunk_bounds):
                self.obs_u8[lo:hi].copy_(src[lo:hi], non_blocking=True)
                self.chunk_events[c].record(self.copy_stream)
        self.h2d_bytes += src.numel()
        self.agent.draw_noise_into(self.noise_buf)
        for c in range(C):
            main.wait_event(self.chunk_events[c])
            self._run_step(step, chunk=c)

    @torch.no_grad()
    def policy_step_resident(self, step, obs_dev, done_dev=None):
        if self.s2d and obs_dev.dtype == torch.uint8:
            self.obs_u8.copy_(obs_dev)
        else:
            self.obs[step].copy_(obs_dev)
        self._run_step(step)

    @torch.no_grad()
    def rollout_resident(self, obs_pool):
        P = obs_pool.shape[0]

        def work():
            for step in range(self.T):
                src = obs_pool[step % P]
                if self.s2d and src.dtype == torch.uint8:
                    self._to_storage(src, step)
                else:
                    self.obs[step].copy_(src)
                self.agent.sample_into(self.obs[step], self.actions[step], self.logprobs[step], self.values[step])

        if not self.agent.graph_friendly:
            return work()
        self._run_graphed(work, ("rollout", obs_pool.data_ptr(), P), warm_key="r")

    def _part_setup(self, P):
        if getattr(self, "_parts", None) is not None and len(self._parts) == P:
            return
        N = self.N
        assert N % P == 0, "num_envs must be divisible by the number of env groups"
        n = N // P
        self._parts = [(p * n, (p + 1) * n) for p in range(P)]
        C = 2 if (n % 2 == 0 and n // 2 >= 64 and self.s2d and self._graphable()) else 1
        want = os.environ.get("CLEANRL_B200_PART_CHUNKS")
        if want and self.s2d and self._graphable() and 1 <= int(want) <= 4 and n % int(want) == 0:
            C = int(want)
        self._part_chunks = [[(lo + c * (n // C), lo + (c + 1) * (n // C)) for c in range(C)] for lo, hi in self._parts]
        if getattr(self, "copy_stream", None) is None:
            self.copy_stream = torch.cuda.Stream(device=self.device)
        self._part_h2d = [[torch.cuda.Event() for _ in ch] for ch in self._part_chunks]
        self._part_d2h = [torch.cuda.Event() for _ in range(P)]
        if self.noise_buf is None:
            self.noise_buf = torch.zeros(self.agent.noise_shape(N), dtype=torch.float32, device=self.device)
        if not hasattr(self, "obs_u8"):
            self.obs_u8 = None
        self._noise_bufs = [self.noise_buf, torch.zeros_like(self.noise_buf)]
        self._noise_step = -1
        self._actions_np = self.actions_h.numpy()
        self._rewards_np, self._dones_np = self.rewards_h.numpy(), self.dones_h.numpy()
        self._dones_ptr = self.dones_h.data_ptr()
        self._part_d2h_bytes = n * self.actions_h.element_size() * max(1, self.act_dim)
        self._part_d2h_handles = [None] * P
        self._plans, self._plan_refs, self._plan_kernels, self._plan_stream = {}, {}, {}, None
        if self.device.type == "cuda":
            from . import _lib
            self._lib = _lib.load()
        self._delta = None
        if self._delta_allowed and self._graphable():
            u8 = torch.uint8
            self._delta = [dict(tr=ops.StackDeltaTracker(n), full_d=torch.zeros((n, 28224), dtype=u8, device=self.device),
                                last=None, boot_obs=None, consumed=torch.cuda.Event()) for _ in range(P)]
            self._new_d = torch.zeros((N, 7056), dtype=u8, device=self.device)
            self._slot_d = torch.zeros(N, dtype=torch.int32, device=self.device)
            self._mis_ptr = [d["tr"].mis_h.data_ptr() for d in self._delta]

    def _part_work(self, step, lo, hi):
        sl = slice(lo, hi)
        if self.s2d:
            self._to_storage(self.obs_u8[sl], step, sl)
        self.agent.sample_into(self.obs[step][sl], self.actions[step][sl], self.logprobs[step][sl], self.values[step][sl],
                               noise=self._noise_bufs[step & 1][sl])

    @torch.no_grad()
    def launch_part(self, step, part, obs_np, done_np):
        if self._delta is not None and self.delta_upload:
            return self._launch_part_delta(step, part, obs_np, done_np)
        lo, hi = self._parts[part]
        src = torch.from_numpy(np.ascontiguousarray(obs_np))
        if src.dtype != self.obs_dtype:
            src = src.to(self.obs_dtype)
        if not src.is_pinned():
            self.obs_stage_h[lo:hi].copy_(src)
            src = self.obs_stage_h[lo:hi]
        main = torch.cuda.current_stream()
        dst = self.obs_u8 if self.s2d else self.obs[step]
        with torch.cuda.stream(self.copy_stream):
            for c, (clo, chi) in enumerate(self._part_chunks[part]):
                dst[clo:chi].copy_(src[clo - lo:chi - lo], non_blocking=True)
                self._part_h2d[part][c].record(self.copy_stream)
        self.h2d_bytes += src.numel() * src.element_size()
        self.dones_h[step][lo:hi].copy_(torch.as_tensor(np.asarray(done_np, dtype=np.float32)))
        if part == 0:
            self._ensure_noise(step)
        for c, (clo, chi) in enumerate(self._part_chunks[part]):
            main.wait_event(self._part_h2d[part][c])
            self._run_graphed(lambda: self._part_work(step, clo, chi), ("part", step, part, c), warm_key=("p", part, c))
        self.actions_h[lo:hi].copy_(self.actions[step][lo:hi], non_blocking=True)
        self._part_d2h[part].record(main)
        self.d2h_bytes += (hi - lo) * self.actions_h.element_size() * max(1, self.act_dim)

    def wait_actions(self, part):
        lo, hi = self._parts[part]
        if self._delta is not None:
# ... 406 lines not shown
```

Baseline: 1.109 million.

## Launch kernels with programmatic dependent launch and pre-draw rollout noise

Adds a launch_pdl helper that uses cudaLaunchKernelEx with programmatic stream serialization, and converts many small kernels (folds, colsum, heads, sampling, loss, Adam, packing, frame conversion, wgrad) to it, with griddepcontrol wait/launch_dependents in each kernel. The aim is to hide launch latency and prologue time between the back-to-back small kernels on the stream. Separately, noise for sampling is drawn into buffers ahead of time, per step or for the whole rollout, when the noise function supports in-place draws. Each kernel calls wait at or near its start, so the overlap is limited to launch and setup. The in-place noise path also changes how randomness is generated.

```diff
diff --git a/cleanrl_b200/csrc/common.cuh b/cleanrl_b200/csrc/common.cuh
--- a/cleanrl_b200/csrc/common.cuh
+++ b/cleanrl_b200/csrc/common.cuh
@@ -16,6 +16,24 @@
     cudaError_t e = cudaGetLastError();
     if (e != cudaSuccess) return fail(B200RL_ERR_CUDA, "%s: %s", what, cudaGetErrorString(e));
     return B200RL_OK;
+}
+
+__device__ __forceinline__ void pdl_wait() { asm volatile("griddepcontrol.wait;" ::: "memory"); }
+__device__ __forceinline__ void pdl_launch_dependents() { asm volatile("griddepcontrol.launch_dependents;" ::: "memory"); }
+
+template <typename... KArgs, typename... Args>
+inline int launch_pdl(const char* what, void (*kernel)(KArgs...), dim3 grid, dim3 block, size_t smem, cudaStream_t s,
+                      Args&&... args) {
+    cudaLaunchAttribute attr[1];
+    attr[0].id = cudaLaunchAttributeProgrammaticStreamSerialization;
+    attr[0].val.programmaticStreamSerializationAllowed = 1;
+    cudaLaunchConfig_t cfg = {};
+    cfg.gridDim = grid; cfg.blockDim = block; cfg.dynamicSmemBytes = smem; cfg.stream = s;
+    cfg.attrs = attr; cfg.numAttrs = 1;
+    const cudaError_t e = cudaLaunchKernelEx(&cfg, kernel, static_cast<Args&&>(args)...);
+    const int rc = check_launch(what);
+    if (rc == B200RL_OK && e != cudaSuccess) return fail(B200RL_ERR_CUDA, "%s: %s", what, cudaGetErrorString(e));
+    return rc;
 }
 
 #define B200RL_REQUIRE(cond, ...) \
diff --git a/cleanrl_b200/csrc/net_tc.cu b/cleanrl_b200/csrc/net_tc.cu
--- a/cleanrl_b200/csrc/net_tc.cu
+++ b/cleanrl_b200/csrc/net_tc.cu
@@ -158,8 +158,7 @@
         if ((rc = make_tmap_3d(&tmX, p.X, p.n_images, p.G, (int64_t)p.cpr * 64, p.WRX, what))) return rc;
     }
     const dim3 grid((unsigned)ceil_div(p.nslots / 2, kWgradWinTilesPerCta), ctas);
-    tc_wgrad_win<<<grid, kWgradWinThreads, smem, s>>>(tmX, tmY, p, use_tma);
-    return check_launch(what);
+    return launch_pdl(what, tc_wgrad_win, grid, kWgradWinThreads, smem, s, tmX, tmY, p, use_tma);
 }
 
 }
@@ -206,7 +205,8 @@
         { ProfScope ps(s, "fc_wgrad", 2.0 * n * 512 * 3136, (double)n * (3136 + 512) * 2 + 512.0 * 3136 * 4);
           if ((splits = launch_wgrad_tma(act + Q.dhid, 512, act + Q.act3, 3136, n, wsbig, s, "naturecnn/fc_wgrad")) < 0) return splits; }
         { ProfScope ps(s, "wgrad_fold_bias", 0, 0);
-          note_launches(1); tc_fold_fc<<<(unsigned)ceil_div((int64_t)512 * 3136, 256), 256, 0, s>>>(wsbig, splits, 512, 13 * 256, 512, 3136, 64, 49, 1.f, grads + L.fcw);
+          if ((rc = launch_pdl("naturecnn/fc_fold", tc_fold_fc, (unsigned)ceil_div((int64_t)512 * 3136, 256), 256, 0, s,
+                               wsbig, splits, 512, 13 * 256, 512, 3136, 64, 49, 1.f, grads + L.fcw))) return rc;
           if ((rc = colsum(act + Q.dhid, n, 512, 512, wssmall, grads + L.fcb, s))) return rc; }
         if (tail_ready_event) {
             cudaError_t e = cudaEventRecord(reinterpret_cast<cudaEvent_t>(tail_ready_event), s);
@@ -237,8 +237,8 @@
         for (int k = 0; k < 10; ++k) { fw.slot_tap[k] = st[k]; fw.slot_skip[k] = (k == 8); }
         { ProfScope ps(s, "wgrad_fold_bias", 0, 0);
           fw.wsb = wssmall; fw.db = grads + L.c3b;
-          tc_fold_win<<<(unsigned)ceil_div(640 * 64 + 64, 32), 256, 0, s>>>(wsbig, fw, grads + L.c3w);
-          if ((rc = check_launch("naturecnn/conv3_fold"))) return rc; }
+          if ((rc = launch_pdl("naturecnn/conv3_fold", tc_fold_win, (unsigned)ceil_div(640 * 64 + 64, 32), 256, 0, s, wsbig, fw,
+                               grads + L.c3w))) return rc; }
         win_defaults(wp);
         wp.A = act + Q.dact3b; wp.n = (int)n; wp.G = 121; wp.Wp = 11; wp.M = n * 121; wp.ntaps = 9;
         for (int ky = 0; ky < 3; ++ky) for (int kx = 0; kx < 3; ++kx) wp.shift[ky * 3 + kx] = (2 - ky) * 11 + (2 - kx);
@@ -263,8 +263,8 @@
         for (int k = 0; k < 8; ++k) { fw.slot_tap[k] = k >> 1; fw.slot_cc[k] = k & 1; }
         { ProfScope ps(s, "wgrad_fold_bias", 0, 0);
           fw.wsb = wssmall; fw.db = grads + L.c2b;
-          tc_fold_win<<<(unsigned)ceil_div(512 * 64 + 64, 32), 256, 0, s>>>(wsbig, fw, grads + L.c2w);
-          if ((rc = check_launch("naturecnn/conv2_fold"))) return rc; }
+          if ((rc = launch_pdl("naturecnn/conv2_fold", tc_fold_win, (unsigned)ceil_div(512 * 64 + 64, 32), 256, 0, s, wsbig, fw,
+                               grads + L.c2w))) return rc; }
         if (dact1_fused) return B200RL_OK;
         win_defaults(wp);
         wp.A = act + Q.dact2b; wp.n = (int)n; wp.G = 121; wp.Wp = 11; wp.M = n * 121; wp.ntaps = 4;
@@ -343,8 +343,7 @@
     B200RL_REQUIRE(n <= (int64_t)1 << 28, "frames_to_s2d_u8: n too large");
     cudaStream_t s = (cudaStream_t)stream;
     ProfScope ps(s, "frames_to_s2d", 0, (double)n * (28224 + 28224 + 28672));
-    tc_frames_to_s2d_u8<<<(unsigned)(n * 4), 256, 0, s>>>(obs, rows, n, out_rm, out_cm);
-    return check_launch("frames_to_s2d_u8");
+    return launch_pdl("frames_to_s2d_u8", tc_frames_to_s2d_u8, (unsigned)(n * 4), 256, 0, s, obs, rows, n, out_rm, out_cm);
 }
 
 static size_t naturecnn_big_bytes(int64_t n, const NatureLayout& L) {
@@ -368,18 +367,24 @@
     bf16* P = reinterpret_cast<bf16*>(packed);
     cudaStream_t s = (cudaStream_t)stream;
     ProfScope ps(s, "pack_weights", 0, (double)L.total * 4 + (double)L.packed_total * 2);
-    tc_pack_conv1_s2d<<<32, 256, 0, s>>>(params + L.c1w, P + L.w1f);
-    tc_pack_conv1_i8<<<32, 256, 0, s>>>(params + L.c1w, reinterpret_cast<int8_t*>(P + L.w1l), reinterpret_cast<float*>(P + L.w1sc));
-    tc_pack_conv2_cells<<<128, 256, 0, s>>>(params + L.c2w, P + L.w2f);
-    tc_pack_conv_s2_classes<<<(unsigned)ceil_div(32768, 256), 256, 0, s>>>(params + L.c2w, 64, 32, P + L.w2dg);
-    tc_pack_conv<<<(unsigned)ceil_div(36864, 256), 256, 0, s>>>(params + L.c3w, 64, 64, 3, 3, 0, P + L.w3f, P + L.w3dg);
-    tc_pack_fc<<<dim3(512 / 8, 49 / 7), 256, 0, s>>>(params + L.fcw, 512, 49, P + L.wfcf, P + L.wfcdg);
+    const char* what = "naturecnn_pack";
+    int rc;
+    if ((rc = launch_pdl(what, tc_pack_conv1_s2d, 32, 256, 0, s, params + L.c1w, P + L.w1f))) return rc;
+    if ((rc = launch_pdl(what, tc_pack_conv1_i8, 32, 256, 0, s, params + L.c1w, reinterpret_cast<int8_t*>(P + L.w1l),
+                         reinterpret_cast<float*>(P + L.w1sc)))) return rc;
+    if ((rc = launch_pdl(what, tc_pack_conv2_cells, 128, 256, 0, s, params + L.c2w, P + L.w2f))) return rc;
+    if ((rc = launch_pdl(what, tc_pack_conv_s2_classes, (unsigned)ceil_div(32768, 256), 256, 0, s, params + L.c2w, 64, 32,
+                         P + L.w2dg))) return rc;
+    if ((rc = launch_pdl(what, tc_pack_conv, (unsigned)ceil_div(36864, 256), 256, 0, s, params + L.c3w, 64, 64, 3, 3, 0,
+                         P + L.w3f, P + L.w3dg))) return rc;
+    if ((rc = launch_pdl(what, tc_pack_fc, dim3(512 / 8, 49 / 7), 256, 0, s, params + L.fcw, 512, 49, P + L.wfcf, P + L.wfcdg)))
+        return rc;
     if (L.wide) {
         tc_pack_head_wide<<<(unsigned)ceil_div((int64_t)L.G * 512, 256), 256, 0, s>>>(params + L.hw, params + L.hb, A + 1, L.G,
                                                                                     P + L.whf, P + L.whdg, reinterpret_cast<float*>(P + L.hbp));
-        return check_launch("naturecnn_pack", 7);
-    }
-    return check_launch("naturecnn_pack", 6);
+        return check_launch(what);
+    }
+    return B200RL_OK;
 }
 
 extern "C" int b200rl_naturecnn_bf16_forward(const void* obs, int obs_format, const int64_t* rows, int64_t n, int A,
@@ -497,8 +502,8 @@
     for (int k = 0; k < 4; ++k) fw.slot_tap[k] = k;
     { ProfScope ps(s, "wgrad_fold_bias", 0, 0);
       fw.wsb = wssmall; fw.db = grads + L.c1b;
-      tc_fold_win<<<(unsigned)ceil_div(256 * 32 + 32, 32), 256, 0, s>>>(wsbig, fw, grads + L.c1w);
-      if ((rc = check_launch("naturecnn/conv1_fold"))) return rc; }
+      if ((rc = launch_pdl("naturecnn/conv1_fold", tc_fold_win, (unsigned)ceil_div(256 * 32 + 32, 32), 256, 0, s, wsbig, fw,
+                           grads + L.c1w))) return rc; }
     return B200RL_OK;
 }
 
diff --git a/cleanrl_b200/csrc/optim.cu b/cleanrl_b200/csrc/optim.cu
--- a/cleanrl_b200/csrc/optim.cu
+++ b/cleanrl_b200/csrc/optim.cu
@@ -15,6 +15,7 @@
 __global__ void __launch_bounds__(kOptThreads) grad_sumsq_kernel(
     const float* __restrict__ g, int64_t P, float inv_world_is_div, float world,
     float max_norm, OptScratch* sc, double* partials, float* norm_out) {
+    pdl_wait(); pdl_launch_dependents();
     __shared__ float red[32];
     __shared__ bool is_last;
     float s = 0.f;
@@ -87,6 +88,7 @@
 __global__ void __launch_bounds__(kOptThreads) adam_kernel(
     float* __restrict__ p, const float* __restrict__ g, float* __restrict__ m, float* __restrict__ v,
     int64_t P, AdamScalars a, const OptScratch* sc, const float* __restrict__ dyn) {
+    pdl_wait(); pdl_launch_dependents();
     if (dyn) { a.bc2_sqrt = __ldg(dyn); a.neg_step_size = __ldg(dyn + 1); }
     const float coef = a.do_clip ? sc->coef : 1.f;
     const int64_t stride = (int64_t)gridDim.x * blockDim.x;
@@ -158,10 +160,9 @@
     if (need_norm) {
         cudaError_t e = cudaMemsetAsync(&sc->ticket, 0, sizeof(unsigned int), s);
         if (e != cudaSuccess) return fail(B200RL_ERR_CUDA, "clip_adam: memset: %s", cudaGetErrorString(e));
-        grad_sumsq_kernel<<<blocks, kOptThreads, 0, s>>>(grads, P, world_size > 1 ? 1.f : 0.f, (float)world_size,
-                                                        (float)max_norm, sc, partials, norm_out);
-        int rc = check_launch("clip_adam/sumsq");
-        if (rc) return rc;
+        if (int rc = launch_pdl("clip_adam/sumsq", grad_sumsq_kernel, blocks, kOptThreads, 0, s, grads, P,
+                                world_size > 1 ? 1.f : 0.f, (float)world_size, (float)max_norm, sc, partials, norm_out))
+            return rc;
     }
     AdamScalars a;
     a.w1 = (float)(1.0 - beta1);
@@ -174,8 +175,8 @@
     a.world = (float)world_size;
     a.divide_world = world_size > 1;
     a.do_clip = max_norm >= 0.0;
-    adam_kernel<<<blocks, kOptThreads, 0, s>>>(params, grads, exp_avg, exp_avg_sq, P, a, sc, dyn);
-    return check_launch("clip_adam/adam");
+    return launch_pdl("clip_adam/adam", adam_kernel, blocks, kOptThreads, 0, s, params, grads, exp_avg, exp_avg_sq, P, a,
+                      sc, dyn);
 }
 }
 
diff --git a/cleanrl_b200/csrc/policy.cu b/cleanrl_b200/csrc/policy.cu
--- a/cleanrl_b200/csrc/policy.cu
+++ b/cleanrl_b200/csrc/policy.cu
@@ -35,6 +35,8 @@
     float* __restrict__ value_out) {
     const int64_t i = (int64_t)blockIdx.x * blockDim.x + threadIdx.x;
     if (i >= n) return;
+    pdl_wait();
+    pdl_launch_dependents();
     const float* x = logits + i * ld;
     const float* q = noise + i * (int64_t)A;
     const RowStats rs = row_stats(x, A);
@@ -98,6 +100,7 @@
 }
 __global__ void __launch_bounds__(1024) adv_stats_kernel(
     const float* __restrict__ b_adv, const int64_t* __restrict__ inds, int64_t M, float* __restrict__ out2) {
+    pdl_wait(); pdl_launch_dependents();
     __shared__ float red[32];
     const float mean = block_sum(adv_pass(b_adv, inds, M, 0.f, false), red) / (float)M;
     const float ss = block_sum(adv_pass(b_adv, inds, M, mean, true), red);
@@ -128,6 +131,7 @@
 };
 
 __global__ void __launch_bounds__(kLossThreads) ppo_loss_kernel(LossParams P) {
+    pdl_wait(); pdl_launch_dependents();
     __shared__ float red[32];
     __shared__ bool is_last;
     const int64_t i = (int64_t)blockIdx.x * blockDim.x + threadIdx.x;
@@ -427,9 +431,8 @@
     B200RL_REQUIRE(ld_logits >= A, "categorical_sample: ld_logits < A");
     const unsigned blocks = (unsigned)ceil_div(n, 128);
     ProfScope ps((cudaStream_t)stream, "categorical_sample", 0, (double)n * (8.0 * A + 24));
-    categorical_sample_kernel<<<blocks, 128, 0, (cudaStream_t)stream>>>(
-        logits, ld_logits, noise, value_in, ld_value, n, A, action, logprob, entropy, value_out);
-    return check_launch("categorical_sample");
+    return launch_pdl("categorical_sample", categorical_sample_kernel, blocks, 128, 0, (cudaStream_t)stream,
+                      logits, ld_logits, noise, value_in, ld_value, n, A, action, logprob, entropy, value_out);
 }
 
 extern "C" int b200rl_categorical_eval_f32(const float* logits, int64_t ld_logits, const int64_t* action,
@@ -481,7 +484,9 @@
     ProfScope ps(s, "ppo_loss", 0, (double)M * (44.0 + 8.0 * A));
     cudaError_t e = cudaMemsetAsync(ticket, 0, sizeof(unsigned int), s);
     if (e != cudaSuccess) return fail(B200RL_ERR_CUDA, "ppo_loss: memset: %s", cudaGetErrorString(e));
-    if (norm_adv) { note_launches(1); adv_stats_kernel<<<1, 1024, 0, s>>>(b_advantages, mb_inds, M, adv_stats); }
+    if (norm_adv) {
+        if (int rc = launch_pdl("ppo_loss", adv_stats_kernel, 1, 1024, 0, s, b_advantages, mb_inds, M, adv_stats)) return rc;
+    }
     LossParams P;
     P.logits = new_logits; P.ld = ld_logits; P.value = new_value; P.ldv = ld_value;
     P.inds = mb_inds; P.b_actions = b_actions; P.b_logprobs = b_logprobs; P.b_adv = b_advantages;
@@ -491,8 +496,7 @@
     P.dlogits = dlogits; P.ldd = ld_dlogits; P.dvalue = dvalue; P.lddv = ld_dvalue;
     P.stats = stats; P.adv_stats = adv_stats; P.partials = partials; P.ticket = ticket;
     const unsigned blocks = (unsigned)ceil_div(M, kLossThreads);
-    ppo_loss_kernel<<<blocks, kLossThreads, 0, s>>>(P);
-    return check_launch("ppo_loss");
+    return launch_pdl("ppo_loss", ppo_loss_kernel, blocks, kLossThreads, 0, s, P);
 }
 
 extern "C" int b200rl_gaussian_sample_f32(const float* mean, int64_t ld_mean, const float* logstd, const float* noise,
diff --git a/cleanrl_b200/csrc/tc_aux.cuh b/cleanrl_b200/csrc/tc_aux.cuh
--- a/cleanrl_b200/csrc/tc_aux.cuh
+++ b/cleanrl_b200/csrc/tc_aux.cuh
@@ -29,6 +29,7 @@
 
 __global__ void tc_pack_conv(const float* __restrict__ w, int Cout, int Cin, int KH, int KW, int nchw_k,
                              bf16* __restrict__ fwd, bf16* __restrict__ dgrad) {
+    pdl_wait(); pdl_launch_dependents();
     const int64_t idx = (int64_t)blockIdx.x * blockDim.x + threadIdx.x;
     const int64_t total = (int64_t)Cout * Cin * KH * KW;
     if (idx >= total) return;
@@ -42,6 +43,7 @@
     if (dgrad) dgrad[(int64_t)c * (KH * KW * Cout) + (ky * KW + kx) * Cout + co] = v;
 }
 __global__ void tc_pack_conv1_s2d(const float* __restrict__ w, bf16* __restrict__ fwd) {
+    pdl_wait(); pdl_launch_dependents();
     const int idx = blockIdx.x * blockDim.x + threadIdx.x;
     if (idx >= 32 * 256) return;
     const int kx = idx & 7, ky = (idx >> 3) & 7, c = (idx >> 6) & 3, co = idx >> 8;
@@ -49,6 +51,7 @@
     fwd[co * 256 + (a * 2 + b) * 64 + c * 16 + sy * 4 + sx] = __float2bfloat16(w[idx]);
 }
 __global__ void tc_pack_conv2_cells(const float* __restrict__ w, bf16* __restrict__ fwd) {
+    pdl_wait(); pdl_launch_dependents();
     const int idx = blockIdx.x * blockDim.x + threadIdx.x;
     if (idx >= 64 * 512) return;
     const int kx = idx & 3, ky = (idx >> 2) & 3, c = (idx >> 4) & 31, co = idx >> 9;
@@ -56,6 +59,7 @@
     fwd[co * 512 + (a * 2 + b) * 128 + (py * 2 + px) * 32 + c] = __float2bfloat16(w[idx]);
 }
 __global__ void tc_pack_conv_s2_classes(const float* __restrict__ w, int Cout, int Cin, bf16* __restrict__ dg) {
+    pdl_wait(); pdl_launch_dependents();
     const int64_t idx = (int64_t)blockIdx.x * blockDim.x + threadIdx.x;
     const int64_t total = (int64_t)4 * Cin * 4 * Cout;
     if (idx >= total) return;
@@ -67,6 +71,7 @@
 }
 __global__ void __launch_bounds__(256) tc_pack_fc(const float* __restrict__ w, int O, int PP, bf16* __restrict__ fwd,
                                                   bf16* __restrict__ dgrad) {
+    pdl_wait(); pdl_launch_dependents();
     constexpr int C = 64, PS = 7, R = 8;
     __shared__ float sw[R * C * PS];
     const int K = C * PP;
diff --git a/cleanrl_b200/csrc/tc_conv1_u8.cuh b/cleanrl_b200/csrc/tc_conv1_u8.cuh
--- a/cleanrl_b200/csrc/tc_conv1_u8.cuh
+++ b/cleanrl_b200/csrc/tc_conv1_u8.cuh
@@ -18,6 +18,8 @@
     __shared__ __align__(16) uint8_t plane[7056];
     const int64_t i = blockIdx.x >> 2;
     const int c = blockIdx.x & 3;
+    pdl_wait();
+    pdl_launch_dependents();
     const int64_t img = rows ? rows[i] : i;
     const int4* src = reinterpret_cast<const int4*>(obs + img * 28224 + c * 7056);
     for (int t = threadIdx.x; t < 441; t += 256) reinterpret_cast<int4*>(plane)[t] = __ldg(src + t);
@@ -47,6 +49,7 @@
 }
 
 __global__ void __launch_bounds__(256) tc_pack_conv1_i8(const float* __restrict__ w, int8_t* __restrict__ limbs, float* __restrict__ sc) {
+    pdl_wait(); pdl_launch_dependents();
     __shared__ float red[32];
     const int co = blockIdx.x, idx = threadIdx.x;
     const float v = w[co * 256 + idx];
@@ -114,6 +117,8 @@
     if (tid < 32) { s_sc[tid] = p.sc[32 + tid]; s_bias[tid] = p.bias[tid]; }
     fence_proxy_async_smem();
     __syncthreads();
+    pdl_wait();
+    pdl_launch_dependents();
     const int tile_begin = (int)(((int64_t)total_tiles * blockIdx.x) / gridDim.x);
     const int tile_end = (int)(((int64_t)total_tiles * (blockIdx.x + 1)) / gridDim.x);
 
@@ -287,6 +292,8 @@
     for (int idx = tid; idx < 2 * kC21ImgBytes / 16; idx += blockDim.x) reinterpret_cast<int4*>(sImg)[idx] = make_int4(0, 0, 0, 0);
     fence_proxy_async_smem();
     __syncthreads();
+    pdl_wait();
+    pdl_launch_dependents();
     const int64_t M = (int64_t)p.n * 512;
     const int64_t m_begin = (int64_t)blockIdx.x * p.rows_per_cta;
     int64_t m_end = m_begin + p.rows_per_cta;
@@ -492,8 +499,7 @@
     if ((rc = make_tmap_3d_u8(&tmY, dact1_f16, p.n, 441, 64, 64, 128, 64, what))) return rc;
     static SmemAttrCache attr;
     if ((rc = attr.ensure(tc_conv21_bwd_u8, smem, what))) return rc;
-    tc_conv21_bwd_u8<<<ctas, kC1WThreads, smem, s>>>(tmX, tmWin, tmY, p);
-    return check_launch(what);
+    return launch_pdl(what, tc_conv21_bwd_u8, ctas, kC1WThreads, smem, s, tmX, tmWin, tmY, p);
 }
 
 constexpr int kConv1I8Stages = 8;
@@ -509,8 +515,7 @@
     if (rc) return rc;
     static SmemAttrCache attr;
     if ((rc = attr.ensure(tc_conv1_i8<STAGES>, smem, what))) return rc;
-    tc_conv1_i8<STAGES><<<grid, kConv1I8Threads, smem, s>>>(tmA, p, total);
-    return check_launch(what);
-}
-
-}
+    return launch_pdl(what, tc_conv1_i8<STAGES>, grid, kConv1I8Threads, smem, s, tmA, p, total);
+}
+
+}
diff --git a/cleanrl_b200/csrc/tc_conv_win.cuh b/cleanrl_b200/csrc/tc_conv_win.cuh
--- a/cleanrl_b200/csrc/tc_conv_win.cuh
+++ b/cleanrl_b200/csrc/tc_conv_win.cuh
@@ -326,6 +326,8 @@
     }
     fence_proxy_async_smem();
     __syncthreads();
+    pdl_wait();
+    pdl_launch_dependents();
     const int tile_begin = (int)(((int64_t)total_tiles * blockIdx.x) / gridDim.x);
     const int tile_end = (int)(((int64_t)total_tiles * (blockIdx.x + 1)) / gridDim.x);
 
@@ -496,8 +498,7 @@
     CUtensorMap tmA;
     memset(&tmA, 0, sizeof(tmA));
     if (int rc = make_tmap_2d(&tmA, p.A, p.M, (int64_t)CPR * 64, p.WR, what)) return rc;
-    tc_conv_win_t<BP, CPR, STAGES, NTAPS><<<grid, kConvWinTThreads, smem, s>>>(tmA, p, total);
-    return check_launch(what);
+    return launch_pdl(what, tc_conv_win_t<BP, CPR, STAGES, NTAPS>, grid, kConvWinTThreads, smem, s, tmA, p, total);
 }
 
 }
diff --git a/cleanrl_b200/csrc/tc_gemm_tma.cuh b/cleanrl_b200/csrc/tc_gemm_tma.cuh
--- a/cleanrl_b200/csrc/tc_gemm_tma.cuh
+++ b/cleanrl_b200/csrc/tc_gemm_tma.cuh
@@ -47,6 +47,8 @@
         tma_prefetch_desc(&tmB);
     }
     __syncthreads();
+    pdl_wait();
+    pdl_launch_dependents();
 
     if (warp == 0) {
         if ((tid & 31) == 0) {
@@ -184,6 +186,8 @@
         tma_prefetch_desc(&tmY);
     }
     __syncthreads();
+    pdl_wait();
+    pdl_launch_dependents();
     const int64_t m_begin = (int64_t)blockIdx.x * rows_per_cta;
     int64_t m_end = m_begin + rows_per_cta;
     if (m_end > M) m_end = M;
@@ -249,8 +253,7 @@
     const int total = (int)ceil_div(p.M, 128) * ntn;
     int grid = num_sms();
     if (grid > total) grid = total;
-    tc_gemm_tma<BN, STAGES><<<grid, kGemmThreads, smem, s>>>(tmA, tmB, p, total, ntn);
-    return check_launch(what);
+    return launch_pdl(what, tc_gemm_tma<BN, STAGES>, grid, kGemmThreads, smem, s, tmA, tmB, p, total, ntn);
 }
 
 static int64_t round_up(int64_t a, int64_t b) { return ceil_div(a, b) * b; }
@@ -280,8 +283,7 @@
     static SmemAttrCache attr;
     if ((rc = attr.ensure(tc_wgrad_tma, smem, what))) return rc;
     const dim3 grid(pl.splits, xcols / (64 * kFcWgradXChunks), (unsigned)ceil_div(ycols, 64 * kFcWgradYChunks));
-    tc_wgrad_tma<<<grid, kWgradTmaThreads, smem, s>>>(tmX, tmY, M, pl.rows_per_cta, ws);
-    if ((rc = check_launch(what))) return rc;
+    if ((rc = launch_pdl(what, tc_wgrad_tma, grid, kWgradTmaThreads, smem, s, tmX, tmY, M, pl.rows_per_cta, ws))) return rc;
     return pl.splits;
 }
 
diff --git a/cleanrl_b200/csrc/tc_heads.cuh b/cleanrl_b200/csrc/tc_heads.cuh
--- a/cleanrl_b200/csrc/tc_heads.cuh
+++ b/cleanrl_b200/csrc/tc_heads.cuh
@@ -22,6 +22,8 @@
     extern __shared__ float sW[];
     for (int i = threadIdx.x; i < A1 * HT; i += blockDim.x) sW[i] = Wh[i];
     __syncthreads();
+    pdl_wait();
+    pdl_launch_dependents();
     const int lane = threadIdx.x & 31, wpb = blockDim.x >> 5;
     for (int64_t row = (int64_t)blockIdx.x * wpb + (threadIdx.x >> 5); row < n; row += (int64_t)gridDim.x * wpb) {
         float hv[8 * NQ];
@@ -60,6 +62,7 @@
 __global__ void __launch_bounds__(256) tc_heads_bwd_data(const float* __restrict__ dhead, const float* __restrict__ Wh,
                                                          const uint8_t* __restrict__ hid_bits, int64_t n, int A1, int H,
                                                          bf16* __restrict__ dhid) {
+    pdl_wait(); pdl_launch_dependents();
     constexpr int G = HT / 8;
     extern __shared__ float sWt[];
     for (int i = threadIdx.x; i < A1 * HT; i += blockDim.x) {
@@ -92,6 +95,7 @@
 __global__ void __launch_bounds__(512) tc_heads_bwd_weight(const float* __restrict__ dhead, const bf16* __restrict__ hid,
                                                            int64_t n, int A1, int H, int64_t rows_per_block,
                                                            float* __restrict__ part) {
+    pdl_wait(); pdl_launch_dependents();
     extern __shared__ float sD[];
     const int hp = threadIdx.x % (HT / 2), rl = threadIdx.x / (HT / 2);
     const int64_t r0 = (int64_t)blockIdx.x * rows_per_block;
@@ -145,6 +149,7 @@
 }
 static __global__ void __launch_bounds__(256) tc_heads_fold(const float* __restrict__ part, int nslabs, int A1, int H,
                                                      float* __restrict__ dW, float* __restrict__ db) {
+    pdl_wait(); pdl_launch_dependents();
     __shared__ float red[256];
     const int idx = blockIdx.x * 32 + (threadIdx.x & 31);
     const int a = idx / (H + 2), h = idx - a * (H + 2);
@@ -159,8 +164,7 @@
                      const char* what) {
     static_assert(H == 128 || H == 256 || H == 512, "head input width");
     const int grid = (int)(ceil_div(n, 8) < (int64_t)num_sms() * 8 ? ceil_div(n, 8) : (int64_t)num_sms() * 8);
-    tc_heads_fwd<H><<<grid, 256, (size_t)A1 * H * sizeof(float), s>>>(hid, Wh, bh, n, A1, H, out);
-    return check_launch(what);
+    return launch_pdl(what, tc_heads_fwd<H>, grid, 256, (size_t)A1 * H * sizeof(float), s, hid, Wh, bh, n, A1, H, out);
 }
 static size_t heads_partial_bytes(int64_t n, int A1, int H) {
     return (size_t)2 * ceil_div(n, heads_rows_per_block(n)) * A1 * (H + 2) * sizeof(float);
@@ -172,18 +176,17 @@
     const int64_t rpb = heads_rows_per_block(n);
     const int nb = (int)ceil_div(n, rpb);
     const size_t sd = (size_t)rpb * A1 * sizeof(float);
-    if (A1 <= 8) tc_heads_bwd_weight<8, H><<<nb, H, sd, s>>>(dhead, hid, n, A1, H, rpb, part);
-    else tc_heads_bwd_weight<kMaxHeads, H><<<nb, H, sd, s>>>(dhead, hid, n, A1, H, rpb, part);
-    tc_heads_fold<<<(unsigned)ceil_div(A1 * (H + 2), 32), 256, 0, s>>>(part, 2 * nb, A1, H, dW, db);
-    return check_launch(what, 2);
+    int rc = A1 <= 8 ? launch_pdl(what, tc_heads_bwd_weight<8, H>, nb, H, sd, s, dhead, hid, n, A1, H, rpb, part)
+                     : launch_pdl(what, tc_heads_bwd_weight<kMaxHeads, H>, nb, H, sd, s, dhead, hid, n, A1, H, rpb, part);
+    if (rc) return rc;
+    return launch_pdl(what, tc_heads_fold, (unsigned)ceil_div(A1 * (H + 2), 32), 256, 0, s, part, 2 * nb, A1, H, dW, db);
 }
 template <int H>
 static int heads_bwd_data(const float* dhead, const float* Wh, const uint8_t* hid_bits, int64_t n, int A1, bf16* dhid,
                           cudaStream_t s, const char* what) {
     static_assert(H == 128 || H == 256 || H == 512, "head input width");
     const int grid = (int)(ceil_div(n * H, 2048) < (int64_t)num_sms() * 8 ? ceil_div(n * H, 2048) : (int64_t)num_sms() * 8);
-    tc_heads_bwd_data<H><<<grid, 256, (size_t)A1 * H * sizeof(float), s>>>(dhead, Wh, hid_bits, n, A1, H, dhid);
-    return check_launch(what);
+    return launch_pdl(what, tc_heads_bwd_data<H>, grid, 256, (size_t)A1 * H * sizeof(float), s, dhead, Wh, hid_bits, n, A1, H, dhid);
 }
 
 }
diff --git a/cleanrl_b200/csrc/tc_reduce.cuh b/cleanrl_b200/csrc/tc_reduce.cuh
--- a/cleanrl_b200/csrc/tc_reduce.cuh
+++ b/cleanrl_b200/csrc/tc_reduce.cuh
@@ -32,6 +32,7 @@
                  float bscale;
                  const float* wsb; float* db; };
 static __global__ void __launch_bounds__(256) tc_fold_win(const float* __restrict__ ws, const FoldWin f, float* __restrict__ dst) {
+    pdl_wait(); pdl_launch_dependents();
     __shared__ float red[256];
     const int idx = blockIdx.x * 32 + (threadIdx.x & 31);
     const int KX = f.nslots * 64;
@@ -65,6 +66,7 @@
 
 static __global__ void tc_fold_fc(const float* __restrict__ ws, int S, int KX, int NY, int validX, int validY,
                            int C, int KK, float scale, float* __restrict__ dst) {
+    pdl_wait(); pdl_launch_dependents();
     const int64_t idx = (int64_t)blockIdx.x * blockDim.x + threadIdx.x;
     const int64_t total = (int64_t)validX * validY;
     if (idx >= total) return;
@@ -78,6 +80,7 @@
 
 static __global__ void __launch_bounds__(256) tc_colsum_partial(const bf16* __restrict__ Y, int64_t M, int ld, int ncols,
                                                          int64_t rows_per_block, float* __restrict__ part) {
+    pdl_wait(); pdl_launch_dependents();
     __shared__ float red[256 * 8];
     const int cg = ncols >> 3;
     const int lanes = 256 / cg;
@@ -111,6 +114,7 @@
 }
 static __global__ void __launch_bounds__(256) tc_colsum_final(const float* __restrict__ part, int nblocks, int ncols,
                                                        float* __restrict__ db) {
+    pdl_wait(); pdl_launch_dependents();
     __shared__ float red[256];
     const int c = blockIdx.x * 32 + (threadIdx.x & 31);
     const float s = zlane_sum(part, ncols, nblocks, c, c < ncols, red);
@@ -124,9 +128,8 @@
 static int colsum(const bf16* Y, int64_t M, int ld, int ncols, float* part, float* db, cudaStream_t s) {
     const int64_t rpb = colsum_rows(M);
     const int nb = (int)ceil_div(M, rpb);
-    tc_colsum_partial<<<nb, 256, 0, s>>>(Y, M, ld, ncols, rpb, part);
-    tc_colsum_final<<<(unsigned)ceil_div(ncols, 32), 256, 0, s>>>(part, nb, ncols, db);
-    return check_launch("colsum", 2);
+    if (int rc = launch_pdl("colsum", tc_colsum_partial, nb, 256, 0, s, Y, M, ld, ncols, rpb, part)) return rc;
+    return launch_pdl("colsum", tc_colsum_final, (unsigned)ceil_div(ncols, 32), 256, 0, s, part, nb, ncols, db);
 }
 static size_t colsum_ws(int64_t M, int ncols) { return (size_t)ceil_div(M, colsum_rows(M)) * ncols * sizeof(float); }
 
diff --git a/cleanrl_b200/csrc/tc_wgrad_win.cuh b/cleanrl_b200/csrc/tc_wgrad_win.cuh
--- a/cleanrl_b200/csrc/tc_wgrad_win.cuh
+++ b/cleanrl_b200/csrc/tc_wgrad_win.cuh
@@ -96,6 +96,8 @@
         if (use_tma) tma_prefetch_desc(&tmY);
     }
     __syncthreads();
+    pdl_wait();
+    pdl_launch_dependents();
     const int64_t m_begin = (int64_t)blockIdx.y * p.rows_per_cta;
     int64_t m_end = m_begin + p.rows_per_cta;
     if (m_end > p.M) m_end = p.M;
diff --git a/cleanrl_b200/ppo_engine.py b/cleanrl_b200/ppo_engine.py
--- a/cleanrl_b200/ppo_engine.py
+++ b/cleanrl_b200/ppo_engine.py
@@ -156,7 +156,27 @@
             dst.copy_(src, non_blocking=True)
         self.h2d_bytes += src.numel() * src.element_size()
 
+    def _draw_step_noise(self):
+        if not hasattr(self.agent.noise_fn, "inplace"):
+            return None
+        if self.noise_buf is None:
+            self.noise_buf = torch.zeros(self.agent.noise_shape(self.N), dtype=torch.float32, device=self.device)
+        self.agent.draw_noise_into(self.noise_buf)
+        return self.noise_buf
+
+    def _draw_rollout_noise(self):
+        if not hasattr(self.agent.noise_fn, "inplace"):
+            return None
+        shape = (self.T,) + tuple(self.agent.noise_shape(self.N))
+        if getattr(self, "_rollout_noise", None) is None or tuple(self._rollout_noise.shape) != shape:
+            self._rollout_noise = torch.zeros(shape, dtype=torch.float32, device=self.device)
+        for t in range(self.T):
+            self.agent.draw_noise_into(self._rollout_noise[t])
+        return self._rollout_noise
+
     def _step_device_work(self, step, noise=None):
+        if noise is None:
+            noise = self._draw_step_noise()
         if self.s2d:
             self._to_storage(self.obs_u8, step)
         self.agent.sample_into(self.obs[step], self.actions[step], self.logprobs[step], self.values[step], noise=noise)
@@ -251,13 +271,15 @@
         P = obs_pool.shape[0]
 
         def work():
+            noise = self._draw_rollout_noise()
             for step in range(self.T):
                 src = obs_pool[step % P]
                 if self.s2d and src.dtype == torch.uint8:
                     self._to_storage(src, step)
                 else:
                     self.obs[step].copy_(src)
-                self.agent.sample_into(self.obs[step], self.actions[step], self.logprobs[step], self.values[step])
+                self.agent.sample_into(self.obs[step], self.actions[step], self.logprobs[step], self.values[step],
+                                       noise=None if noise is None else noise[step])
 
         if not self.agent.graph_friendly:
             return work()
```

Result: faster. 1.136 million (median of 6 runs) (+2.5%).
